# NVlabs/FoundationPose

Measured on AMD Instinct MI355X. Metric: pose-hypotheses/sec (raster+refine+score), 252 hyp x 160x160 @ 640x480 RGB-D, higher is better.
Workload: dtype f16

## Files before the change

foundationpose_amd/_lib.py:

```python
import ctypes as C
import os

import torch

_HERE = os.path.dirname(os.path.abspath(__file__))
LIB_PATH = os.environ.get("FP_AMD_LIB") or os.path.join(_HERE, "csrc", "libfp_amd.so")
ABI_VERSION = 230
_lib = None

vp, ci, cf, cd, sz = C.c_void_p, C.c_int, C.c_float, C.c_double, C.c_size_t

SIGNATURES = {
    "fp_last_error": (C.c_char_p, []),
    "fp_version": (ci, []),
    "fp_mesh_create": (ci, [vp, vp, vp, vp, vp, vp, vp, ci, ci, ci, ci, C.POINTER(vp)]),
    "fp_mesh_destroy": (None, [vp]),
    "fp_mesh_set_create": (ci, [vp, ci, C.POINTER(vp)]),
    "fp_mesh_set_destroy": (None, [vp]),
    "fp_mesh_set_workspace_bytes": (sz, [vp, ci, ci, ci]),
    "fp_depth_erode": (ci, [vp, vp, ci, ci, ci, cf, cf, cf, vp]),
    "fp_depth_bilateral": (ci, [vp, vp, ci, ci, ci, cf, cf, cf, vp]),
    "fp_depth_to_xyz": (ci, [vp, vp, cf, ci, vp, ci, ci, vp]),
    "fp_crop_windows": (ci, [vp, vp, vp, vp, ci, cd, vp, vp, ci, cd, ci, ci, ci, vp, vp, vp]),
    "fp_depth_erode_frames": (ci, [vp, vp, ci, ci, ci, ci, cf, cf, cf, vp]),
    "fp_depth_bilateral_frames": (ci, [vp, vp, ci, ci, ci, ci, cf, cf, cf, vp]),
    "fp_depth_to_xyz_frames": (ci, [vp, vp, cf, ci, vp, ci, ci, ci, vp]),
    "fp_mask_depth_stats": (ci, [vp, vp, vp, ci, ci, ci, ci, cf, vp, vp]),
    "fp_depth_agreement": (ci, [vp, vp, vp, vp, ci, ci, ci, ci, ci, ci, cf, vp, vp]),
    "fp_icp_workspace_bytes": (sz, [ci, ci, ci]),
    "fp_icp_point_plane": (ci, [vp, vp, vp, vp, vp, ci, ci, ci, vp, ci, ci, ci, cf, cd, ci, vp, vp, vp, sz, vp]),
    "fp_pose_errors_workspace_bytes": (sz, [ci, ci, ci]),
    "fp_pose_errors": (ci, [vp, ci, vp, ci, vp, vp, vp, ci, ci, ci, vp, vp, sz, vp]),
    "fp_vsd_counts": (ci, [vp, vp, vp, ci, ci, ci, ci, vp, vp, ci, ci, ci, ci, cf, vp, ci, vp, vp]),
    "fp_mspd": (ci, [vp, ci, vp, ci, vp, vp, vp, ci, ci, vp, vp, vp]),
    "fp_tsdf_integrate": (ci, [vp, vp, vp, vp, vp, ci, ci, ci, ci, ci, ci, vp, cf, cf, cf, vp, vp, vp, vp, vp]),
    "fp_tsdf_count_triangles": (ci, [vp, vp, ci, ci, ci, cf, vp, vp]),
    "fp_tsdf_emit_triangles": (ci, [vp, vp, vp, vp, ci, ci, ci, vp, cf, cf, vp, C.c_longlong, vp, vp, vp, vp, vp]),
    "fp_tsdf_label_components": (ci, [vp, ci, ci, ci, vp, vp, vp]),
    "fp_tsdf_raycast": (ci, [vp, vp, vp, vp, ci, ci, ci, vp, cf, cf, vp, vp, vp, vp, ci, vp, ci, ci, ci, ci, ci, cf, cf, cf, vp, vp, vp, vp, vp]),
    "fp_texture_bake": (ci, [vp, ci, vp, ci, vp, vp, vp, vp, vp, vp, ci, ci, ci, ci, ci, cf, cf, cf, vp, vp, vp]),
    "fp_workspace_bytes": (sz, [ci, ci, ci, ci, ci]),
    "fp_raster_lds_bytes": (sz, [ci]),
    "fp_render_crops": (ci, [vp, vp, vp, vp, cf, vp, vp, vp, vp, vp, ci, ci, ci, ci, ci, ci, cf, cf, cf, ci, vp, vp, vp, vp, vp, vp, vp, vp, sz, vp]),
    "fp_warp_crops": (ci, [vp, vp, vp, vp, vp, vp, vp, ci, vp, cf, vp, vp, ci, ci, ci, ci, ci, ci, ci, ci, vp, vp]),
    "fp_pose_update": (ci, [vp, vp, vp, ci, ci, vp, cf, cf, vp, vp, ci, ci, vp, vp, vp, ci, vp, vp, vp, ci, vp, cf, vp]),
    "fp_conv7x7s2_bn_relu_fwd": (ci, [vp, vp, vp, vp, vp, vp, ci, ci, ci, ci, vp]),
    "fp_igemm_f16_fwd": (ci, [vp, vp, vp, vp, vp, ci, ci, ci, ci, vp, vp]),
    "fp_pack_conv3x3_tiles_f16": (ci, [vp, vp, ci, ci, vp]),
    "fp_pack_conv3x3_tiles_direct_f16": (ci, [vp, vp, ci, ci, vp]),
    "fp_conv3x3_sw_lds_bytes": (ci, []),
    "fp_igemm_splitk_workspace_bytes": (sz, [ci, ci, ci]),
    "fp_igemm_f16_splitk_fwd": (ci, [vp, vp, vp, vp, vp, ci, ci, ci, ci, vp, ci, vp, sz, vp]),
    "fp_add_pe_f16_fwd": (ci, [vp, vp, vp, ci, ci, ci, vp]),
    "fp_replicate_rows_f16": (ci, [vp, vp, ci, ci, ci, ci, ci, C.c_longlong, vp]),
    "fp_replicate_segments_f16": (ci, [vp, vp, ci, ci, ci, ci, ci, C.c_longlong, vp]),
    "fp_layernorm_res_fwd": (ci, [vp, vp, vp, ci, vp, vp, vp, cf, vp, vp, ci, ci, vp]),
    "fp_pack_linear512_f16": (ci, [vp, vp, vp]),
    "fp_linear512_f16_fwd": (ci, [vp, vp, vp, vp, ci, ci, ci, vp]),
    "fp_linear_layernorm_fwd": (ci, [vp, vp, vp, vp, vp, vp, ci, vp, vp, cf, vp, vp, ci, ci, ci, ci, vp]),
    "fp_ffn_layernorm_mean_fwd": (ci, [vp, vp, vp, vp, vp, vp, vp, vp, cf, vp, vp, C.c_size_t, ci, ci, vp]),
    "fp_encoder_tail_workspace_bytes": (sz, [ci, ci]),
    "fp_encoder_tail_mean_fwd": (ci, [vp, ci, vp, vp, vp, vp, vp, vp, vp, vp, vp, vp, vp, vp, cf, vp, vp, sz, ci, ci, vp]),
    "fp_colmean_f16_fwd": (ci, [vp, vp, vp, vp, cf, vp, ci, ci, ci, vp]),
    "fp_rows_linear_fwd": (ci, [vp, vp, vp, vp, ci, ci, ci, ci, vp]),
    "fp_attention_f16_fwd": (ci, [vp, vp, ci, ci, ci, ci, ci, vp]),
    "fp_attention_segments_f16_fwd": (ci, [vp, vp, vp, ci, ci, ci, ci, ci, vp]),
    "fp_cluster_poses": (ci, [cf, cf, vp, ci, vp, ci, vp]),
}


class FpAmdError(RuntimeError):
    pass


def lib():
    global _lib
    if _lib is None:
        if not os.path.exists(LIB_PATH):
            raise FpAmdError(
                f"{LIB_PATH} is missing: the HIP extension is not built (run __graft_entry__.build() or "
                f"`make -C foundationpose_amd/csrc`). There is no CPU fallback.")
        handle = C.CDLL(LIB_PATH)
        for name, (res, args) in SIGNATURES.items():
            fn = getattr(handle, name)
            fn.restype = res
            fn.argtypes = args
        got = int(handle.fp_version())
        if got != ABI_VERSION:
            raise FpAmdError(f"{LIB_PATH} reports ABI version {got}, this binding was written for {ABI_VERSION}: rebuild the library "
                             f"(`make -C foundationpose_amd/csrc`) -- entry points changed meaning between versions (include/fp_amd.h)")
        _lib = handle
    return _lib


def check(status, what):
    if status != 0:
        msg = lib().fp_last_error()
        raise FpAmdError(f"{what} failed ({status}): {msg.decode() if msg else '?'}")
```

foundationpose_amd/csrc/conv_sw.hip:

```cpp
#include <hip/hip_fp16.h>
#include <stdlib.h>
#include <string.h>
#include <type_traits>
#include "igemm_common.h"
#include "igemm_epilogue.h"

#ifdef FP_PROFILE_BUILD
__device__ unsigned long long sw_dbg[10];
extern "C" int fp_dbg_conv_sw(unsigned long long* out, int reset) {
  if (reset) { unsigned long long z[10] = {0, 0, 0, 0, 0, 0, ~0ull, 0, 0, 0}; return (int)hipMemcpyToSymbol(HIP_SYMBOL(sw_dbg), z, sizeof(z)); }
  return (int)hipMemcpyFromSymbol(out, HIP_SYMBOL(sw_dbg), 8 * sizeof(unsigned long long));
}
extern "C" int fp_dbg_conv_sw_direct(unsigned long long* out) {
  return (int)hipMemcpyFromSymbol(out, HIP_SYMBOL(sw_dbg), 2 * sizeof(unsigned long long), 8 * sizeof(unsigned long long));
}
extern "C" int fp_dbg_conv_sw_epilogue(unsigned long long* out, int reset) {
  if (reset) { unsigned long long z[8] = {0, 0, 0, 0, 0, 0, 0, 0}; return (int)hipMemcpyToSymbol(HIP_SYMBOL(ig_epi_dbg), z, sizeof(z)); }
  return (int)hipMemcpyFromSymbol(out, HIP_SYMBOL(ig_epi_dbg), 8 * sizeof(unsigned long long));
}
#define SW_CLK(t) const unsigned long long t = wall_clock64()
#else
#define SW_CLK(t)
#endif

#ifndef SW_DEFAULT_VARIANT
#define SW_DEFAULT_VARIANT 0
#endif

namespace {

constexpr int SW_BK = 32, SW_NSTW = 4;
constexpr int sw_prows(int BM) { return BM == 256 ? 512 : 768; }

template <int N>
__device__ __forceinline__ void sw_wait_vm() {
  static_assert(N >= 0 && N < 64, "vmcnt is a 6-bit field");
  asm volatile("s_waitcnt vmcnt(%0)" ::"n"(N) : "memory");
}

typedef float sw_float4 __attribute__((ext_vector_type(4)));
__device__ __forceinline__ void sw_mfma16(sw_float4& acc, const half8& a, const half8& b) {
  asm volatile("v_mfma_f32_16x16x32_f16 %0, %1, %2, %0" : "+v"(acc) : "v"(a), "v"(b));
}

template <bool DIRECT>
__device__ __forceinline__ void sw_mfma16x(sw_float4& acc, const half8& w, const half8& a) {
  if constexpr (DIRECT) sw_mfma16(acc, a, w);
  else sw_mfma16(acc, w, a);
}

__host__ __device__ constexpr int sw_direct_row(int r) {
  return (r & 64) + 4 * (4 * ((0x2130 >> (4 * ((r >> 2) & 3))) & 3) + (r & 3)) + ((r >> 4) & 3);
}

__device__ __forceinline__ int sw_div(int n, unsigned mul, unsigned shr) { return (int)(__umulhi((unsigned)n, mul) >> shr); }

struct SwGeom {
  int HoWo, Wo, Hp, Wp;
  unsigned mulP, shrP, mulW, shrW;
};

template <typename G>
__device__ __forceinline__ int sw_q(const G& g, int m) {
  const int b = sw_div(m, g.mulP, g.shrP);
  const int r = m - b * g.HoWo;
  const int oy = sw_div(r, g.mulW, g.shrW);
  const int ox = r - oy * g.Wo;
  return (b * g.Hp + oy) * g.Wp + ox;
}

template <int BM, int BN, int TM, bool S16>
__global__ __launch_bounds__(512, 1) void k_conv_sw(IgemmParams p) {
  constexpr bool DIRECT = false;
#include "conv_sw_tile.inc"
}

template <int BM, int BN, int TM, bool S16>
__global__ __launch_bounds__(512, 1) void k_conv_sw_direct(IgemmParams p) {
  constexpr bool DIRECT = true;
#include "conv_sw_tile.inc"
}

constexpr int LS_PROWS = 448, LS_NSTW = 3;

template <int BM, int BN, int TM>
__global__ __launch_bounds__(256, 2) void k_conv_sw_ls(IgemmParams p) {
  constexpr int BK = SW_BK, NW = 4, THREADS = 256;
  constexpr int NWN = BN / 64;
  static_assert((BM / (32 * TM)) * NWN == NW, "4 waves");
  constexpr int ROWB = BK * 2;
  constexpr int W_BYTES = BN * ROWB;
  constexpr int PATCH_BYTES = LS_PROWS * ROWB;
  constexpr int WI = BN / 16 / NW;
  constexpr int PI = LS_PROWS / 16 / NW;
  static_assert(WI >= 1 && PI >= 1 && PI <= 8 && LS_PROWS == PI * 16 * NW, "tile shape");
  constexpr int STAGES_BYTES = 2 * PATCH_BYTES + LS_NSTW * W_BYTES;
  static_assert(STAGES_BYTES >= BM * BN * 2 + BM * 16 + IG_BIAS_LDS, "the epilogue tile, its tables and the vectors reuse the staging area");
  auto swz = [](int row) { return (row >> 2) & 3; };
  extern __shared__ __attribute__((aligned(16))) unsigned char smem[];
  unsigned char* const patch = smem;
  unsigned char* const wring = smem + 2 * PATCH_BYTES;
  const int tid = threadIdx.x, lane = tid & 63;
  const int wid = __builtin_amdgcn_readfirstlane(tid >> 6);
  const int wm = wid / NWN, wn = wid - wm * NWN;

  const int tiles_n = p.N / BN;
  const int nwg = gridDim.x;
  const int xcd = blockIdx.x & 7, loc = blockIdx.x >> 3;
  const int qd8 = nwg >> 3, r8 = nwg & 7;
  const int tile = (xcd < r8 ? xcd * (qd8 + 1) : r8 * (qd8 + 1) + (xcd - r8) * qd8) + loc;
  const int bm = tile / tiles_n, bn = tile - bm * tiles_n;
  const int m0 = bm * BM, n0 = bn * BN;
  const int Cin = p.Cin, Ktot = 9 * Cin, Wp = p.in.Wp;
  const int ncc = Cin / BK;

  const int q0 = sw_q(p.in, m0);
  const int qmax = (p.M / p.in.HoWo) * p.in.Hp * Wp - 1;
  unsigned poff32[PI], woff32[WI];
#pragma unroll
  for (int j = 0; j < PI; ++j) {
    const int row = (wid * PI + j) * 16 + (lane >> 2);
    const int c = (lane & 3) ^ swz(row);
    int q = q0 + row;
    q = q < qmax ? q : qmax;
    poff32[j] = (unsigned)(((long long)q * p.in.cstride + p.in.coff + c * 8) * 2);
  }
#pragma unroll
  for (int j = 0; j < WI; ++j) {
    const int row = (wid * WI + j) * 16 + (lane >> 2);
    const int c = (lane & 3) ^ swz(row);
    woff32[j] = (unsigned)((((size_t)(n0 + row) * Ktot) + c * 8) * 2);
  }
  const __amdgpu_buffer_rsrc_t rsA = __builtin_amdgcn_make_buffer_rsrc(const_cast<_Float16*>(p.A), 0, 0x7FFFFFFF, 0x00020000);
  const __amdgpu_buffer_rsrc_t rsW = __builtin_amdgcn_make_buffer_rsrc(const_cast<_Float16*>(p.Wt), 0, 0x7FFFFFFF, 0x00020000);

  auto stage_patch = [&](int cc, int j) {
    unsigned char* dst = patch + (cc & 1) * PATCH_BYTES + (wid * PI + j) * 1024;
    __builtin_amdgcn_raw_ptr_buffer_load_lds(rsA, (__attribute__((address_space(3))) void*)dst, 16, (int)poff32[j],
                                             cc * (BK * 2), 0, 0);
  };
  auto stage_w = [&](int cc, int tap, int slot) {
    const int wsoff = (tap * Cin + cc * BK) * 2;
    unsigned char* dst = wring + slot * W_BYTES + wid * (WI * 1024);
#pragma unroll
    for (int j = 0; j < WI; ++j)
      __builtin_amdgcn_raw_ptr_buffer_load_lds(rsW, (__attribute__((address_space(3))) void*)(dst + j * 1024), 16,
                                               (int)woff32[j], wsoff, 0, 0);
  };

  float16_ acc[2][TM];
#pragma unroll
  for (int i = 0; i < 2; ++i)
#pragma unroll
    for (int j = 0; j < TM; ++j)
#pragma unroll
      for (int e = 0; e < 16; ++e) acc[i][j][e] = 0.f;

  const int frow = lane & 31, fhalf = lane >> 5;
  int arow[TM], w_off[2][2];
#pragma unroll
  for (int t = 0; t < TM; ++t) {
    int m = m0 + wm * (32 * TM) + t * 32 + frow;
    m = m < p.M ? m : p.M - 1;
    arow[t] = sw_q(p.in, m) - q0;
  }
#pragma unroll
  for (int t = 0; t < 2; ++t) {
    const int rw = wn * 64 + t * 32 + frow;
#pragma unroll
    for (int kk = 0; kk < 2; ++kk) w_off[t][kk] = rw * ROWB + (((2 * kk + fhalf) ^ swz(rw)) << 4);
  }

#pragma unroll
  for (int j = 0; j < PI; ++j) stage_patch(0, j);
  stage_w(0, 0, 0);
  stage_w(0, 1, 1);

  auto kstep = [&](int cc, auto tap_c, auto last_c, auto first_c) {
    constexpr int T = decltype(tap_c)::value;
    constexpr bool LAST = decltype(last_c)::value;
    constexpr bool FIRST = decltype(first_c)::value;
    constexpr int ky = T / 3, kx = T - 3 * ky;
    {
      constexpr bool prev_w = FIRST || T == 0 || !LAST || (T - 1) + 2 < 9;
      constexpr bool prev_p = !FIRST && T >= 1 && !LAST && (T - 1) < PI;
      sw_wait_vm<(prev_w ? WI : 0) + (prev_p ? 1 : 0)>();
    }
    __builtin_amdgcn_sched_barrier(0);
    __builtin_amdgcn_s_barrier();
    __builtin_amdgcn_sched_barrier(0);
    if constexpr (!LAST) {
      if constexpr (T < PI) stage_patch(cc + 1, T);
      if constexpr (T + 2 < 9) stage_w(cc, T + 2, (T + 2) % LS_NSTW);
      else stage_w(cc + 1, T - 7, (T + 2) % LS_NSTW);
    } else {
      if constexpr (T + 2 < 9) stage_w(cc, T + 2, (T + 2) % LS_NSTW);
    }
    const unsigned char* pb = patch + (cc & 1) * PATCH_BYTES;
    const unsigned char* wb = wring + (T % LS_NSTW) * W_BYTES;
    const int shift = ky * Wp + kx;
    half8 fa[2][TM], fw[2][2];
    int a0[TM];
#pragma unroll
    for (int t = 0; t < TM; ++t) {
      int ar = arow[t];
      asm volatile("" : "+v"(ar));
      const int pr = ar + shift;
      a0[t] = (pr << 6) + ((fhalf ^ swz(pr)) << 4);
    }
#pragma unroll
    for (int t = 0; t < TM; ++t) fa[0][t] = *reinterpret_cast<const half8*>(pb + a0[t]);
#pragma unroll
    for (int t = 0; t < 2; ++t) fw[0][t] = *reinterpret_cast<const half8*>(wb + w_off[t][0]);
#pragma unroll
    for (int t = 0; t < TM; ++t) fa[1][t] = *reinterpret_cast<const half8*>(pb + (a0[t] ^ 32));
#pragma unroll
    for (int t = 0; t < 2; ++t) fw[1][t] = *reinterpret_cast<const half8*>(wb + w_off[t][1]);
    __builtin_amdgcn_sched_barrier(0);
#pragma unroll
    for (int kk = 0; kk < 2; ++kk)
#pragma unroll
      for (int i = 0; i < 2; ++i)
#pragma unroll
        for (int j = 0; j < TM; ++j)
          acc[i][j] = __builtin_amdgcn_mfma_f32_32x32x16_f16(fw[kk][i], fa[kk][j], acc[i][j], 0, 0, 0);
    __builtin_amdgcn_sched_barrier(0);
  };
  auto chunk = [&](int cc, auto last_c, auto first_c) {
    kstep(cc, std::integral_constant<int, 0>{}, last_c, first_c);
    kstep(cc, std::integral_constant<int, 1>{}, last_c, std::false_type{});
    kstep(cc, std::integral_constant<int, 2>{}, last_c, std::false_type{});
    kstep(cc, std::integral_constant<int, 3>{}, last_c, std::false_type{});
    kstep(cc, std::integral_constant<int, 4>{}, last_c, std::false_type{});
    kstep(cc, std::integral_constant<int, 5>{}, last_c, std::false_type{});
    kstep(cc, std::integral_constant<int, 6>{}, last_c, std::false_type{});
    kstep(cc, std::integral_constant<int, 7>{}, last_c, std::false_type{});
    kstep(cc, std::integral_constant<int, 8>{}, last_c, std::false_type{});
  };
  chunk(0, std::false_type{}, std::true_type{});
  for (int cc = 1; cc + 1 < ncc; ++cc) chunk(cc, std::false_type{}, std::false_type{});
  chunk(ncc - 1, std::true_type{}, std::false_type{});
  __syncthreads();
  float* bias_lds = reinterpret_cast<float*>(smem + BM * BN * 2 + BM * 16);
  ig_bias_to_lds(p, n0, bias_lds, wid, lane);
  asm volatile("s_waitcnt vmcnt(0)" ::: "memory");
  ig_epilogue<BM, BN, TM, THREADS, 0>(p, acc, smem, m0, n0, wm, wn, tid, lane, bias_lds);
}

template <int BM, int BN, int TM>
int sw_ls_launch(const IgemmParams& p, hipStream_t stream) {
  constexpr int LDS = 2 * LS_PROWS * SW_BK * 2 + LS_NSTW * BN * SW_BK * 2;
  static_assert(2 * LDS <= 160 * 1024, "two workgroups per CU");
  const long long tiles = (long long)fp_cdiv(p.M, BM) * (p.N / BN);
  FP_REQUIRE(tiles < (1ll << 31), "fp_igemm_f16_fwd: too many tiles");
  FP_SET_MAX_LDS((k_conv_sw_ls<BM, BN, TM>), LDS);
  hipLaunchKernelGGL((k_conv_sw_ls<BM, BN, TM>), dim3((unsigned)tiles), dim3(256), LDS, stream, p);
  FP_CHECK_LAUNCH("fp_igemm_f16_fwd(conv_sw_ls)");
  return FP_OK;
}

constexpr int sw_lds_bytes(int BM, int BN) {
  return (BM == 256 ? ig_lds_main_slim<256, 256>(2 * sw_prows(256) * SW_BK * 2 + SW_NSTW * 256 * SW_BK * 2)
                    : ig_lds_main_slim<512, 128>(2 * sw_prows(512) * SW_BK * 2 + SW_NSTW * 128 * SW_BK * 2)) + IG_BIAS_LDS;
}

template <int BM, int BN, int TM, bool S16>
int sw_launch(const IgemmParams& p, hipStream_t stream) {
  static_assert((BM == 256 && BN == 256) || (BM == 512 && BN == 128), "tile shapes of sw_lds_bytes");
  constexpr int LDS = sw_lds_bytes(BM, BN);
  static_assert(LDS <= 160 * 1024, "does not fit the 160 KiB LDS");
  const long long tiles = (long long)fp_cdiv(p.M, BM) * (p.N / BN);
  FP_REQUIRE(tiles < (1ll << 31), "fp_igemm_f16_fwd: too many tiles");
  FP_SET_MAX_LDS((k_conv_sw<BM, BN, TM, S16>), LDS);
  hipLaunchKernelGGL((k_conv_sw<BM, BN, TM, S16>), dim3((unsigned)tiles), dim3(512), LDS, stream, p);
  FP_CHECK_LAUNCH("fp_igemm_f16_fwd(conv_sw)");
  return FP_OK;
}

}

static int sw_span(const IgemmGeom& g, int BM) {
  const int row_cross = (BM - 1) / g.Wo + 1, img_cross = (BM - 1) / g.HoWo + 1;
  return (BM - 1) + 2 * row_cross + (2 * g.Wp + 2) * img_cross + 2 * g.Wp + 3;
}

static int sw_variant(const IgemmParams& p) {
  int v = SW_DEFAULT_VARIANT;
#ifdef FP_PROFILE_BUILD
  static int forced = -2;
  if (forced == -2) {
    const char* e = getenv("FP_CONV_SW");
    forced = e ? (!strcmp(e, "ls") ? 1 : (!strcmp(e, "pp") ? 0 : -1)) : -1;
  }
  if (forced >= 0) v = forced;
#endif
  if (v == 2) v = p.Cin <= 128 ? 1 : 0;
  if (v == 3) v = p.Cin <= 256 ? 1 : 0;
  if (v == 1 && sw_span(p.in, 256) > LS_PROWS) v = 0;
  return v;
}

#ifndef SW_FORCE_512
#define SW_FORCE_512 1
#endif
static bool sw_use_256(const IgemmParams& p) { return (p.N % 256) == 0 && (!SW_FORCE_512 || p.M < 2 * 512); }
static int sw_tile_rows(const IgemmParams& p) { return sw_variant(p) == 1 ? 256 : (sw_use_256(p) ? 256 : 512); }

bool fp_conv3x3_sw_applicable(const IgemmParams& p) {
  const IgemmGeom& g = p.in;
  if (p.taps != 9 || g.stride != 1 || g.off != 0 || g.bsplit != 0) return false;
  if (g.HoWo % g.Wo != 0 || g.Wp != g.Wo + 2 || g.Hp != g.HoWo / g.Wo + 2) return false;
  if (g.Wo < 2) return false;
  const int BM = sw_tile_rows(p);
  if (p.M % g.HoWo != 0 || p.M < 2 * BM) return false;
  if (p.Cin % 64 != 0 || p.N % 128 != 0) return false;
  const long long bytes = (long long)(p.M / g.HoWo) * g.Hp * g.Wp * g.cstride * 2;
  if (bytes >= (1ll << 31)) return false;
  if (g.cstride >= (1 << 19)) return false;
  const IgemmGeom& o = p.out;
  const long long imgs = o.bsplit > 0 ? o.bsplit : p.M / g.HoWo, groups = o.bsplit > 0 ? (p.M / g.HoWo) / o.bsplit + 1 : 0;
  if (imgs * o.Hp * o.Wp * o.cstride + o.coff + groups * (long long)o.cgroup >= (1ll << 31)) return false;
  if (p.R) {
    const IgemmGeom& r = p.res;
    const long long rimgs = r.bsplit > 0 ? r.bsplit : p.M / g.HoWo, rgroups = r.bsplit > 0 ? (p.M / g.HoWo) / r.bsplit + 1 : 0;
    if (rimgs * r.Hp * r.Wp * r.cstride + r.coff + rgroups * (long long)r.cgroup >= (1ll << 31)) return false;
  }
  return sw_span(g, BM) <= (sw_variant(p) == 1 ? LS_PROWS : sw_prows(BM));
}

int fp_conv3x3_sw_tile_rows(const IgemmParams& p) { return sw_tile_rows(p); }

extern "C" int fp_conv3x3_sw_lds_bytes(void) { return sw_lds_bytes(512, 128); }

static bool sw_direct(const IgemmParams& p) {
  if (!p.direct || !p.mfma16 || sw_variant(p) == 1 || sw_use_256(p)) return false;
  return p.epi == IG_EPI_CONV || p.epi == (IG_EPI_CONV | IG_EPI_RES) || p.epi == (IG_EPI_CONV | IG_EPI_BN) || p.epi == (IG_EPI_CONV | IG_EPI_BN | IG_EPI_RES);
}

static int sw_direct_launch(const IgemmParams& p, hipStream_t stream) {
  constexpr int LDS = sw_lds_bytes(512, 128);
  const long long tiles = (long long)fp_cdiv(p.M, 512) * (p.N / 128);
  FP_REQUIRE(tiles < (1ll << 31), "fp_igemm_f16_fwd: too many tiles");
  FP_SET_MAX_LDS((k_conv_sw_direct<512, 128, 4, true>), LDS);
  hipLaunchKernelGGL((k_conv_sw_direct<512, 128, 4, true>), dim3((unsigned)tiles), dim3(512), LDS, stream, p);
  FP_CHECK_LAUNCH("fp_igemm_f16_fwd(conv_sw_direct)");
  return FP_OK;
}

int fp_conv3x3_sw_launch(const IgemmParams& p, hipStream_t stream) {
  const bool direct = sw_direct(p);
  if (p.Wpk && sw_variant(p) != 1 && !sw_use_256(p))
    FP_REQUIRE((p.wpk_direct != 0) == direct, "fp_igemm_f16_fwd: w_tiles is in the layout of %s but this launch runs %s (FP_IGEMM_W_TILES_DIRECT, FP_IGEMM_DIRECT_STORE)",
               p.wpk_direct ? "fp_pack_conv3x3_tiles_direct_f16" : "fp_pack_conv3x3_tiles_f16", direct ? "k_conv_sw_direct" : "k_conv_sw");
  if (direct) return sw_direct_launch(p, stream);
  if (sw_variant(p) == 1) return sw_ls_launch<256, 128, 4>(p, stream);
  if (sw_use_256(p)) return p.mfma16 ? sw_launch<256, 256, 4, true>(p, stream) : sw_launch<256, 256, 4, false>(p, stream);
  return p.mfma16 ? sw_launch<512, 128, 4, true>(p, stream) : sw_launch<512, 128, 4, false>(p, stream);
}

template <bool DIRECT>
__global__ __launch_bounds__(256) void k_pack_conv3x3_tiles(const _Float16* __restrict__ w, _Float16* __restrict__ out, int N, int Cin) {
  const int nk = 9 * (Cin / 32);
  const long long total = (long long)N * nk * 4;
  const long long q = (long long)blockIdx.x * 256 + threadIdx.x;
  if (q >= total) return;
  const int pc = (int)(q & 3);
  const int r = (int)((q >> 2) & 127);
  const long long blk = q >> 9;
  const int s = (int)(blk % nk), bn = (int)(blk / nk);
  const int cc = s / 9, tap = s - 9 * cc;
  const int lc = pc ^ ((r >> 2) & 3);
  const int src = DIRECT ? sw_direct_row(r) : r;
  const half8 v = *reinterpret_cast<const half8*>(w + (size_t)(bn * 128 + src) * (9 * Cin) + tap * Cin + cc * 32 + lc * 8);
  *reinterpret_cast<half8*>(out + q * 8) = v;
}

template <bool DIRECT>
static int sw_pack_tiles(const void* w, void* w_tiles, int N, int Cin, void* stream, const char* who) {
  FP_REQUIRE(w && w_tiles && w != w_tiles, "%s: NULL tensor or in-place repack", who);
  FP_REQUIRE(N > 0 && N % 128 == 0 && Cin > 0 && Cin % 32 == 0, "%s: N=%d must be a multiple of 128, Cin=%d of 32", who, N, Cin);
  FP_REQUIRE((((size_t)w | (size_t)w_tiles) & 15) == 0, "%s: tensors must be 16-byte aligned", who);
  const long long total = (long long)N * 9 * (Cin / 32) * 4;
  hipLaunchKernelGGL(k_pack_conv3x3_tiles<DIRECT>, dim3((unsigned)((total + 255) / 256)), dim3(256), 0, (hipStream_t)stream, (const _Float16*)w,
                     (_Float16*)w_tiles, N, Cin);
  FP_CHECK_LAUNCH(who);
  return FP_OK;
}

extern "C" int fp_pack_conv3x3_tiles_f16(const void* w, void* w_tiles, int N, int Cin, void* stream) {
  return sw_pack_tiles<false>(w, w_tiles, N, Cin, stream, "fp_pack_conv3x3_tiles_f16");
}

extern "C" int fp_pack_conv3x3_tiles_direct_f16(const void* w, void* w_tiles, int N, int Cin, void* stream) {
  return sw_pack_tiles<true>(w, w_tiles, N, Cin, stream, "fp_pack_conv3x3_tiles_direct_f16");
}
```

foundationpose_amd/csrc/conv_sw_tile.inc:

```
  static_assert(!DIRECT || (S16 && BM == 512 && BN == 128 && TM == 4), "the direct epilogue is the 512 x 128 tile's, on 16x16x32 MFMAs");
  constexpr int BK = SW_BK, NW = 8, THREADS = 512;
  constexpr int NWN = BN / 64;
  static_assert((BM / (32 * TM)) * NWN == NW, "8 waves");
  constexpr int ROWB = BK * 2;
  constexpr int W_BYTES = BN * ROWB;
  constexpr int SW_PROWS = sw_prows(BM);
  constexpr int SW_PATCH_BYTES = SW_PROWS * ROWB;
  constexpr int WI = BN / 16 / NW;
  constexpr int PI = SW_PROWS / 16 / NW;
  static_assert(WI >= 1 && PI >= 1 && PI <= 7 && SW_PROWS == PI * 16 * NW, "tile shape");
  constexpr int STAGES_BYTES = 2 * SW_PATCH_BYTES + SW_NSTW * W_BYTES;
  constexpr int LDS_MAIN = ig_lds_main_slim<BM, BN>(STAGES_BYTES);
  auto swz = [](int row) { return (row >> 2) & 3; };
  auto swzp = [](int row) { return S16 ? (row >> 1) & 2 : (row >> 2) & 3; };
  extern __shared__ __attribute__((aligned(16))) unsigned char smem[];
  SW_CLK(t_start);
  unsigned char* const patch = smem;
  unsigned char* const wring = smem + 2 * SW_PATCH_BYTES;
  const int tid = threadIdx.x, lane = tid & 63;
  const int wid = __builtin_amdgcn_readfirstlane(tid >> 6);
  const int grp = wid >> 2;
  const int wm = wid / NWN, wn = wid - wm * NWN;
  float* bias_lds = reinterpret_cast<float*>(smem + LDS_MAIN);

  const _Float16* A_ = p.A;
  const _Float16* W_ = p.Wt;
  const _Float16* Wpk_ = p.Wpk;
  const float* bias_ = p.bias;
  const float* bnsc_ = p.bn_scale;
  const float* bnsh_ = p.bn_shift;
  const int M = p.M, N = p.N, Cin = p.Cin, cstride = p.in.cstride, coff = p.in.coff;
  const SwGeom gi = {p.in.HoWo, p.in.Wo, p.in.Hp, p.in.Wp, p.in.mulP, p.in.shrP, p.in.mulW, p.in.shrW};
  asm volatile("" ::"s"(A_), "s"(W_), "s"(Wpk_), "s"(bias_), "s"(bnsc_), "s"(bnsh_), "s"(M), "s"(N), "s"(Cin), "s"(cstride), "s"(coff),
               "s"(gi.HoWo), "s"(gi.Wo), "s"(gi.Hp), "s"(gi.Wp), "s"(gi.mulP), "s"(gi.shrP), "s"(gi.mulW), "s"(gi.shrW));
  __builtin_amdgcn_sched_barrier(0);

  const int tiles_n = N / BN;
  const int nwg = (int)(((unsigned)M + BM - 1) / BM) * tiles_n;
  const int xcd = blockIdx.x & 7, loc = blockIdx.x >> 3;
  const int qd8 = nwg >> 3, r8 = nwg & 7;
  const int tile = (xcd < r8 ? xcd * (qd8 + 1) : r8 * (qd8 + 1) + (xcd - r8) * qd8) + loc;
  const int bm = __builtin_popcount(tiles_n) == 1 ? tile >> __builtin_ctz(tiles_n) : tile / tiles_n, bn = tile - bm * tiles_n;
  const int m0 = bm * BM, n0 = bn * BN;
  const int Ktot = 9 * Cin, Wp = gi.Wp;
  const int ncc = Cin / BK;
  ig_bias_to_lds(bias_, bnsc_, bnsh_, N, n0, bias_lds, wid, lane);

  const int q0 = sw_q(gi, m0);
  const int qmax = sw_div(M, gi.mulP, gi.shrP) * gi.Hp * Wp - 1;
  unsigned poff32[PI], woff32[WI];
  {
    const int row0 = wid * PI * 16 + (lane >> 2);
    const int c = (lane & 3) ^ swzp(row0);
    static_assert(((16 >> 1) & 2) == 0 && ((16 >> 2) & 3) == 0, "swzp(row0 + 16 j) == swzp(row0)");
    const unsigned ps2 = (unsigned)cstride * 2, omax = (unsigned)qmax * ps2, lane_off = (unsigned)(coff + c * 8) * 2;
    const unsigned o0 = (unsigned)(q0 + row0) * ps2;
#pragma unroll
    for (int j = 0; j < PI; ++j) {
      const unsigned o = o0 + j * 16 * ps2;
      poff32[j] = (o < omax ? o : omax) + lane_off;
    }
  }
#pragma unroll
  for (int j = 0; j < WI; ++j) {
    const int row = (wid * WI + j) * 16 + (lane >> 2);
    const int c = (lane & 3) ^ swz(row);
    const int src = DIRECT ? sw_direct_row(row) : row;
    woff32[j] = (unsigned)((((size_t)(n0 + src) * Ktot) + c * 8) * 2);
  }
  const bool wpk = (BN == 128) && Wpk_ != nullptr;
  if (wpk) {
#pragma unroll
    for (int j = 0; j < WI; ++j) woff32[j] = (unsigned)(((wid * WI + j) * 64 + lane) * 16);
  }
  const int wpk_base = wpk ? bn * (ncc * 9) * W_BYTES : 0;
  const __amdgpu_buffer_rsrc_t rsA = __builtin_amdgcn_make_buffer_rsrc(const_cast<_Float16*>(A_), 0, 0x7FFFFFFF, 0x00020000);
  const __amdgpu_buffer_rsrc_t rsW = __builtin_amdgcn_make_buffer_rsrc(const_cast<_Float16*>(wpk ? Wpk_ : W_), 0, 0x7FFFFFFF, 0x00020000);

  auto stage_patch = [&](int cc, int j) {
    unsigned char* dst = patch + (cc & 1) * SW_PATCH_BYTES + (wid * PI + j) * 1024;
    __builtin_amdgcn_raw_ptr_buffer_load_lds(rsA, (__attribute__((address_space(3))) void*)dst, 16, (int)poff32[j],
                                             cc * (BK * 2), 0, 0);
  };
  auto stage_w = [&](int cc, int tap, int slot) {
    const int wsoff = wpk ? wpk_base + (cc * 9 + tap) * W_BYTES : (tap * Cin + cc * BK) * 2;
    unsigned char* dst = wring + slot * W_BYTES + wid * (WI * 1024);
#pragma unroll
    for (int j = 0; j < WI; ++j)
      __builtin_amdgcn_raw_ptr_buffer_load_lds(rsW, (__attribute__((address_space(3))) void*)(dst + j * 1024), 16,
                                               (int)woff32[j], wsoff, 0, 0);
  };

#pragma unroll
  for (int j = 0; j < PI; ++j) stage_patch(0, j);
  stage_w(0, 0, 0);
  stage_w(0, 1, 1);
  stage_w(0, 2, 2);
  __builtin_amdgcn_sched_barrier(0);
  SW_CLK(t_issue);

  constexpr int NFA = S16 ? 2 * TM : TM, NFW = S16 ? 4 : 2;
  constexpr int FR = S16 ? 16 : 32;
  typedef float float4_ __attribute__((ext_vector_type(4)));
  typedef typename std::conditional<S16, float4_, float16_>::type acc_t;
  acc_t acc[NFW][NFA];
#pragma unroll
  for (int i = 0; i < NFW; ++i)
#pragma unroll
    for (int j = 0; j < NFA; ++j)
#pragma unroll
      for (int e = 0; e < (S16 ? 4 : 16); ++e) acc[i][j][e] = 0.f;

  const int frow = lane & (FR - 1), fhalf = lane >> (S16 ? 4 : 5);
  int arow[NFA], w_off[2][2];
#pragma unroll
  for (int t = 0; t < NFA; ++t) {
    int m = m0 + wm * (32 * TM) + t * FR + frow;
    m = m < M ? m : M - 1;
    arow[t] = sw_q(gi, m) - q0;
    if constexpr (S16) arow[t] = (arow[t] << 6) + (fhalf << 4);
  }
  if constexpr (S16) {
    const int quad = (0x1320 >> (4 * (frow >> 2))) & 3;
#pragma unroll
    for (int t = 0; t < 4; ++t) {
      const int rw = wn * 64 + t * 16 + 4 * quad + (frow & 3);
      w_off[t >> 1][t & 1] = rw * ROWB + ((fhalf ^ swz(rw)) << 4);
    }
  } else {
#pragma unroll
    for (int t = 0; t < 2; ++t) {
      const int rw = wn * 64 + t * 32 + frow;
#pragma unroll
      for (int kk = 0; kk < 2; ++kk) w_off[t][kk] = rw * ROWB + (((2 * kk + fhalf) ^ swz(rw)) << 4);
    }
  }
  static_assert(TM == 4, "the fragment addresses of the next tap are computed behind the MFMA groups of a k-step, one per group of four");
  int anext[NFA], aflip[NFA];
#pragma unroll
  for (int t = 0; t < NFA; ++t) {
    anext[t] = S16 ? arow[t] : (arow[t] << 6) + ((fhalf ^ swz(arow[t])) << 4);
    aflip[t] = S16 ? (arow[t] >> 3) & 32 : 0;
  }

#pragma unroll
  for (int t = 0; t < NFA; ++t) {
    asm volatile("" : "+v"(arow[t]), "+v"(anext[t]));
    if constexpr (S16) asm volatile("" : "+v"(aflip[t]));
  }
  asm volatile("" : "+v"(w_off[0][0]), "+v"(w_off[0][1]), "+v"(w_off[1][0]), "+v"(w_off[1][1]));
#pragma unroll
  for (int i = 0; i < NFW; ++i)
#pragma unroll
    for (int j = 0; j < NFA; ++j) asm volatile("" : "+v"(acc[i][j]));
  if constexpr (DIRECT) {
    static_assert(THREADS == BM && STAGES_BYTES + BM * 4 <= LDS_MAIN, "one thread per row; the table lies behind the stages");
    const int m = m0 + tid;
    reinterpret_cast<int*>(smem + STAGES_BYTES)[tid] = m < M ? (int)(ig_row_off(p.out, m) + n0) : IG_ROW_NONE;
  }
  __builtin_amdgcn_sched_barrier(0);

  sw_wait_vm<2 * WI>();
  __builtin_amdgcn_s_barrier();
  SW_CLK(t_cold);
  if (grp) __builtin_amdgcn_s_barrier();

  half8 fa[2][TM], fw[2][2];
  auto kstep = [&](int cc, auto tap_c, auto last_c) {
    constexpr int T = decltype(tap_c)::value;
    constexpr bool LAST = decltype(last_c)::value;
    constexpr int ky = T / 3, kx = T - 3 * ky;
    const int s = cc * 9 + T;
    const unsigned char* pb = patch + (cc & 1) * SW_PATCH_BYTES;
    const unsigned char* wb = wring + (s & (SW_NSTW - 1)) * W_BYTES;
    const int shift = ky * Wp + kx;
    if constexpr (S16) {
#pragma unroll
      for (int t = 0; t < NFA; ++t) fa[t >> 2][t & 3] = *reinterpret_cast<const half8*>(pb + (anext[t] ^ aflip[t]));
#pragma unroll
      for (int t = 0; t < 4; ++t) fw[t >> 1][t & 1] = *reinterpret_cast<const half8*>(wb + w_off[t >> 1][t & 1]);
    } else {
#pragma unroll
      for (int t = 0; t < TM; ++t) {
        const int a0 = anext[t];
        fa[0][t] = *reinterpret_cast<const half8*>(pb + a0);
        fa[1][t] = *reinterpret_cast<const half8*>(pb + (a0 ^ 32));
      }
#pragma unroll
      for (int kk = 0; kk < 2; ++kk)
#pragma unroll
        for (int t = 0; t < 2; ++t) fw[kk][t] = *reinterpret_cast<const half8*>(wb + w_off[t][kk]);
    }
    (void)shift;
    if constexpr (!LAST) {
      if constexpr (T < PI) stage_patch(cc + 1, T);
      if constexpr (T + 3 < 9) stage_w(cc, T + 3, (s + 3) & (SW_NSTW - 1));
      else stage_w(cc + 1, T - 6, (s + 3) & (SW_NSTW - 1));
      constexpr int NP = (T < PI ? 1 : 0) + ((T >= 1 && T - 1 < PI) ? 1 : 0);
      sw_wait_vm<2 * WI + NP>();
    } else {
      if constexpr (T + 3 < 9) stage_w(cc, T + 3, (s + 3) & (SW_NSTW - 1));
      constexpr int NYOUNGER = T <= 5 ? 2 : (T == 6 ? 1 : 0);
      sw_wait_vm<NYOUNGER * WI>();
    }
    asm volatile("s_waitcnt lgkmcnt(0)" ::: "memory");
    __builtin_amdgcn_sched_barrier(0);
    __builtin_amdgcn_s_barrier();
    __builtin_amdgcn_sched_barrier(0);
    __builtin_amdgcn_s_setprio(1);
    {
      constexpr int TN = (T + 1) % 9, kyn = TN / 3, kxn = TN - 3 * kyn;
      const int shift_n = kyn * Wp + kxn;
      if constexpr (S16) {
        int sh = shift_n << 6;
        asm volatile("" : "+s"(sh));
#pragma unroll
        for (int i = 0; i < 4; ++i)
#pragma unroll
          for (int jh = 0; jh < 2; ++jh) {
            const int t = i * 2 + jh;
            int x, y;
            sw_mfma16x<DIRECT>(acc[i][jh * 4 + 0], fw[i >> 1][i & 1], fa[jh][0]);
            asm volatile("v_add_u32 %0, %1, %2" : "=v"(x) : "s"(sh), "v"(arow[t]));
            sw_mfma16x<DIRECT>(acc[i][jh * 4 + 1], fw[i >> 1][i & 1], fa[jh][1]);
            asm volatile("v_lshrrev_b32 %0, 3, %1" : "=v"(y) : "v"(x));
            sw_mfma16x<DIRECT>(acc[i][jh * 4 + 2], fw[i >> 1][i & 1], fa[jh][2]);
            asm volatile("v_and_b32 %0, 32, %0" : "+v"(y));
            sw_mfma16x<DIRECT>(acc[i][jh * 4 + 3], fw[i >> 1][i & 1], fa[jh][3]);
            anext[t] = x; aflip[t] = y;
          }
      } else {
#pragma unroll
      for (int kk = 0; kk < 2; ++kk)
#pragma unroll
        for (int i = 0; i < 2; ++i) {
#pragma unroll
          for (int j = 0; j < TM; ++j)
            acc[i][j] = __builtin_amdgcn_mfma_f32_32x32x16_f16(fw[kk][i], fa[kk][j], acc[i][j], 0, 0, 0);
          const int t = kk * 2 + i;
          {
            int ar = arow[t];
            asm volatile("" : "+v"(ar));
            const int pr = ar + shift_n;
            anext[t] = (pr << 6) + ((fhalf ^ swz(pr)) << 4);
          }
        }
      }
    }
    __builtin_amdgcn_s_setprio(0);
    __builtin_amdgcn_sched_barrier(0);
    __builtin_amdgcn_s_barrier();
    __builtin_amdgcn_sched_barrier(0);
  };
  auto chunk = [&](int cc, auto last_c) {
    kstep(cc, std::integral_constant<int, 0>{}, last_c);
    kstep(cc, std::integral_constant<int, 1>{}, last_c);
    kstep(cc, std::integral_constant<int, 2>{}, last_c);
    kstep(cc, std::integral_constant<int, 3>{}, last_c);
    kstep(cc, std::integral_constant<int, 4>{}, last_c);
    kstep(cc, std::integral_constant<int, 5>{}, last_c);
    kstep(cc, std::integral_constant<int, 6>{}, last_c);
    kstep(cc, std::integral_constant<int, 7>{}, last_c);
    kstep(cc, std::integral_constant<int, 8>{}, last_c);
  };
  for (int cc = 0; cc + 1 < ncc; ++cc) chunk(cc, std::false_type{});
  chunk(ncc - 1, std::true_type{});
  if (!grp) __builtin_amdgcn_s_barrier();
  __syncthreads();
  SW_CLK(t_loop);
  if constexpr (DIRECT) {
    const IgEpiArgs q = {p.out, p.res, p.R, p.Y, p.pe, p.Ype, p.pe_period, p.pe_mul, p.pe_shr, p.N};
    const int* rowY32 = reinterpret_cast<const int*>(smem + STAGES_BYTES);
#define SW_DIRECT_CASE(E)                                                                                     \
    case E:                                                                                                   \
      if (m0 + BM <= M) ig_epilogue_direct<E, true>(q, acc, smem, rowY32, m0, n0, M, wm, wn, tid, lane, bias_lds);  \
      else ig_epilogue_direct<E, false>(q, acc, smem, rowY32, m0, n0, M, wm, wn, tid, lane, bias_lds);         \
      break
    switch (p.epi) {
      SW_DIRECT_CASE(IG_EPI_CONV);
      SW_DIRECT_CASE(IG_EPI_CONV | IG_EPI_RES);
      SW_DIRECT_CASE(IG_EPI_CONV | IG_EPI_BN);
      SW_DIRECT_CASE(IG_EPI_CONV | IG_EPI_BN | IG_EPI_RES);
      default: break;
    }
#undef SW_DIRECT_CASE
  } else {
    ig_epilogue<BM, BN, TM, THREADS, 0, true>(p, acc, smem, m0, n0, wm, wn, tid, lane, bias_lds);
  }
#ifdef FP_PROFILE_BUILD
  asm volatile("s_waitcnt vmcnt(0)" ::: "memory");
  SW_CLK(t_end);
  if (tid == 0) {
    atomicAdd(&sw_dbg[0], t_cold - t_start); atomicAdd(&sw_dbg[1], t_loop - t_cold); atomicAdd(&sw_dbg[2], t_end - t_loop);
    atomicAdd(&sw_dbg[3], 1ull); atomicAdd(&sw_dbg[4], t_issue - t_start); atomicMin(&sw_dbg[6], t_start); atomicMax(&sw_dbg[7], t_end);
    if constexpr (DIRECT) { atomicAdd(&sw_dbg[8], t_end - t_loop); atomicAdd(&sw_dbg[9], 1ull); }
  }
#endif
```

foundationpose_amd/csrc/igemm.hip:

```cpp
#include <hip/hip_fp16.h>
#include <stdlib.h>
#include <string.h>
#include "igemm_common.h"
#include "igemm_epilogue.h"

int fp_igemm_pp_launch(const IgemmParams& p, int variant, hipStream_t stream);
int fp_conv3x3_sw_launch(const IgemmParams& p, hipStream_t stream);
bool fp_conv3x3_sw_applicable(const IgemmParams& p);
int fp_conv3x3_sw_tile_rows(const IgemmParams& p);

template <int BM, int BN, int TM, int NST, int BK, bool SPLITK = false>
__global__ __launch_bounds__((BM / (32 * TM)) * (BN / 64) * 64, ((BM / (32 * TM)) * (BN / 64) == 4 && TM == 4) ? 2 : 1) void k_igemm_f16(IgemmParams p) {
  constexpr int NWN = BN / 64;
  constexpr int NW = (BM / (32 * TM)) * NWN;
  constexpr int THREADS = NW * 64;
  constexpr int ROWB = BK * 2;
  constexpr int CPK = BK / 8;
  constexpr int RPI = 1024 / ROWB;
  constexpr int KK = BK / 16;
  constexpr int A_BYTES = BM * ROWB;
  constexpr int STAGE_BYTES = A_BYTES + BN * ROWB;
  constexpr int AI = BM / RPI / NW;
  constexpr int WI = BN / RPI / NW;
  static_assert(AI >= 1 && WI >= 1, "tile too small for this wave count");
// ... 14 lines not shown
  const int bm = tile / tiles_n, bn = tile - bm * tiles_n;
  const int m0 = bm * BM, n0 = bn * BN;
  const int Ktot = p.taps * p.Cin;
  if constexpr (!SPLITK) ig_bias_to_lds(p, n0, bias_lds, wid, lane);

  unsigned aoff32[AI], woff32[WI];
#pragma unroll
  for (int j = 0; j < AI; ++j) {
    const int row = wid * (AI * RPI) + j * RPI + lane / CPK;
    const int c = (lane % CPK) ^ swz(row);
    int m = m0 + row;
    m = m < p.M ? m : p.M - 1;
    aoff32[j] = (unsigned)((ig_row_off(p.in, m) + c * 8) * 2);
  }
#pragma unroll
  for (int j = 0; j < WI; ++j) {
    const int row = wid * (WI * RPI) + j * RPI + lane / CPK;
    const int c = (lane % CPK) ^ swz(row);
    woff32[j] = (unsigned)((((size_t)(n0 + row) * Ktot) + c * 8) * 2);
  }
  int nk = p.taps * (p.Cin / BK);
  int st_ci0 = 0, st_kx = 0, st_ky = 0, st_k = 0;
  const int inWp = p.in.Wp, inCs = p.in.cstride, Cin = p.Cin;
  if constexpr (SPLITK) {
    const int split = blockIdx.y, cpt = Cin / BK;
    const int ks0 = (int)(((long long)split * nk) / p.nsplit), ks1 = (int)(((long long)(split + 1) * nk) / p.nsplit);
    const int tap = ks0 / cpt;
    st_k = ks0; st_ci0 = (ks0 - tap * cpt) * BK; st_ky = tap / 3; st_kx = tap - 3 * st_ky;
    nk = ks1 - ks0;
  }
  const __amdgpu_buffer_rsrc_t rsA = __builtin_amdgcn_make_buffer_rsrc(const_cast<_Float16*>(p.A), 0, 0x7FFFFFFF, 0x00020000);
  const __amdgpu_buffer_rsrc_t rsW = __builtin_amdgcn_make_buffer_rsrc(const_cast<_Float16*>(p.Wt), 0, 0x7FFFFFFF, 0x00020000);

  auto stage = [&](int buf) {
    const int asoff = (((st_ky * inWp + st_kx) * inCs) + st_ci0) * 2;
    const int wsoff = st_k * (BK * 2);
    unsigned char* sa = smem + buf * STAGE_BYTES + wid * (AI * 1024);
    unsigned char* sw = smem + buf * STAGE_BYTES + A_BYTES + wid * (WI * 1024);
#pragma unroll
    for (int j = 0; j < AI; ++j)
      __builtin_amdgcn_raw_ptr_buffer_load_lds(rsA, (__attribute__((address_space(3))) void*)(sa + j * 1024), 16,
                                               (int)aoff32[j], asoff, 0, 0);
#pragma unroll
    for (int j = 0; j < WI; ++j)
      __builtin_amdgcn_raw_ptr_buffer_load_lds(rsW, (__attribute__((address_space(3))) void*)(sw + j * 1024), 16,
                                               (int)woff32[j], wsoff, 0, 0);
    ++st_k;
    st_ci0 += BK;
    if (st_ci0 == Cin) { st_ci0 = 0; if (++st_kx == 3) { st_kx = 0; ++st_ky; } }
  };

  float16_ acc[2][TM];
#pragma unroll
  for (int i = 0; i < 2; ++i)
#pragma unroll
    for (int j = 0; j < TM; ++j)
#pragma unroll
      for (int e = 0; e < 16; ++e) acc[i][j][e] = 0.f;

  const int frow = lane & 31, fhalf = lane >> 5;
  int a_off[TM][KK], w_off[2][KK];
#pragma unroll
  for (int t = 0; t < TM; ++t) {
    const int ra = wm * (32 * TM) + t * 32 + frow;
#pragma unroll
    for (int kk = 0; kk < KK; ++kk) a_off[t][kk] = ra * ROWB + (((2 * kk + fhalf) ^ swz(ra)) << 4);
  }
#pragma unroll
  for (int t = 0; t < 2; ++t) {
    const int rw = wn * 64 + t * 32 + frow;
#pragma unroll
    for (int kk = 0; kk < KK; ++kk) w_off[t][kk] = A_BYTES + rw * ROWB + (((2 * kk + fhalf) ^ swz(rw)) << 4);
  }

#pragma unroll
  for (int s = 0; s < NST - 1; ++s)
    if (s < nk) stage(s);
  int buf = 0, nbuf = NST - 1;
  for (int ks = 0; ks < nk; ++ks) {
    if (NST > 2 && ks + NST - 2 < nk) {
      constexpr int INFLIGHT = LPS * (NST - 2);
      static_assert(NST <= 2 || INFLIGHT == 4 || INFLIGHT == 6 || INFLIGHT == 8 || INFLIGHT == 12, "add the counted wait");
      if (INFLIGHT == 4) asm volatile("s_waitcnt vmcnt(4)" ::: "memory");
      else if (INFLIGHT == 6) asm volatile("s_waitcnt vmcnt(6)" ::: "memory");
      else if (INFLIGHT == 8) asm volatile("s_waitcnt vmcnt(8)" ::: "memory");
      else asm volatile("s_waitcnt vmcnt(12)" ::: "memory");
    } else {
      asm volatile("s_waitcnt vmcnt(0)" ::: "memory");
    }
    __builtin_amdgcn_s_barrier();
    if (ks + NST - 1 < nk) stage(nbuf);
    const unsigned char* sb = smem + buf * STAGE_BYTES;
    half8 fa[2][TM], fw[2][2];
    auto load_frags = [&](int kk, int slot) {
#pragma unroll
      for (int t = 0; t < TM; ++t) fa[slot][t] = *reinterpret_cast<const half8*>(sb + a_off[t][kk]);
#pragma unroll
      for (int t = 0; t < 2; ++t) fw[slot][t] = *reinterpret_cast<const half8*>(sb + w_off[t][kk]);
    };
    load_frags(0, 0);
#pragma unroll
    for (int kk = 0; kk < KK; ++kk) {
      if (kk < KK - 1) load_frags(kk + 1, (kk + 1) & 1);
      __builtin_amdgcn_sched_barrier(0);
#pragma unroll
      for (int i = 0; i < 2; ++i)
#pragma unroll
        for (int j = 0; j < TM; ++j)
          acc[i][j] = __builtin_amdgcn_mfma_f32_32x32x16_f16(fw[kk & 1][i], fa[kk & 1][j], acc[i][j], 0, 0, 0);
    }
    buf = (buf + 1 == NST) ? 0 : buf + 1;
    nbuf = (nbuf + 1 == NST) ? 0 : nbuf + 1;
  }
  if constexpr (SPLITK) {
    typedef float float4_ __attribute__((ext_vector_type(4)));
    float4_* dst = reinterpret_cast<float4_*>(p.slab) + ((((size_t)blockIdx.y * nwg + tile) * NW + wid) * (8 * TM)) * 64 + lane;
#pragma unroll
    for (int i = 0; i < 2; ++i)
#pragma unroll
      for (int g = 0; g < 4; ++g)
#pragma unroll
        for (int j = 0; j < TM; ++j) {
          const float4_ v = {acc[i][j][g * 4 + 0], acc[i][j][g * 4 + 1], acc[i][j][g * 4 + 2], acc[i][j][g * 4 + 3]};
          dst[((i * 4 + g) * TM + j) * 64] = v;
        }
    return;
  }
  __syncthreads();

  ig_epilogue<BM, BN, TM, THREADS, 0>(p, acc, smem, m0, n0, wm, wn, tid, lane, bias_lds);
}

template <int BM, int BN, int TM, int NST, int BK>
static int ig_launch(const IgemmParams& p, hipStream_t stream) {
  constexpr int LDS = ig_lds_main<BM, BN>(NST * (BM + BN) * BK * 2) + IG_BIAS_LDS;
  constexpr int THREADS = (BM / (32 * TM)) * (BN / 64) * 64;
  static_assert(LDS <= 160 * 1024, "tile does not fit the 160 KiB LDS");
  const long long tiles = (long long)fp_cdiv(p.M, BM) * (p.N / BN);
  FP_REQUIRE(tiles < (1ll << 31), "fp_igemm_f16_fwd: too many tiles");
  FP_SET_MAX_LDS((k_igemm_f16<BM, BN, TM, NST, BK>), LDS);
  hipLaunchKernelGGL((k_igemm_f16<BM, BN, TM, NST, BK>), dim3((unsigned)tiles), dim3(THREADS), LDS, stream, p);
  FP_CHECK_LAUNCH("fp_igemm_f16_fwd");
  return FP_OK;
}

template <int BM, int BN, int TM>
__global__ __launch_bounds__(256) void k_splitk_epilogue(IgemmParams p, int ntiles) {
  constexpr int NWN = BN / 64, NW = (BM / (32 * TM)) * NWN;
  typedef float float4_ __attribute__((ext_vector_type(4)));
  typedef _Float16 half2_ __attribute__((ext_vector_type(2)));
  const size_t t = (size_t)blockIdx.x * 256 + threadIdx.x;
  const int lane = (int)(t & 63);
  size_t q = t >> 6;
  const int j = (int)(q % TM); q /= TM;
  const int g = (int)(q & 3); q >>= 2;
  const int i = (int)(q & 1); q >>= 1;
  const int wid = (int)(q % NW);
  const int tile = (int)(q / NW);
  if (tile >= ntiles) return;
  const int tiles_n = p.N / BN;
  const int bm = tile / tiles_n, bn = tile - bm * tiles_n;
  const int wm = wid / NWN, wn = wid - wm * NWN;
  const int m = bm * BM + wm * (32 * TM) + j * 32 + (lane & 31);
  const int n = bn * BN + wn * 64 + i * 32 + 8 * g + 4 * (lane >> 5);
  if (m >= p.M) return;
  const float4_* src = reinterpret_cast<const float4_*>(p.slab) + t;
  const size_t per_split = (size_t)ntiles * NW * (8 * TM) * 64;
  float4_ a = src[0];
  for (int s = 1; s < p.nsplit; ++s) {
    const float4_ b = src[(size_t)s * per_split];
    a[0] += b[0]; a[1] += b[1]; a[2] += b[2]; a[3] += b[3];
  }
  float4_ bv = {0.f, 0.f, 0.f, 0.f};
  if (p.bias) bv = *reinterpret_cast<const float4_*>(p.bias + n);
  half4 v;
  if (p.round_acc) {
    const half2_ b01 = {(_Float16)bv[0], (_Float16)bv[1]}, b23 = {(_Float16)bv[2], (_Float16)bv[3]};
    half2_ t01 = {(_Float16)a[0], (_Float16)a[1]};
    half2_ t23 = {(_Float16)a[2], (_Float16)a[3]};
    t01 = t01 + b01;
    t23 = t23 + b23;
    if (p.bn_scale) {
      const float4_ sc = *reinterpret_cast<const float4_*>(p.bn_scale + n), sh = *reinterpret_cast<const float4_*>(p.bn_shift + n);
      v[0] = (_Float16)fmaf((float)t01[0], sc[0], sh[0]);
      v[1] = (_Float16)fmaf((float)t01[1], sc[1], sh[1]);
      v[2] = (_Float16)fmaf((float)t23[0], sc[2], sh[2]);
      v[3] = (_Float16)fmaf((float)t23[1], sc[3], sh[3]);
    } else {
      v[0] = t01[0]; v[1] = t01[1]; v[2] = t23[0]; v[3] = t23[1];
    }
  } else {
#pragma unroll
    for (int e = 0; e < 4; ++e) v[e] = (_Float16)(a[e] + bv[e]);
  }
  if (p.R) v = v + *reinterpret_cast<const half4*>(p.R + ig_row_off(p.res, m) + n);
  if (p.relu) {
    const half4 zero = {0, 0, 0, 0};
    v = __builtin_elementwise_max(v, zero);
  }
  *reinterpret_cast<half4*>(p.Y + ig_row_off(p.out, m) + n) = v;
  if (p.Ype) {
    const float4_ e0 = *reinterpret_cast<const float4_*>(p.pe + (size_t)(m % p.pe_period) * p.N + n);
    half4 w;
#pragma unroll
    for (int e = 0; e < 4; ++e) w[e] = (_Float16)((float)v[e] + e0[e]);
    *reinterpret_cast<half4*>(p.Ype + (size_t)m * p.N + n) = w;
  }
}

constexpr int SK_BM = 128, SK_BN = 128, SK_TM = 2, SK_NST = 2, SK_BK = 64;
static size_t ig_splitk_bytes(int M, int N, int splits) {
  return (size_t)splits * fp_cdiv(M, SK_BM) * (N / SK_BN) * (size_t)(SK_BM * SK_BN * 4);
}
static int ig_launch_splitk(const IgemmParams& p, hipStream_t stream) {
  constexpr int LDS = ig_lds_main<SK_BM, SK_BN>(SK_NST * (SK_BM + SK_BN) * SK_BK * 2) + IG_BIAS_LDS;
  const long long tiles = (long long)fp_cdiv(p.M, SK_BM) * (p.N / SK_BN);
  FP_REQUIRE(tiles * p.nsplit < (1ll << 31) && p.nsplit <= 65535, "fp_igemm_f16_splitk_fwd: too many tiles");
  FP_SET_MAX_LDS((k_igemm_f16<SK_BM, SK_BN, SK_TM, SK_NST, SK_BK, true>), LDS);
  hipLaunchKernelGGL((k_igemm_f16<SK_BM, SK_BN, SK_TM, SK_NST, SK_BK, true>), dim3((unsigned)tiles, (unsigned)p.nsplit), dim3(256), LDS, stream, p);
  FP_CHECK_LAUNCH("fp_igemm_f16_splitk_fwd(partial products)");
  const long long threads = tiles * 4 * (8 * SK_TM) * 64;
  hipLaunchKernelGGL((k_splitk_epilogue<SK_BM, SK_BN, SK_TM>), dim3((unsigned)((threads + 255) / 256)), dim3(256), 0, stream, p, (int)tiles);
  FP_CHECK_LAUNCH("fp_igemm_f16_splitk_fwd(reduce + epilogue)");
  return FP_OK;
}

static int ig_check_geom(const fp_igemm_geom* g, const char* what, const char* who) {
  FP_REQUIRE(g->pixels_per_image > 0 && g->width > 0 && g->padded_h > 0 && g->padded_w > 0 && g->cstride > 0 &&
                 g->stride > 0 && g->offset >= 0 && g->coff >= 0 && g->bsplit >= 0,
             "%s: bad %s geometry", who, what);
  FP_REQUIRE((g->cstride % 8) == 0 && (g->coff % 8) == 0 && (g->cgroup % 8) == 0,
             "%s: %s channel stride/offset must be multiples of 8 (16-byte rows)", who, what);
  return FP_OK;
}

static IgemmGeom ig_geom(const fp_igemm_geom* g) {
  IgemmGeom o;
  o.HoWo = g->pixels_per_image; o.Wo = g->width; o.Hp = g->padded_h; o.Wp = g->padded_w; o.stride = g->stride;
  o.off = g->offset; o.cstride = g->cstride; o.coff = g->coff; o.bsplit = g->bsplit; o.cgroup = g->cgroup;
  ig_fastdiv_init(o.HoWo, &o.mulP, &o.shrP);
  ig_fastdiv_init(o.Wo, &o.mulW, &o.shrW);
  ig_fastdiv_init(o.bsplit, &o.mulB, &o.shrB);
  return o;
}

static int ig_dispatch(IgemmParams& p, hipStream_t stream) {
  int sel = 0;
#ifdef FP_PROFILE_BUILD
  static int forced = -1;
  if (forced < 0) {
    const char* e = getenv("FP_IGEMM_TILE");
    forced = 0;
    if (e) {
      if (!strcmp(e, "128x128")) forced = 1;
      else if (!strcmp(e, "256x128")) forced = 2;
      else if (!strcmp(e, "256x256")) forced = 3;
      else if (!strcmp(e, "ls256x128")) forced = 4;
      else if (!strcmp(e, "pp256x256")) forced = 7;
      else if (!strcmp(e, "pp256x128")) forced = 9;
      else if (!strcmp(e, "generic")) forced = 100;
    }
  }
  sel = forced;
#endif
  const bool sw = sel == 0 && fp_conv3x3_sw_applicable(p);
  if (sel >= 100) sel = 0;
  if (!sw && sel == 0) {
    const bool wide = (p.N % 256) == 0;
    const bool pp = wide && (p.M >= 150000 || p.N >= 1024 || (p.taps == 9 && p.Cin >= 256) || (p.taps == 1 && p.M < 75000 && p.M >= 4096));
    sel = pp ? 7 : 1;
    if ((p.taps == 9 && p.in.stride == 2 && p.Cin <= 64) || (p.taps == 1 && p.N >= 1024)) sel = 4;
  }
  if (sel == 3 && (p.N % 256) != 0) sel = 2;
  if (sel == 7 && (p.N % 256) != 0) sel = 9;
  if (sw) return fp_conv3x3_sw_launch(p, stream);
  if (sel >= 7) return fp_igemm_pp_launch(p, sel - 7, stream);
#ifdef FP_PROFILE_BUILD
  if (sel == 2) return ig_launch<256, 128, 2, 3, 64>(p, stream);
  if (sel == 3) return ig_launch<256, 256, 4, 2, 64>(p, stream);
#endif
  if (sel == 4) return ig_launch<256, 128, 4, 3, 32>(p, stream);
  return ig_launch<128, 128, 2, 2, 64>(p, stream);
}


static int ig_epilogue_mode(const IgemmParams& p, int flags) {
  if (flags & FP_IGEMM_EPILOGUE_GENERIC) return 0;
  if (!p.round_acc || !p.bias || !p.relu || (p.Ype && !p.R)) return 0;
  return IG_EPI_CONV | (p.bn_scale ? IG_EPI_BN : 0) | (p.R ? IG_EPI_RES : 0) | (p.Ype ? IG_EPI_PE : 0);
}

static int ig_build_params(const void* x, const fp_igemm_geom* x_geom, const void* w, void* y, const fp_igemm_geom* y_geom,
                           int M, int N, int Cin, int taps, const fp_igemm_epilogue* ep, IgemmParams& p, const char* who) {
  FP_REQUIRE(x && w && y && x_geom && y_geom, "%s: NULL tensor / geometry", who);
  FP_REQUIRE(taps == 1 || taps == 9, "%s: taps must be 1 (GEMM) or 9 (3x3 conv), got %d", who, taps);
  FP_REQUIRE(N > 0 && N % 128 == 0, "%s: N=%d must be a multiple of 128", who, N);
  FP_REQUIRE(Cin > 0 && Cin % 64 == 0, "%s: Cin=%d must be a multiple of 64", who, Cin);
  static const fp_igemm_epilogue no_epilogue = {nullptr, nullptr, nullptr, nullptr, nullptr, 0, nullptr, 0, nullptr, nullptr};
  const fp_igemm_epilogue& e = ep ? *ep : no_epilogue;
  FP_REQUIRE(!e.residual || e.r_geom, "%s: residual without geometry", who);
  FP_REQUIRE((e.bn_scale == nullptr) == (e.bn_shift == nullptr), "%s: bn_scale and bn_shift go together", who);
  FP_REQUIRE(!e.bn_scale || (e.flags & FP_IGEMM_ROUND_ACC), "%s: BatchNorm needs FP_IGEMM_ROUND_ACC (conv semantics)", who);
  FP_REQUIRE((e.flags & ~(FP_IGEMM_RELU | FP_IGEMM_ROUND_ACC | FP_IGEMM_HAS_W_TILES | FP_IGEMM_MFMA_16X16X32 | FP_IGEMM_MFMA_32X32X16 | FP_IGEMM_EPILOGUE_GENERIC |
                           FP_IGEMM_DIRECT_STORE | FP_IGEMM_W_TILES_DIRECT)) == 0,
             "%s: unknown flags 0x%x", who, e.flags);
  FP_REQUIRE((e.flags & (FP_IGEMM_MFMA_16X16X32 | FP_IGEMM_MFMA_32X32X16)) != (FP_IGEMM_MFMA_16X16X32 | FP_IGEMM_MFMA_32X32X16),
             "%s: FP_IGEMM_MFMA_16X16X32 and FP_IGEMM_MFMA_32X32X16 exclude each other", who);
  FP_REQUIRE((e.pe == nullptr) == (e.y_pe == nullptr) && (!e.pe || e.pe_period > 0), "%s: pe, pe_period and y_pe go together", who);
  FP_REQUIRE((((size_t)x | (size_t)w | (size_t)y | (size_t)e.residual | (size_t)e.bias | (size_t)e.bn_scale | (size_t)e.bn_shift |
               (size_t)e.pe | (size_t)e.y_pe) & 15) == 0, "%s: tensors must be 16-byte aligned", who);
  if (int err = ig_check_geom(x_geom, "input", who)) return err;
  if (int err = ig_check_geom(y_geom, "output", who)) return err;
  if (e.residual) if (int err = ig_check_geom(e.r_geom, "residual", who)) return err;
  const void* w_tiles = (e.flags & FP_IGEMM_HAS_W_TILES) ? e.w_tiles : nullptr;
  FP_REQUIRE(!(e.flags & FP_IGEMM_W_TILES_DIRECT) || w_tiles, "%s: FP_IGEMM_W_TILES_DIRECT without w_tiles (and FP_IGEMM_HAS_W_TILES)", who);
  FP_REQUIRE(!w_tiles || (taps == 9 && (((size_t)w_tiles) & 15) == 0 && w_tiles != w), "%s: w_tiles is for 3x3 convolutions, 16-byte aligned, not w itself", who);
  p.A = (const _Float16*)x; p.Wt = (const _Float16*)w; p.Wpk = (const _Float16*)w_tiles; p.bias = e.bias; p.bn_scale = e.bn_scale; p.bn_shift = e.bn_shift;
  p.R = (const _Float16*)e.residual; p.Y = (_Float16*)y;
  p.pe = e.pe; p.Ype = (_Float16*)e.y_pe; p.pe_period = e.pe_period;
  p.M = M; p.N = N; p.Cin = Cin; p.taps = taps; p.relu = (e.flags & FP_IGEMM_RELU) ? 1 : 0;
  p.round_acc = (e.flags & FP_IGEMM_ROUND_ACC) ? 1 : 0;
  p.mfma16 = (e.flags & FP_IGEMM_MFMA_32X32X16) ? 0 : ((e.flags & FP_IGEMM_MFMA_16X16X32) ? 1 : SW_DEFAULT_MFMA16);
  p.in = ig_geom(x_geom); p.out = ig_geom(y_geom); p.res = e.residual ? ig_geom(e.r_geom) : ig_geom(y_geom);
  p.slab = nullptr; p.nsplit = 0;
  p.epi = ig_epilogue_mode(p, e.flags);
  p.direct = (e.flags & FP_IGEMM_DIRECT_STORE) ? 1 : 0; p.wpk_direct = (e.flags & FP_IGEMM_W_TILES_DIRECT) ? 1 : 0;
  ig_fastdiv_init(p.pe_period, &p.pe_mul, &p.pe_shr);
  return FP_OK;
}

extern "C" int fp_igemm_f16_fwd(const void* x, const fp_igemm_geom* x_geom, const void* w, void* y, const fp_igemm_geom* y_geom,
                                int M, int N, int Cin, int taps, const fp_igemm_epilogue* ep, void* stream) {
  FP_REQUIRE(M >= 0, "fp_igemm_f16_fwd: M < 0");
  if (M == 0) return FP_OK;
  IgemmParams p;
  if (int err = ig_build_params(x, x_geom, w, y, y_geom, M, N, Cin, taps, ep, p, "fp_igemm_f16_fwd")) return err;
  return ig_dispatch(p, (hipStream_t)stream);
}

extern "C" size_t fp_igemm_splitk_workspace_bytes(int M, int N, int splits) {
  if (M <= 0 || N <= 0 || N % SK_BN != 0 || splits <= 0) return 0;
  return ig_splitk_bytes(M, N, splits);
}

extern "C" int fp_igemm_f16_splitk_fwd(const void* x, const fp_igemm_geom* x_geom, const void* w, void* y, const fp_igemm_geom* y_geom,
                                       int M, int N, int Cin, int taps, const fp_igemm_epilogue* ep, int splits, void* workspace,
                                       size_t workspace_bytes, void* stream) {
  FP_REQUIRE(M >= 0, "fp_igemm_f16_splitk_fwd: M < 0");
  if (M == 0) return FP_OK;
  IgemmParams p;
  if (int err = ig_build_params(x, x_geom, w, y, y_geom, M, N, Cin, taps, ep, p, "fp_igemm_f16_splitk_fwd")) return err;
  FP_REQUIRE(!p.Wpk, "fp_igemm_f16_splitk_fwd: w_tiles is the operand layout of the shifted-window kernel; the split-K kernels do not take it");
  const int nk = taps * (Cin / SK_BK);
  FP_REQUIRE(splits >= 1 && splits <= nk, "fp_igemm_f16_splitk_fwd: splits=%d must be in [1, %d] (k-steps of 64)", splits, nk);
  const size_t need = ig_splitk_bytes(M, N, splits);
  if (!workspace || workspace_bytes < need || ((size_t)workspace & 15)) {
    fp_set_error("fp_igemm_f16_splitk_fwd: workspace too small or unaligned (%zu < %zu bytes, see fp_igemm_splitk_workspace_bytes)", workspace_bytes, need);
    return FP_ERR_WORKSPACE;
  }
  p.slab = (float*)workspace; p.nsplit = splits;
  return ig_launch_splitk(p, (hipStream_t)stream);
}
```

foundationpose_amd/csrc/igemm_common.h:

```cpp
#pragma once
#include <hip/hip_fp16.h>
#include <stddef.h>
#include "fp_common.h"

typedef _Float16 half8 __attribute__((ext_vector_type(8)));
typedef _Float16 half4 __attribute__((ext_vector_type(4)));
typedef float float16_ __attribute__((ext_vector_type(16)));

#define IG_BK 64
#ifndef SW_DEFAULT_MFMA16
#define SW_DEFAULT_MFMA16 1
#endif

struct IgemmGeom {
  int HoWo, Wo;
  int Hp, Wp;
  int stride;
  int off;
  int cstride;
  int coff;
  int bsplit;
  int cgroup;
  unsigned mulP, shrP;
  unsigned mulW, shrW;
  unsigned mulB, shrB;
};

static inline void ig_fastdiv_init(int d, unsigned* mul, unsigned* shr) {
  if (d <= 1) { *mul = 0; *shr = 0; return; }
  int lg = 0;
  while ((1u << lg) < (unsigned)d) ++lg;
  const int p = 31 + lg;
  *mul = (unsigned)(((1ull << p) + (unsigned)d - 1) / (unsigned)d);
  *shr = (unsigned)(p - 32);
}
__device__ __forceinline__ int ig_fastdiv(int n, unsigned mul, unsigned shr) {
  return mul ? (int)(__umulhi((unsigned)n, mul) >> shr) : n;
}

struct IgemmParams {
  const _Float16* A;
  const _Float16* Wt;
  const _Float16* Wpk;
  const float* bias;
  const float* bn_scale;
  const float* bn_shift;
  int M, N, Cin, taps;
  IgemmGeom in;
  IgemmGeom out, res;
  const _Float16* R;
  _Float16* Y;
  const float* pe;
  _Float16* Ype;
  int pe_period;
  int relu;
  int round_acc;
  int mfma16;
  int epi;
  unsigned pe_mul, pe_shr;
  int direct;
  float* slab;
  int nsplit;
  int wpk_direct;
};
static_assert(sizeof(IgemmParams) == 336, "IgemmParams grew: the hidden kernel arguments move");
static_assert(sizeof(IgemmGeom) == 64 && offsetof(IgemmParams, in) == 64 && offsetof(IgemmParams, out) == 128, "the head of IgemmParams is its first 128 bytes");

#define IG_EPI_SPEC 1
#define IG_EPI_ROUND_ACC 2
#define IG_EPI_BIAS 4
#define IG_EPI_BN 8
#define IG_EPI_RES 16
#define IG_EPI_RELU 32
#define IG_EPI_PE 64
#define IG_EPI_CONV (IG_EPI_SPEC | IG_EPI_ROUND_ACC | IG_EPI_BIAS | IG_EPI_RELU)

__device__ __forceinline__ long long ig_row_off(const IgemmGeom& g, int m) {
  const int b = ig_fastdiv(m, g.mulP, g.shrP);
  const int r = m - b * g.HoWo;
  const int oy = ig_fastdiv(r, g.mulW, g.shrW);
  const int ox = r - oy * g.Wo;
  int bb = b, cg = 0;
  if (g.bsplit > 0) { cg = ig_fastdiv(b, g.mulB, g.shrB); bb = b - cg * g.bsplit; }
  return (((long long)bb * g.Hp + (oy * g.stride + g.off)) * g.Wp + (ox * g.stride + g.off)) * g.cstride + g.coff +
         (long long)cg * g.cgroup;
}
```

foundationpose_amd/csrc/igemm_epilogue.h:

```cpp
#pragma once
#include <type_traits>
#include "igemm_common.h"

#ifdef FP_PROFILE_BUILD
static __device__ unsigned long long ig_epi_dbg[8];
#define IG_CLK(t) const unsigned long long t = wall_clock64()
#else
#define IG_CLK(t)
#endif

#define IG_VEC_FLOATS 256
#define IG_BIAS_LDS (3 * IG_VEC_FLOATS * 4)

template <int BM, int BN>
constexpr int ig_lds_main(int stage_bytes) {
  return stage_bytes > BM * BN * 2 + BM * 16 ? stage_bytes : BM * BN * 2 + BM * 16;
}

template <int BM, int BN>
constexpr int ig_lds_main_slim(int stage_bytes) {
  return stage_bytes > BM * BN * 2 + BM * 4 ? stage_bytes : BM * BN * 2 + BM * 4;
}
#define IG_ROW_NONE ((int)0x80000000)

typedef float ig_float4 __attribute__((ext_vector_type(4)));
struct IgEpiArgs {
  IgemmGeom out, res;
  const _Float16* R;
  _Float16* Y;
  const float* pe;
  _Float16* Ype;
  int pe_period;
  unsigned pe_mul, pe_shr;
  int N;
};

template <typename T>
__device__ __forceinline__ T* ig_uniform_ptr(const T* ptr) {
  const unsigned long long a = reinterpret_cast<unsigned long long>(ptr);
  const unsigned lo = __builtin_amdgcn_readfirstlane((unsigned)a), hi = __builtin_amdgcn_readfirstlane((unsigned)(a >> 32));
  return reinterpret_cast<T*>(((unsigned long long)hi << 32) | lo);
}

__device__ __forceinline__ half8 ig_relu8(const half8& v) {
  typedef _Float16 half2_ __attribute__((ext_vector_type(2)));
  half8 r;
#pragma unroll
  for (int e = 0; e < 4; ++e) {
    const half2_ x = {v[2 * e], v[2 * e + 1]};
    half2_ y;
    asm("v_pk_max_f16 %0, %1, 0" : "=v"(y) : "v"(x));
    r[2 * e] = y[0]; r[2 * e + 1] = y[1];
  }
  return r;
}

__device__ __forceinline__ half4 ig_relu4(const half4& v) {
  typedef _Float16 half2_ __attribute__((ext_vector_type(2)));
  half4 r;
#pragma unroll
  for (int e = 0; e < 2; ++e) {
    const half2_ x = {v[2 * e], v[2 * e + 1]};
    half2_ y;
    asm("v_pk_max_f16 %0, %1, 0" : "=v"(y) : "v"(x));
    r[2 * e] = y[0]; r[2 * e + 1] = y[1];
  }
  return r;
}

template <int BM, int BN, int TM, int THREADS, bool SLIM, int EPI, typename Acc>
__device__ __forceinline__ void ig_epilogue_spec(const IgEpiArgs& p, Acc& acc, unsigned char* smem, int m0, int n0,
                                                 int wm, int wn, int tid, int lane, const float* bias_lds) {
  constexpr bool S16 = std::is_same<Acc, ig_float4[4][2 * TM]>::value;
  static_assert(S16 || std::is_same<Acc, float16_[2][TM]>::value, "accumulator layout");
  static_assert((EPI & IG_EPI_SPEC) && (EPI & IG_EPI_BIAS), "a layer kind with a bias");
  constexpr bool ROUND_ACC = (EPI & IG_EPI_ROUND_ACC) != 0, HAS_BN = (EPI & IG_EPI_BN) != 0, RES = (EPI & IG_EPI_RES) != 0;
  constexpr bool RELU = (EPI & IG_EPI_RELU) != 0, PE = (EPI & IG_EPI_PE) != 0;
  static_assert(ROUND_ACC || !HAS_BN, "BatchNorm follows the conv rounding");
  constexpr int CPR = BN / 8;
  constexpr int NIT = (BM * CPR) / THREADS;
  constexpr int RPI = THREADS / CPR;
  static_assert(THREADS % CPR == 0 && RPI % 16 == 0 && NIT * RPI == BM, "the store loop's swizzle term must not depend on the iteration");
  constexpr int ROWB = 2 * BN;
  typedef float float4_ __attribute__((ext_vector_type(4)));
  typedef _Float16 half2_ __attribute__((ext_vector_type(2)));
  typedef unsigned uint4_ __attribute__((ext_vector_type(4)));
  unsigned char* E = smem;
  long long* rowY = reinterpret_cast<long long*>(smem + BM * ROWB);
  long long* rowR = SLIM ? reinterpret_cast<long long*>(smem) : rowY + BM;
  int* rowY32 = reinterpret_cast<int*>(smem + BM * ROWB);
  const long long baseY = SLIM ? ig_row_off(p.out, m0) + n0 : 0;
  IG_CLK(te0);
  for (int r = tid; r < BM; r += THREADS) {
    const int m = m0 + r;
    if constexpr (SLIM) rowY32[r] = (int)(ig_row_off(p.out, m) + n0 - baseY);
    else rowY[r] = ig_row_off(p.out, m) + n0;
    if constexpr (RES) rowR[r] = ig_row_off(p.res, m) + n0;
  }
  __syncthreads();
  IG_CLK(te1);
  const int ml0 = tid / CPR, ch = tid % CPR;
  half8 rv[RES ? NIT : 1];
  constexpr int NRG = S16 ? 4 : 8;
  static_assert(NIT % NRG == 0, "residual loads per channel group");
  unsigned roff[RES && SLIM ? NIT : 1];
  const __amdgpu_buffer_rsrc_t rsR = __builtin_amdgcn_make_buffer_rsrc(ig_uniform_ptr(p.R), 0, -1, 0x00020000);
  auto res_group = [&](int g) {
    if constexpr (RES && SLIM) {
#pragma unroll
      for (int it = g * (NIT / NRG); it < (g + 1) * (NIT / NRG); ++it)
        rv[it] = __builtin_bit_cast(half8, __builtin_amdgcn_raw_buffer_load_b128(rsR, (int)roff[it], 0, 0));
      __builtin_amdgcn_sched_barrier(0);
    }
  };
  if constexpr (RES) {
    if constexpr (SLIM) {
      const int* rR = reinterpret_cast<const int*>(rowR + ml0);
#pragma unroll
      for (int it = 0; it < NIT; ++it) roff[it] = ((unsigned)rR[it * RPI * 2] + ch * 8) << 1;
      __builtin_amdgcn_sched_barrier(0);
      asm volatile("s_waitcnt lgkmcnt(0)" ::: "memory");
      __builtin_amdgcn_s_barrier();
      __builtin_amdgcn_sched_barrier(0);
    } else {
      const long long* rR = rowR + ml0;
#pragma unroll
      for (int it = 0; it < NIT; ++it) rv[it] = *reinterpret_cast<const half8*>(p.R + rR[it * RPI] + ch * 8);
    }
  }
  IG_CLK(te2);
  struct Vecs { float4_ bv, sc, sh; half2_ b01, b23; };
  auto vecs = [&](int nl) {
    Vecs c;
    c.bv = *reinterpret_cast<const float4_*>(bias_lds + nl);
    c.b01 = half2_{(_Float16)c.bv[0], (_Float16)c.bv[1]};
    c.b23 = half2_{(_Float16)c.bv[2], (_Float16)c.bv[3]};
    if constexpr (HAS_BN) {
      c.sc = *reinterpret_cast<const float4_*>(bias_lds + IG_VEC_FLOATS + nl);
      c.sh = *reinterpret_cast<const float4_*>(bias_lds + 2 * IG_VEC_FLOATS + nl);
    }
    return c;
  };
  auto put4 = [&](unsigned char* dst, float a0, float a1, float a2, float a3, const Vecs& c) {
    half4 v;
    if constexpr (ROUND_ACC) {
      half2_ t01 = {(_Float16)a0, (_Float16)a1};
      half2_ t23 = {(_Float16)a2, (_Float16)a3};
      t01 = t01 + c.b01;
      t23 = t23 + c.b23;
      if constexpr (HAS_BN) {
        v[0] = (_Float16)fmaf((float)t01[0], c.sc[0], c.sh[0]);
        v[1] = (_Float16)fmaf((float)t01[1], c.sc[1], c.sh[1]);
        v[2] = (_Float16)fmaf((float)t23[0], c.sc[2], c.sh[2]);
        v[3] = (_Float16)fmaf((float)t23[1], c.sc[3], c.sh[3]);
      } else {
        v[0] = t01[0]; v[1] = t01[1]; v[2] = t23[0]; v[3] = t23[1];
      }
    } else {
      v[0] = (_Float16)(a0 + c.bv[0]); v[1] = (_Float16)(a1 + c.bv[1]); v[2] = (_Float16)(a2 + c.bv[2]); v[3] = (_Float16)(a3 + c.bv[3]);
    }
    *reinterpret_cast<half4*>(dst) = v;
  };
  const int r15 = lane & 15;
  if constexpr (S16) {
    const int quad = (0x1320 >> (4 * (lane >> 4))) & 3;
    unsigned char* Erow = E + (wm * (32 * TM) + r15) * ROWB + ((quad & 1) << 3);
    const int cx = (wn * 8 + (quad >> 1)) ^ r15;
#pragma unroll
    for (int i = 0; i < 4; ++i) {
      res_group(i);
      const Vecs c = vecs(wn * 64 + i * 16 + 4 * quad);
      unsigned char* Ei = Erow + ((cx ^ (2 * i)) << 4);
#pragma unroll
      for (int j = 0; j < 2 * TM; ++j) put4(Ei + j * (16 * ROWB), acc[i][j][0], acc[i][j][1], acc[i][j][2], acc[i][j][3], c);
    }
  } else {
    unsigned char* Erow = E + (wm * (32 * TM) + (lane & 31)) * ROWB + ((lane >> 5) << 3);
    const int cx = (wn * 8) ^ r15;
#pragma unroll
    for (int i = 0; i < 2; ++i) {
#pragma unroll
      for (int g = 0; g < 4; ++g) {
        res_group(i * 4 + g);
        const Vecs c = vecs(wn * 64 + i * 32 + 8 * g + 4 * (lane >> 5));
        unsigned char* Ei = Erow + ((cx ^ (4 * i + g)) << 4);
#pragma unroll
        for (int j = 0; j < TM; ++j)
          put4(Ei + j * (32 * ROWB), acc[i][j][g * 4 + 0], acc[i][j][g * 4 + 1], acc[i][j][g * 4 + 2], acc[i][j][g * 4 + 3], c);
      }
    }
  }
  __syncthreads();
  IG_CLK(te3);
  const unsigned char* Erd = E + ml0 * ROWB + ((ch ^ (ml0 & 15)) << 4);
  const __amdgpu_buffer_rsrc_t rsY = __builtin_amdgcn_make_buffer_rsrc(ig_uniform_ptr(p.Y), 0, -1, 0x00020000);
  const unsigned cbY = ((unsigned)baseY + ch * 8) << 1;
#pragma unroll
  for (int it = 0; it < NIT; ++it) {
    half8 v = *reinterpret_cast<const half8*>(Erd + it * (RPI * ROWB));
    if constexpr (RES) v = v + rv[it];
    if constexpr (RELU) v = ig_relu8(v);
    if constexpr (SLIM) __builtin_amdgcn_raw_buffer_store_b128(__builtin_bit_cast(uint4_, v), rsY, (int)(cbY + ((unsigned)rowY32[ml0 + it * RPI] << 1)), 0, 0);
    else *reinterpret_cast<half8*>(p.Y + rowY[ml0 + it * RPI] + ch * 8) = v;
    if constexpr (PE) {
      const int m = m0 + ml0 + it * RPI;
      const int mp = m - ig_fastdiv(m, p.pe_mul, p.pe_shr) * p.pe_period;
      const float* per = p.pe + (size_t)mp * p.N + n0 + ch * 8;
      const float4_ e0 = *reinterpret_cast<const float4_*>(per), e1 = *reinterpret_cast<const float4_*>(per + 4);
      half8 w;
#pragma unroll
      for (int e = 0; e < 4; ++e) { w[e] = (_Float16)((float)v[e] + e0[e]); w[4 + e] = (_Float16)((float)v[4 + e] + e1[e]); }
      *reinterpret_cast<half8*>(p.Ype + (size_t)m * p.N + n0 + ch * 8) = w;
      __builtin_amdgcn_sched_barrier(0);
    }
  }
#ifdef FP_PROFILE_BUILD
  IG_CLK(te4);
  if (tid == 0) {
    atomicAdd(&ig_epi_dbg[0], te1 - te0); atomicAdd(&ig_epi_dbg[1], te2 - te1); atomicAdd(&ig_epi_dbg[2], te3 - te2);
    atomicAdd(&ig_epi_dbg[3], te4 - te3); atomicAdd(&ig_epi_dbg[4], 1ull);
  }
#endif
}
template <int EPI, bool FULL, typename Acc>
__device__ __forceinline__ void ig_epilogue_direct(const IgEpiArgs& p, Acc& acc, unsigned char* smem, const int* rowY32, int m0, int n0, int M,
                                                   int wm, int wn, int tid, int lane, const float* bias_lds) {
  constexpr int TM = 4;
  static_assert(std::is_same<Acc, ig_float4[4][2 * TM]>::value, "accumulators of the 16x16x32 loop");
  static_assert((EPI & IG_EPI_CONV) == IG_EPI_CONV && !(EPI & IG_EPI_PE), "conv rounding + bias + ReLU, without the positional output");
  constexpr bool HAS_BN = (EPI & IG_EPI_BN) != 0, RES = (EPI & IG_EPI_RES) != 0;
  typedef float float4_ __attribute__((ext_vector_type(4)));
  typedef int int4_ __attribute__((ext_vector_type(4)));
  typedef unsigned uint2_ __attribute__((ext_vector_type(2)));
  typedef _Float16 half2_ __attribute__((ext_vector_type(2)));
  constexpr int JG = 2, NG = 2 * TM / JG;
  const int nl = wn * 64 + 4 * (lane & 15);
  const int prow = wm * (32 * TM) + 4 * (lane >> 4);
  int* rowR32 = reinterpret_cast<int*>(smem);
  IG_CLK(te0);
  if constexpr (RES) {
    const int m = FULL || m0 + tid < M ? m0 + tid : M - 1;
    rowR32[tid] = (int)(ig_row_off(p.res, m) + n0);
    __syncthreads();
  }
  IG_CLK(te1);
  const float4_ bv = *reinterpret_cast<const float4_*>(bias_lds + nl);
  const half2_ b01 = {(_Float16)bv[0], (_Float16)bv[1]}, b23 = {(_Float16)bv[2], (_Float16)bv[3]};
  float4_ sc, sh;
  if constexpr (HAS_BN) {
    sc = *reinterpret_cast<const float4_*>(bias_lds + IG_VEC_FLOATS + nl);
    sh = *reinterpret_cast<const float4_*>(bias_lds + 2 * IG_VEC_FLOATS + nl);
  }
  const __amdgpu_buffer_rsrc_t rsY = __builtin_amdgcn_make_buffer_rsrc(ig_uniform_ptr(p.Y), 0, -1, 0x00020000);
  const __amdgpu_buffer_rsrc_t rsR = __builtin_amdgcn_make_buffer_rsrc(ig_uniform_ptr(p.R), 0, -1, 0x00020000);
  half4 rv[RES ? 2 : 1][JG * 4];
  auto res_group = [&](int g) {
    if constexpr (RES) {
#pragma unroll
      for (int jj = 0; jj < JG; ++jj) {
        const int4_ ro = *reinterpret_cast<const int4_*>(rowR32 + prow + 16 * (g * JG + jj));
#pragma unroll
        for (int e = 0; e < 4; ++e)
          rv[g & 1][jj * 4 + e] = __builtin_bit_cast(half4, __builtin_amdgcn_raw_buffer_load_b64(rsR, (int)((unsigned)(ro[e] + nl) << 1), 0, 0));
      }
      __builtin_amdgcn_sched_barrier(0);
    }
  };
  res_group(0);
#pragma unroll
  for (int g = 0; g < NG; ++g) {
    if (g + 1 < NG) res_group(g + 1);
#pragma unroll
    for (int jj = 0; jj < JG; ++jj) {
      const int j = g * JG + jj;
      const int4_ yo = *reinterpret_cast<const int4_*>(rowY32 + prow + 16 * j);
#pragma unroll
      for (int e = 0; e < 4; ++e) {
        half4 v;
        half2_ t01 = {(_Float16)acc[0][j][e], (_Float16)acc[1][j][e]};
        half2_ t23 = {(_Float16)acc[2][j][e], (_Float16)acc[3][j][e]};
        t01 = t01 + b01;
        t23 = t23 + b23;
        if constexpr (HAS_BN) {
          v[0] = (_Float16)fmaf((float)t01[0], sc[0], sh[0]);
          v[1] = (_Float16)fmaf((float)t01[1], sc[1], sh[1]);
          v[2] = (_Float16)fmaf((float)t23[0], sc[2], sh[2]);
          v[3] = (_Float16)fmaf((float)t23[1], sc[3], sh[3]);
        } else {
          v[0] = t01[0]; v[1] = t01[1]; v[2] = t23[0]; v[3] = t23[1];
        }
        if constexpr (RES) v = v + rv[g & 1][jj * 4 + e];
        v = ig_relu4(v);
        if (FULL || yo[e] != IG_ROW_NONE)
          __builtin_amdgcn_raw_buffer_store_b64(__builtin_bit_cast(uint2_, v), rsY, (int)((unsigned)(yo[e] + nl) << 1), 0, 0);
      }
    }
    __builtin_amdgcn_sched_barrier(0);
  }
#ifdef FP_PROFILE_BUILD
  IG_CLK(te2);
  if (tid == 0) { atomicAdd(&ig_epi_dbg[5], te1 - te0); atomicAdd(&ig_epi_dbg[6], te2 - te1); atomicAdd(&ig_epi_dbg[7], 1ull); }
#endif
}

template <int BM, int BN, int TM, int THREADS, int DBG, bool FULL, bool SLIM, int EPI = 0, typename Acc, typename P>
__device__ __forceinline__ void ig_epilogue_body(const P& p, Acc& acc, unsigned char* smem, int m0, int n0,
                                                 int wm, int wn, int tid, int lane, const float* bias_lds) {
  if constexpr (EPI != 0) {
    static_assert(FULL && std::is_same<P, IgEpiArgs>::value, "the layer-kind bodies take whole tiles and their own argument block");
    ig_epilogue_spec<BM, BN, TM, THREADS, SLIM, EPI>(p, acc, smem, m0, n0, wm, wn, tid, lane, bias_lds);
  } else {
  static_assert(std::is_same<P, IgemmParams>::value, "the generic body reads IgemmParams");
  constexpr bool S16 = std::is_same<Acc, ig_float4[4][2 * TM]>::value;
  static_assert(S16 || std::is_same<Acc, float16_[2][TM]>::value, "accumulator layout");
  constexpr int CPR = BN / 8;
  constexpr int NIT = (BM * CPR) / THREADS;
  unsigned char* E = smem;
  typedef float float4_ __attribute__((ext_vector_type(4)));
  const bool round_acc = p.round_acc != 0, has_bn = p.bn_scale != nullptr;
  long long* rowY = reinterpret_cast<long long*>(smem + BM * 2 * BN);
  long long* rowR = SLIM ? reinterpret_cast<long long*>(smem) : rowY + BM;
  int* rowY32 = reinterpret_cast<int*>(smem + BM * 2 * BN);
  const long long baseY = SLIM ? ig_row_off(p.out, m0) + n0 : 0;
  auto row_exists = [&](int ml) { return SLIM ? rowY32[ml] != IG_ROW_NONE : rowY[ml] >= 0; };
  IG_CLK(te0);
  for (int r = tid; r < BM; r += THREADS) {
    const int m = m0 + r;
    const bool in = m < p.M;
    if constexpr (SLIM) rowY32[r] = in ? (int)(ig_row_off(p.out, m) + n0 - baseY) : IG_ROW_NONE;
    else rowY[r] = in ? ig_row_off(p.out, m) + n0 : -1;
    if (p.R) rowR[r] = in ? ig_row_off(p.res, m) + n0 : 0;
  }
  __syncthreads();
  IG_CLK(te1);
  half8 rv[NIT];
  if (p.R) {
#pragma unroll
    for (int it = 0; it < NIT; ++it) {
      const int qd = tid + it * THREADS;
      const int ml = qd / CPR, ch = qd % CPR;
      if (FULL || row_exists(ml)) rv[it] = *reinterpret_cast<const half8*>(p.R + rowR[ml] + ch * 8);
    }
    if constexpr (SLIM) {
      __builtin_amdgcn_sched_barrier(0);
      asm volatile("s_waitcnt lgkmcnt(0)" ::: "memory");
      __builtin_amdgcn_s_barrier();
      __builtin_amdgcn_sched_barrier(0);
    }
  }
  IG_CLK(te2);
  auto put4 = [&](int nl, int ml, float a0, float a1, float a2, float a3, const float4_& bv, const float4_& sc, const float4_& sh) {
    half4 v;
    if (round_acc) {
      typedef _Float16 half2_ __attribute__((ext_vector_type(2)));
      const half2_ b01 = {(_Float16)bv[0], (_Float16)bv[1]}, b23 = {(_Float16)bv[2], (_Float16)bv[3]};
      half2_ t01 = {(_Float16)a0, (_Float16)a1};
      half2_ t23 = {(_Float16)a2, (_Float16)a3};
      t01 = t01 + b01;
      t23 = t23 + b23;
      if (has_bn) {
        v[0] = (_Float16)fmaf((float)t01[0], sc[0], sh[0]);
        v[1] = (_Float16)fmaf((float)t01[1], sc[1], sh[1]);
        v[2] = (_Float16)fmaf((float)t23[0], sc[2], sh[2]);
        v[3] = (_Float16)fmaf((float)t23[1], sc[3], sh[3]);
      } else {
        v[0] = t01[0]; v[1] = t01[1]; v[2] = t23[0]; v[3] = t23[1];
      }
    } else {
      v[0] = (_Float16)(a0 + bv[0]); v[1] = (_Float16)(a1 + bv[1]); v[2] = (_Float16)(a2 + bv[2]); v[3] = (_Float16)(a3 + bv[3]);
    }
    const int chunk = (nl >> 3) ^ (ml & 15);
    *reinterpret_cast<half4*>(E + ml * (2 * BN) + (chunk << 4) + ((nl & 4) << 1)) = v;
  };
  auto vecs = [&](int nl, float4_& bv, float4_& sc, float4_& sh) {
    bv = *reinterpret_cast<const float4_*>(bias_lds + nl);
    sc = float4_{1.f, 1.f, 1.f, 1.f}; sh = float4_{0.f, 0.f, 0.f, 0.f};
    if (has_bn) {
      sc = *reinterpret_cast<const float4_*>(bias_lds + IG_VEC_FLOATS + nl);
      sh = *reinterpret_cast<const float4_*>(bias_lds + 2 * IG_VEC_FLOATS + nl);
    }
  };
  if constexpr (S16) {
    const int quad = (0x1320 >> (4 * (lane >> 4))) & 3;
#pragma unroll
    for (int i = 0; i < 4; ++i) {
      const int nl = wn * 64 + i * 16 + 4 * quad;
      float4_ bv, sc, sh;
      vecs(nl, bv, sc, sh);
#pragma unroll
      for (int j = 0; j < 2 * TM; ++j) {
        const int ml = wm * (32 * TM) + j * 16 + (lane & 15);
        put4(nl, ml, acc[i][j][0], acc[i][j][1], acc[i][j][2], acc[i][j][3], bv, sc, sh);
      }
    }
  } else {
#pragma unroll
    for (int i = 0; i < 2; ++i) {
#pragma unroll
      for (int g = 0; g < 4; ++g) {
        const int nl = wn * 64 + i * 32 + 8 * g + 4 * (lane >> 5);
        float4_ bv, sc, sh;
        vecs(nl, bv, sc, sh);
#pragma unroll
        for (int j = 0; j < TM; ++j) {
          const int ml = wm * (32 * TM) + j * 32 + (lane & 31);
          put4(nl, ml, acc[i][j][g * 4 + 0], acc[i][j][g * 4 + 1], acc[i][j][g * 4 + 2], acc[i][j][g * 4 + 3], bv, sc, sh);
        }
      }
    }
  }
  __syncthreads();
  IG_CLK(te3);
  const half8 zero = {0, 0, 0, 0, 0, 0, 0, 0};
#pragma unroll
  for (int it = 0; it < NIT; ++it) {
    const int qd = tid + it * THREADS;
    const int ml = qd / CPR, ch = qd % CPR;
    if (!FULL && !row_exists(ml)) continue;
    const long long yo = SLIM ? baseY + rowY32[ml] : rowY[ml];
    half8 v = *reinterpret_cast<const half8*>(E + ml * (2 * BN) + ((ch ^ (ml & 15)) << 4));
    if (p.R) v = v + rv[it];
    if (p.relu) v = __builtin_elementwise_max(v, zero);
    *reinterpret_cast<half8*>(p.Y + yo + ch * 8) = v;
    if (p.Ype) {
      const int m = m0 + ml;
      const float* per = p.pe + (size_t)(m % p.pe_period) * p.N + n0 + ch * 8;
      const float4_ e0 = *reinterpret_cast<const float4_*>(per), e1 = *reinterpret_cast<const float4_*>(per + 4);
      half8 w;
#pragma unroll
      for (int e = 0; e < 4; ++e) { w[e] = (_Float16)((float)v[e] + e0[e]); w[4 + e] = (_Float16)((float)v[4 + e] + e1[e]); }
      *reinterpret_cast<half8*>(p.Ype + (size_t)m * p.N + n0 + ch * 8) = w;
    }
  }
#ifdef FP_PROFILE_BUILD
  IG_CLK(te4);
  if (tid == 0) {
    atomicAdd(&ig_epi_dbg[0], te1 - te0); atomicAdd(&ig_epi_dbg[1], te2 - te1); atomicAdd(&ig_epi_dbg[2], te3 - te2);
    atomicAdd(&ig_epi_dbg[3], te4 - te3); atomicAdd(&ig_epi_dbg[4], 1ull);
  }
#endif
  }
}

template <int BM, int BN, int TM, int THREADS, int DBG = 0, bool SLIM = false, typename Acc>
__device__ __forceinline__ void ig_epilogue(const IgemmParams& p, Acc& acc, unsigned char* smem, int m0, int n0,
                                            int wm, int wn, int tid, int lane, const float* bias_lds) {
  if (m0 + BM <= p.M) {
    if constexpr (DBG == 0) {
#define IG_EPI_CASE(E) case E: ig_epilogue_body<BM, BN, TM, THREADS, DBG, true, SLIM, E>(q, acc, smem, m0, n0, wm, wn, tid, lane, bias_lds); return
      const IgEpiArgs q = {p.out, p.res, p.R, p.Y, p.pe, p.Ype, p.pe_period, p.pe_mul, p.pe_shr, p.N};
      switch (p.epi) {
        IG_EPI_CASE(IG_EPI_CONV);
        IG_EPI_CASE(IG_EPI_CONV | IG_EPI_RES);
        IG_EPI_CASE(IG_EPI_CONV | IG_EPI_RES | IG_EPI_PE);
        IG_EPI_CASE(IG_EPI_CONV | IG_EPI_BN);
        IG_EPI_CASE(IG_EPI_CONV | IG_EPI_BN | IG_EPI_RES);
        IG_EPI_CASE(IG_EPI_CONV | IG_EPI_BN | IG_EPI_RES | IG_EPI_PE);
        default: break;
      }
#undef IG_EPI_CASE
    }
    ig_epilogue_body<BM, BN, TM, THREADS, DBG, true, SLIM>(p, acc, smem, m0, n0, wm, wn, tid, lane, bias_lds);
  }
  else ig_epilogue_body<BM, BN, TM, THREADS, DBG, false, SLIM>(p, acc, smem, m0, n0, wm, wn, tid, lane, bias_lds);
}
__device__ __forceinline__ void ig_bias_to_lds(const float* bias, const float* bn_scale, const float* bn_shift, int N, int n0, float* bias_lds,
                                               int wid, int lane) {
  if (wid > 2) return;
  const float* src = wid == 0 ? bias : (wid == 1 ? bn_scale : bn_shift);
  float* dst = bias_lds + wid * IG_VEC_FLOATS;
  if (src) {
    const __amdgpu_buffer_rsrc_t rs = __builtin_amdgcn_make_buffer_rsrc(const_cast<float*>(src), 0, N * 4, 0x00020000);
    __builtin_amdgcn_raw_ptr_buffer_load_lds(rs, (__attribute__((address_space(3))) void*)dst, 16, lane * 16, n0 * 4, 0, 0);
  } else if (wid == 0) {
    typedef float f4 __attribute__((ext_vector_type(4)));
    *reinterpret_cast<f4*>(dst + lane * 4) = f4{0.f, 0.f, 0.f, 0.f};
  }
}
__device__ __forceinline__ void ig_bias_to_lds(const IgemmParams& p, int n0, float* bias_lds, int wid, int lane) {
  ig_bias_to_lds(p.bias, p.bn_scale, p.bn_shift, p.N, n0, bias_lds, wid, lane);
}
```

foundationpose_amd/engine.py:

```python
import contextlib

import torch
import torch.nn.functional as F

from . import ops

USE_MIOPEN = False


FUSED_OUT_PROJ_LN = True


FUSED_FFN = True


ROWS_QKV = True
ROWS_QKV_MIN_ROWS = 4096
PACKED_CONV_TILES = True
MERGED_HEAD_QKV = True
FUSED_TAIL = True
CONV_MFMA_16X16X32 = True
SPECIALIZED_EPILOGUE = True
CONV_DIRECT_STORE = True


def _conv_backend():
    if USE_MIOPEN or not torch.backends.cudnn.is_available():
        return contextlib.nullcontext()
    return torch.backends.cudnn.flags(enabled=False)


def _bn_affine(sd, bn_p):
    if bn_p is None or (bn_p + ".weight") not in sd:
        return None, None
    scale = sd[bn_p + ".weight"].float() / torch.sqrt(sd[bn_p + ".running_var"].float() + 1e-5)
    shift = sd[bn_p + ".bias"].float() - sd[bn_p + ".running_mean"].float() * scale
    return scale.contiguous(), shift.contiguous()


def _r16(t):
    return t.to(torch.float16).to(torch.float32).contiguous()


class _Conv:

    def __init__(self, sd, conv_p, bn_p, stride, dtype, channels_last):
        w = sd[conv_p + ".weight"].float()
        b = sd.get(conv_p + ".bias")
        b = torch.zeros(w.shape[0], device=w.device) if b is None else b.float()
        scale, shift = _bn_affine(sd, bn_p)
        if scale is not None:
            w, b = w * scale[:, None, None, None], b * scale + shift
        wf = w.to(dtype)
        self.w = wf.contiguous(memory_format=torch.channels_last) if channels_last else wf.contiguous()
        self.b = b.to(dtype)
        self.stride = stride
        self.pad = (w.shape[-1] - 1) // 2

    def __call__(self, x, relu=True):
        y = F.conv2d(x, self.w, self.b, stride=self.stride, padding=self.pad)
        return F.relu_(y) if relu else y


class _Block:
    def __init__(self, sd, p, dtype, cl):
        self.c1 = _Conv(sd, p + ".conv1", p + ".bn1", 1, dtype, cl)
        self.c2 = _Conv(sd, p + ".conv2", p + ".bn2", 1, dtype, cl)

    def __call__(self, x):
        y = self.c2(self.c1(x), relu=False)
        y += x
        return F.relu_(y)


class _Encoder:

    def __init__(self, sd, stem, joint, dtype, channels_last):
        cl = channels_last
        self.dtype, self.cl = dtype, cl
        self.c1 = _Conv(sd, stem + ".0.net.0", stem + ".0.net.1", 2, dtype, cl)
        self.c2 = _Conv(sd, stem + ".1.net.0", stem + ".1.net.1", 2, dtype, cl)
        self.s2, self.s3 = _Block(sd, stem + ".2", dtype, cl), _Block(sd, stem + ".3", dtype, cl)
        self.j0, self.j1 = _Block(sd, joint + ".0", dtype, cl), _Block(sd, joint + ".1", dtype, cl)
        self.j2 = _Conv(sd, joint + ".2.net.0", joint + ".2.net.1", 2, dtype, cl)
        self.j3, self.j4 = _Block(sd, joint + ".3", dtype, cl), _Block(sd, joint + ".4", dtype, cl)
        self.pe = sd["pos_embed.pe"].to(dtype)

    def __call__(self, AB):
        n = AB.shape[0] // 2
        if self.cl:
            AB = AB.contiguous(memory_format=torch.channels_last)
        x = self.s3(self.s2(self.c2(self.c1(AB))))
        ab = torch.cat((x[:n], x[n:]), dim=1)
        ab = self.j4(self.j3(self.j2(self.j1(self.j0(ab)))))
        tok = ab.permute(0, 2, 3, 1).reshape(n, -1, ab.shape[1])
        return tok + self.pe[:, : tok.shape[1]]


class _TorchMHA:

    def __init__(self, sd, p, dtype, nhead=4):
        self.wi, self.bi = sd[p + ".in_proj_weight"].to(dtype), sd[p + ".in_proj_bias"].to(dtype)
        self.wo, self.bo = sd[p + ".out_proj.weight"].to(dtype), sd[p + ".out_proj.bias"].to(dtype)
        self.nhead = nhead

    def __call__(self, x):
        Bn, L, D = x.shape
        hd = D // self.nhead
        qkv = F.linear(x, self.wi, self.bi).reshape(Bn, L, 3, self.nhead, hd)
        q, k, v = (qkv[:, :, i].permute(0, 2, 1, 3) for i in range(3))
        ctx = F.scaled_dot_product_attention(q, k, v).permute(0, 2, 1, 3).reshape(Bn, L, D)
        return F.linear(ctx, self.wo, self.bo)


class _TorchEncoderLayer:

    def __init__(self, sd, p, dtype):
        self.att = _TorchMHA(sd, p + ".self_attn", dtype)
        self.l1 = (sd[p + ".linear1.weight"].to(dtype), sd[p + ".linear1.bias"].to(dtype))
        self.l2 = (sd[p + ".linear2.weight"].to(dtype), sd[p + ".linear2.bias"].to(dtype))
        self.n1 = (sd[p + ".norm1.weight"].to(dtype), sd[p + ".norm1.bias"].to(dtype))
        self.n2 = (sd[p + ".norm2.weight"].to(dtype), sd[p + ".norm2.bias"].to(dtype))

    def __call__(self, x):
        x = F.layer_norm(x + self.att(x), (x.shape[-1],), self.n1[0], self.n1[1], 1e-5)
        ff = F.linear(F.relu(F.linear(x, *self.l1)), *self.l2)
        return F.layer_norm(x + ff, (x.shape[-1],), self.n2[0], self.n2[1], 1e-5)


def _conv_params(sd, conv_p, bn_p, second_output=False):
    w = sd[conv_p + ".weight"].float()
    b = sd.get(conv_p + ".bias")
    scale, shift = _bn_affine(sd, bn_p)
    wk = w.permute(0, 2, 3, 1).reshape(w.shape[0], -1).to(torch.float16).contiguous()
    tiles, direct = None, bool(CONV_DIRECT_STORE and CONV_MFMA_16X16X32 and SPECIALIZED_EPILOGUE and b is not None and not second_output)
    if wk.is_cuda and w.shape[2] == 3 and w.shape[3] == 3 and w.shape[0] % 128 == 0 and w.shape[1] % 32 == 0 and PACKED_CONV_TILES:
        tiles = (ops.pack_conv3x3_tiles_direct if direct else ops.pack_conv3x3_tiles)(wk, w.shape[0], w.shape[1])
    return dict(w=wk, w_tiles=tiles, tiles_direct=direct and tiles is not None, bias=None if b is None else _r16(b.float()), scale=scale, shift=shift)


SPLITK_MAX_HYPS = 12
HEADS_TWO_STREAMS_MAX_HYPS = 12
SPLITK_TARGET_WGS = 384
SMALL_CALL_CEILING = 31

_SWITCHES = ("FUSED_OUT_PROJ_LN", "FUSED_FFN", "ROWS_QKV", "PACKED_CONV_TILES", "MERGED_HEAD_QKV", "FUSED_TAIL", "CONV_MFMA_16X16X32", "SPECIALIZED_EPILOGUE", "CONV_DIRECT_STORE", "SPLITK_MAX_HYPS", "HEADS_TWO_STREAMS_MAX_HYPS")


@contextlib.contextmanager
def overrides(**kw):
    g = globals()
    for k, v in kw.items():
        if k not in _SWITCHES:
            raise KeyError(f"engine.overrides: unknown switch {k!r} (known: {', '.join(_SWITCHES)})")
        if k.endswith("_MAX_HYPS") and not (0 <= int(v) <= SMALL_CALL_CEILING):
            raise ValueError(f"engine.overrides: {k} = {v} is outside 0..{SMALL_CALL_CEILING}")
    saved = {k: g[k] for k in kw}
    g.update(kw)
    try:
        yield
    finally:
        g.update(saved)


def small_call(n, limit):
    return n <= min(int(limit), SMALL_CALL_CEILING)


def splitk_pieces(rows, cout, cin):
    tiles = -(-rows // 128) * (cout // 128)
    nk = 9 * cin // 64
    return max(1, min(nk // 2, round(SPLITK_TARGET_WGS / tiles)))


class _HipEncoder:

    def __init__(self, sd, stem, joint, device):
        c1 = sd[stem + ".0.net.0.weight"].float()
        self.c1_w = c1.to(torch.float16).reshape(64, -1).contiguous()
        b1 = sd.get(stem + ".0.net.0.bias")
        self.c1_b = None if b1 is None else _r16(b1.float())
        self.c1_scale, self.c1_shift = _bn_affine(sd, stem + ".0.net.1")
        names = [("c2", stem + ".1.net.0", stem + ".1.net.1")]
        for blk, pre in (("s2", stem + ".2"), ("s3", stem + ".3"), ("j0", joint + ".0"), ("j1", joint + ".1"),
                         ("j3", joint + ".3"), ("j4", joint + ".4")):
            names += [(blk + "a", pre + ".conv1", pre + ".bn1"), (blk + "b", pre + ".conv2", pre + ".bn2")]
        names.append(("j2", joint + ".2.net.0", joint + ".2.net.1"))
        self.w = {k: _conv_params(sd, c, b, second_output=(k == "j4b")) for k, c, b in names}
        self.pe = sd["pos_embed.pe"].float().reshape(-1, sd["pos_embed.pe"].shape[-1]).contiguous()
        self.device = device
        self._bufs = {}

    def _buffers(self, n, H, W, slot, small=True):
        small = bool(small) and small_call(n, SPLITK_MAX_HYPS)
        key = (n, H, W, slot, small)
        b = self._bufs.get(key)
        if b is None:
            z = lambda *shape: torch.zeros(shape, dtype=torch.float16, device=self.device)
            h1, w1, h2, w2, h3, w3 = H // 2, W // 2, H // 4, W // 4, H // 8, W // 8
            sk = None
            if small:
                need = max(ops.igemm_splitk_workspace_bytes(r, co, splitk_pieces(r, co, ci))
                           for r, co, ci in ((2 * n * h2 * w2, 128, 64), (2 * n * h2 * w2, 128, 128), (n * h2 * w2, 256, 256),
                                             (n * h3 * w3, 512, 256), (n * h3 * w3, 512, 512)))
                sk = torch.empty(need, dtype=torch.uint8, device=self.device)
            b = dict(SK=sk, P1=z(2 * n, h1 + 2, w1 + 2, 64), P2=z(2 * n, h2 + 2, w2 + 2, 128), P3=z(2 * n, h2 + 2, w2 + 2, 128),
                     T=z(2 * n, h2 + 2, w2 + 2, 128), CAT=z(n, h2 + 2, w2 + 2, 256), J0=z(n, h2 + 2, w2 + 2, 256),
                     T2=z(n, h2 + 2, w2 + 2, 256), Q0=z(n, h3 + 2, w3 + 2, 512), Q1=z(n, h3 + 2, w3 + 2, 512),
                     T3=z(n, h3 + 2, w3 + 2, 512), dims=(h1, w1, h2, w2, h3, w3))
            self._bufs[key] = b
        return b

    def _conv(self, name, x, Bn, Ho, Wo, Cin, Cout, y, stride=1, res=None, relu=True, gout=None, gres=None, pe=None, y_pe=None, sk=None,
              sk_rows=None):
        c = self.w[name]
        G = ops.IgemmGeom.image
        gin = G(Ho, Wo, 1, Cin, stride=stride, offset=0)
        gout = gout if gout is not None else G(Ho, Wo, 1, Cout)
        if res is not None and gres is None:
            gres = G(Ho, Wo, 1, Cout)
        if sk is not None:
            return ops.igemm_f16_splitk(x, gin, c["w"], c["bias"], y, gout, Bn * Ho * Wo, Cout, Cin, 9,
                                        splitk_pieces(sk_rows if sk_rows is not None else Bn * Ho * Wo, Cout, Cin), sk,
                                        relu=relu, residual=res, r_geom=gres, bn_scale=c["scale"], bn_shift=c["shift"],
                                        conv_rounding=True, pe=pe, y_pe=y_pe)
        return ops.igemm_f16(x, gin, c["w"], c["bias"], y, gout, Bn * Ho * Wo, Cout, Cin, 9, relu=relu, residual=res, r_geom=gres,
                             bn_scale=c["scale"], bn_shift=c["shift"], conv_rounding=True, pe=pe, y_pe=y_pe,
                             w_tiles=c["w_tiles"] if stride == 1 else None, w_tiles_direct=c["tiles_direct"] and stride == 1)

    def __call__(self, AB, slot=0, shared_b=False, small_calls=True):
        n2, _, H, W = AB.shape
        segs = shared_b if isinstance(shared_b, ops.Segments) else None
        if segs is not None:
            n = n2 - len(segs)
            if segs.total != n:
                raise ValueError(f"shared_b: {n2} images and {len(segs)} segments, but the segments cover {segs.total} pairs")
        else:
            n = n2 - 1 if shared_b else n2 // 2
        b = self._buffers(n, H, W, slot, small_calls)
        h1, w1, h2, w2, h3, w3 = b["dims"]
        G = ops.IgemmGeom.image
        ops.conv7x7s2_bn_relu(AB, self.c1_w, self.c1_b, self.c1_scale, self.c1_shift, b["P1"][:n2], 1)
        self._conv("c2", b["P1"], n2, h2, w2, 64, 128, b["P2"], stride=2, sk=b["SK"], sk_rows=2 * n * h2 * w2)
        self._conv("s2a", b["P2"], n2, h2, w2, 128, 128, b["T"], sk=b["SK"], sk_rows=2 * n * h2 * w2)
        self._conv("s2b", b["T"], n2, h2, w2, 128, 128, b["P3"], res=b["P2"], sk=b["SK"], sk_rows=2 * n * h2 * w2)
        self._conv("s3a", b["P3"], n2, h2, w2, 128, 128, b["T"], sk=b["SK"], sk_rows=2 * n * h2 * w2)
        self._conv("s3b", b["T"], n2, h2, w2, 128, 128, b["CAT"], res=b["P3"],
                   gout=G(h2, w2, 1, 256, bsplit=n, cgroup=128), gres=G(h2, w2, 1, 128), sk=b["SK"], sk_rows=2 * n * h2 * w2)
        if segs is not None:
            ops.replicate_segments(b["CAT"], segs, 128, 256)
        elif shared_b and n > 1:
            ops.replicate_channels(b["CAT"], n, 128, 256)
        self._conv("j0a", b["CAT"], n, h2, w2, 256, 256, b["T2"], sk=b["SK"])
        self._conv("j0b", b["T2"], n, h2, w2, 256, 256, b["J0"], res=b["CAT"], sk=b["SK"])
        self._conv("j1a", b["J0"], n, h2, w2, 256, 256, b["T2"], sk=b["SK"])
        self._conv("j1b", b["T2"], n, h2, w2, 256, 256, b["CAT"], res=b["J0"], sk=b["SK"])
        self._conv("j2", b["CAT"], n, h3, w3, 256, 512, b["Q0"], stride=2, sk=b["SK"])
        self._conv("j3a", b["Q0"], n, h3, w3, 512, 512, b["T3"], sk=b["SK"])
        self._conv("j3b", b["T3"], n, h3, w3, 512, 512, b["Q1"], res=b["Q0"], sk=b["SK"])
        self._conv("j4a", b["Q1"], n, h3, w3, 512, 512, b["T3"], sk=b["SK"])
        tok = torch.empty((n, h3 * w3, 512), dtype=torch.float16, device=AB.device)
        x16 = torch.empty_like(tok)
        self._conv("j4b", b["T3"], n, h3, w3, 512, 512, tok, res=b["Q1"], gout=G(h3, w3, 0, 512), gres=G(h3, w3, 1, 512),
                   pe=self.pe[: h3 * w3], y_pe=x16, sk=b["SK"])
        return tok, x16


class _HipLinear:

    def __init__(self, w, b):
        assert w.shape[0] % 128 == 0 and w.shape[1] % 64 == 0
        self.w = w.to(torch.float16).contiguous()
        self.b = _r16(b.float())

    def __call__(self, x, relu=False):
        x2 = x.reshape(-1, x.shape[-1])
        M, K = x2.shape
        No = self.w.shape[0]
        y = torch.empty((M, No), dtype=torch.float16, device=x.device)
        Gm = ops.IgemmGeom.matrix
        ops.igemm_f16(x2, Gm(K), self.w, self.b, y, Gm(No), M, No, K, 1, relu=relu)
        return y.reshape(*x.shape[:-1], No)


class _HipRowsLinear:

    def __init__(self, w, b):
        self.w = w.to(torch.float16).contiguous()
        self.b = _r16(b.float())

    def __call__(self, x, round_f16=True, out_f16=False, out=None):
        return ops.rows_linear(x, self.w, self.b, round_f16=round_f16, out_f16=out_f16, out=out)


class _HipMHA:
    def __init__(self, sd, p, fp16_scores, nhead=4, small_calls=True):
        self.qkv = _HipLinear(sd[p + ".in_proj_weight"], sd[p + ".in_proj_bias"])
        self.out = _HipLinear(sd[p + ".out_proj.weight"], sd[p + ".out_proj.bias"])
        self.out_rows = _HipRowsLinear(sd[p + ".out_proj.weight"], sd[p + ".out_proj.bias"])
        self.nhead, self.fp16_scores = nhead, fp16_scores
        self.qkv_p = ops.PackedLinear512(self.qkv.w) if tuple(self.qkv.w.shape) == (1536, 512) else None
        self.small_calls = small_calls
        self._sk = {}

    def context(self, x16, slot=0, small_calls=True):
        Bn, L, D = x16.shape
        qkv = self.in_proj(x16, slot, small_calls)
        return ops.attention_f16(qkv.reshape(Bn, L, 3 * D), self.nhead, fp16_scores=self.fp16_scores)

    def in_proj(self, x16, slot=0, small_calls=True):
        Bn, L, D = x16.shape
        if ROWS_QKV and self.qkv_p is not None and Bn * L >= ROWS_QKV_MIN_ROWS:
            qkv = ops.linear512(x16, self.qkv_p, self.qkv.b)
        elif self.small_calls and small_calls and small_call(Bn, SPLITK_MAX_HYPS) and D % 64 == 0 and D // 64 >= 4:
            M, No = Bn * L, self.qkv.w.shape[0]
            pieces = max(1, min(D // 64 // 2, round(SPLITK_TARGET_WGS / (-(-M // 128) * (No // 128)))))
            key = (M, No, pieces, x16.device, slot)
            ws = self._sk.get(key)
            if ws is None:
                ws = self._sk[key] = torch.empty(ops.igemm_splitk_workspace_bytes(M, No, pieces), dtype=torch.uint8, device=x16.device)
            qkv = torch.empty((M, No), dtype=torch.float16, device=x16.device)
            Gm = ops.IgemmGeom.matrix
            ops.igemm_f16_splitk(x16.reshape(M, D), Gm(D), self.qkv.w, self.qkv.b, qkv, Gm(No), M, No, D, 1, pieces, ws)
        else:
            qkv = self.qkv(x16)
        return qkv

    def __call__(self, x16, slot=0, small_calls=True):
        return self.out(self.context(x16, slot, small_calls))


class _HipEncoderLayer:

    def __init__(self, sd, p):
        self.att = _HipMHA(sd, p + ".self_attn", fp16_scores=False)
        self.l1 = _HipLinear(sd[p + ".linear1.weight"], sd[p + ".linear1.bias"])
        self.l2 = _HipLinear(sd[p + ".linear2.weight"], sd[p + ".linear2.bias"])
        self.n1 = (sd[p + ".norm1.weight"].float().contiguous(), sd[p + ".norm1.bias"].float().contiguous())
        self.n2 = (sd[p + ".norm2.weight"].float().contiguous(), sd[p + ".norm2.bias"].float().contiguous())
        self.out_p, self.l1_p, self.l2_p = (ops.PackedLinear512(m.w) for m in (self.att.out, self.l1, self.l2))

    def pooled(self, tok16, x16, pe, slot=0, small_calls=True):
        return self.pooled_from_context(self.att.context(x16, slot, small_calls), tok16, pe)

    def pooled_from_context(self, ctx16, tok16, pe):
        if FUSED_TAIL and FUSED_OUT_PROJ_LN and FUSED_FFN and ctx16.shape[1] % 16 == 0 and tuple(pe.shape) == (ctx16.shape[1], 512):
            return ops.encoder_tail_mean(ctx16, self.out_p, self.att.out.b, tok16, pe, self.n1[0], self.n1[1], self.l1_p, self.l1.b,
                                         self.l2_p, self.l2.b, self.n2[0], self.n2[1], 1e-5)
        if FUSED_OUT_PROJ_LN:
            y32, y16 = ops.linear_layernorm_res(ctx16, self.out_p, self.att.out.b, self.n1[0], self.n1[1], 1e-5, tok16=tok16, pe=pe)
        else:
            sa = self.att.out(ctx16.contiguous())
            y32, y16 = ops.layernorm_res(sa, self.n1[0], self.n1[1], 1e-5, tok16=tok16, pe=pe)
        if FUSED_FFN and y16.shape[1] % 16 == 0:
            return ops.ffn_layernorm_mean(y16, self.l1_p, self.l1.b, self.l2_p, self.l2.b, y32, self.n2[0], self.n2[1], 1e-5)
        ff = self.l2(self.l1(y16, relu=True))
        return ops.colmean_f16(ff, self.n2[0], self.n2[1], 1e-5, resid32=y32)


def _check_precision(precision):
    if precision not in ("fp16", "fp32", "torch_amp"):
        raise ValueError(f"precision must be 'fp16', 'fp32' or 'torch_amp', got {precision!r}")


def _dev_sd(module_or_sd, device):
    sd = module_or_sd.state_dict() if hasattr(module_or_sd, "state_dict") else module_or_sd
    return {k: v.detach().to(device) for k, v in sd.items()}


class RefinePlan:
    small_calls = True

    def __init__(self, model, device, precision="fp16", channels_last=True):
        _check_precision(precision)
        self.dtype = torch.float16 if precision == "fp16" else torch.float32
        self.hip = self.dtype == torch.float16
        self.module = model if precision == "torch_amp" else None
        if self.module is not None:
            return
        sd = _dev_sd(model, device)
        self.heads = {}
        if self.hip:
            self.enc = _HipEncoder(sd, "encodeA", "encodeAB", device)
            for name in ("trans", "rot"):
                self.heads[name] = (_HipEncoderLayer(sd, f"{name}_head.0"),
                                    _HipRowsLinear(sd[f"{name}_head.1.weight"], sd[f"{name}_head.1.bias"]))
            wt, wr = (self.heads[n][0].att.qkv for n in ("trans", "rot"))
            if tuple(wt.w.shape) == (1536, 512) and tuple(wr.w.shape) == (1536, 512):
                cut = lambda t: (t[0:512], t[512:1024], t[1024:1536])
                self.qkv2_p = ops.PackedLinear512(torch.cat([p for pair in zip(cut(wt.w), cut(wr.w)) for p in pair], 0).contiguous())
                self.qkv2_b = torch.cat([p for pair in zip(cut(wt.b), cut(wr.b)) for p in pair], 0).contiguous()
            else:
                self.qkv2_p = None
        else:
            self.enc = _Encoder(sd, "encodeA", "encodeAB", self.dtype, channels_last)
            for name in ("trans", "rot"):
                self.heads[name] = (_TorchEncoderLayer(sd, f"{name}_head.0", self.dtype),
                                    sd[f"{name}_head.1.weight"].to(self.dtype), sd[f"{name}_head.1.bias"].to(self.dtype))

    def _head_side_stream(self, tok16):
        if not getattr(self, "two_stream_heads", True) or not self.small_calls or not small_call(tok16.shape[0], HEADS_TWO_STREAMS_MAX_HYPS) \
                or tok16.device.type != "cuda" or ops.KernelTimers.active is not None:
            return None
        from . import overlap
        if torch.cuda.is_current_stream_capturing() and not overlap.reserved(tok16.device, 1):
            return None
        if not overlap.side_streams_overlap(tok16.device, 1):
            return None
        return overlap.reserve_streams(tok16.device, 1)[0]

    @torch.inference_mode()
    def __call__(self, AB, slot=0, shared_b=False):
        out = {}
        if shared_b is not False and shared_b is not None and not self.hip:
            raise ValueError("shared_b is a property of the fp16 plan; expand the observed crop for the torch plans")
        if self.module is not None:
            n = AB.shape[0] // 2
            with _conv_backend(), torch.autocast("cuda", dtype=torch.float16):
                o = self.module(AB[:n], AB[n:])
            return {k: v.float() for k, v in o.items()}
        if self.hip:
            sc = self.small_calls
            tok16, x16 = self.enc(AB, slot, shared_b=shared_b, small_calls=sc)
            run = lambda name, hslot: self.heads[name][1](self.heads[name][0].pooled(tok16, x16, self.enc.pe, hslot, sc), round_f16=True)
            side = self._head_side_stream(tok16)
            if side is None:
                n_seq, L = int(tok16.shape[0]), int(tok16.shape[1])
                if MERGED_HEAD_QKV and self.qkv2_p is not None and ROWS_QKV and n_seq * L >= ROWS_QKV_MIN_ROWS and \
                        not (sc and small_call(n_seq, SPLITK_MAX_HYPS)):
                    ctx = ops.attention_f16(ops.linear512(x16, self.qkv2_p, self.qkv2_b), 8)
                    for i, name in enumerate(("trans", "rot")):
                        layer, lin = self.heads[name]
                        out[name] = lin(layer.pooled_from_context(ctx[..., 512 * i:512 * (i + 1)], tok16, self.enc.pe), round_f16=True)
                    return out
                for name in self.heads:
                    out[name] = run(name, slot)
                return out
            cur = torch.cuda.current_stream(tok16.device)
            side.wait_stream(cur)
            with torch.cuda.stream(side):
                out["rot"] = run("rot", (slot, "side"))
            out["trans"] = run("trans", slot)
            cur.wait_stream(side)
            for t in (tok16, x16):
                t.record_stream(side)
            out["rot"].record_stream(cur)
            return out
        with _conv_backend():
            tok = self.enc(AB)
# ... 87 lines not shown
```

foundationpose_amd/ops.py:

```python
import ctypes as C
from typing import NamedTuple

import numpy as np
import torch

from . import _lib

FLAG_NORMALIZE_XYZ = 1
FLAG_OUT_F16 = 2
MODE_REFINE = 0
MODE_SCORE = 1
ROT_AXIS_ANGLE = 0
ROT_6D = 1
TRANS_TRACKNET, TRANS_DEEPIM, TRANS_RAW = 0, 1, 2


def _stream(t=None):
    if t is None:
        return C.c_void_p(torch.cuda.current_stream().cuda_stream)
    dev = t.device
    if dev.index is not None and dev.index != torch.cuda.current_device():
        raise _lib.FpAmdError(f"tensor on {dev} but the current device is cuda:{torch.cuda.current_device()}: wrap the call in "
                              f"`with torch.cuda.device({dev.index}):` (kernels launch on the current device)")
    return C.c_void_p(torch.cuda.current_stream(dev).cuda_stream)
# ... 894 lines not shown
    host = tri.cpu().numpy().astype(np.int64)
    if host.size == 0:
        return [], roots
    if keep == "largest":
        kept = roots[int(np.argmax(host)):][:1]
    else:
        if int(host.max()) < keep:
            raise ValueError(f"{what}: keep={keep} triangles, the largest of the {host.size} components has {int(host.max())}")
        kept = roots[tri >= keep]
    return sorted((int(x) for x in host), reverse=True), kept


def tsdf_extract(tsdf, weight, color, color_weight, origin, voxel, min_weight=1.0, keep=None):
    what = "tsdf_extract"
    dims, o, s = _tsdf_grid(what, tsdf, weight, color, color_weight, origin, voxel)
    mw = float(min_weight)
    if not np.isfinite(mw):
        raise ValueError(f"{what}: min_weight must be finite, got {min_weight!r}")
    keep = _check_keep(what, keep)
    f, w, c, cw = [_dev(t, torch.float32, name) for name, t in (("tsdf", tsdf), ("weight", weight), ("color", color), ("color_weight", color_weight))]
    dev, L, st = f.device, _lib.lib(), _stream(f)
    nz, ny, nx = dims
    ncubes = (nz - 1) * (ny - 1) * (nx - 1)
    total = 0
    if ncubes > 0:
        counts = torch.empty((ncubes,), dtype=torch.int32, device=dev)
        _lib.check(L.fp_tsdf_count_triangles(_ptr(f), _ptr(w), nz, ny, nx, mw, _ptr(counts), st), "fp_tsdf_count_triangles")
        ends = torch.cumsum(counts, 0, dtype=torch.int64)
        total = int(ends[-1].item())
    report = {} if keep is None else dict(components=[], dropped_triangles=0)
    if total == 0:
        e = torch.empty((0, 3), dtype=torch.float32, device=dev)
        return dict(report, pos=e, vnormals=e.clone(), vertex_color=e.clone(), faces=torch.empty((0, 3), dtype=torch.int32, device=dev))
    if total > 1 << 29:
        raise _lib.FpAmdError(f"{what}: {total} triangles, more than 2^29: use a coarser volume")
    keep_cube = None
    if keep is not None:
        labels, sizes = tsdf_components(counts, dims)
        report["components"], kept = _component_report(what, labels, sizes, keep)
        is_kept = torch.zeros((ncubes,), dtype=torch.bool, device=dev)
        is_kept[kept] = True
        labels = labels.reshape(-1)
        keep_cube = (labels >= 0) & is_kept[labels.clamp(min=0).long()]
    offsets = (ends - counts).contiguous()
    keys = torch.empty((3 * total,), dtype=torch.int64, device=dev)
    pos, col, nrm = (torch.empty((3 * total, 3), dtype=torch.float32, device=dev) for _ in range(3))
    _lib.check(L.fp_tsdf_emit_triangles(_ptr(f), _ptr(w), _ptr(c), _ptr(cw), nz, ny, nx, o.ctypes.data_as(C.c_void_p), s, mw, _ptr(offsets),
                                        total, _ptr(keys), _ptr(pos), _ptr(col), _ptr(nrm), st), "fp_tsdf_emit_triangles")
    if keep_cube is not None:
        rows = torch.repeat_interleave(keep_cube, counts.long(), output_size=total).repeat_interleave(3)
        keys, pos, col, nrm = keys[rows], pos[rows], col[rows], nrm[rows]
        report["dropped_triangles"] = total - int(keys.numel()) // 3
        total = int(keys.numel()) // 3
    uk, inv = torch.unique(keys, return_inverse=True)
    first = torch.full((int(uk.numel()),), 3 * total, dtype=torch.int64, device=dev)
    first.scatter_reduce_(0, inv, torch.arange(3 * total, dtype=torch.int64, device=dev), "amin")
    return dict(report, pos=pos[first], vnormals=nrm[first], vertex_color=col[first], faces=inv.reshape(total, 3).to(torch.int32))


RAYCAST_OUTPUTS = ("depth", "xyz", "normal", "color")
TSDF_RAYCAST_MAX_SAMPLES = 65536
RAYCAST_NO_Z_FAR = float(np.finfo(np.float32).max)


def tsdf_raycast(tsdf, weight, color, color_weight, origin, voxel, poses, K, H, W, out_hw=None, bbox2d=None, step=None, min_weight=1.0,
                 z_near=0.001, z_far=None, want=RAYCAST_OUTPUTS, out=None, views=None):
    what = "tsdf_raycast"
    dims, o, s = _tsdf_grid(what, tsdf, weight, color, color_weight, origin, voxel)
    if not torch.is_tensor(poses):
        raise _lib.FpAmdError(f"{what}: poses must be a tensor, got {type(poses).__name__}")
    if poses.dim() != 3 or tuple(poses.shape[1:]) != (4, 4):
        raise _lib.FpAmdError(f"{what}: poses must be (N,4,4), got {tuple(poses.shape)}")
    N, H, W = int(poses.shape[0]), int(H), int(W)
    if N > 65535:
        raise _lib.FpAmdError(f"{what}: {N} poses in one call, at most 65535 (chunk the batch)")
    if H < 1 or W < 1:
        raise _lib.FpAmdError(f"{what}: a frame of {H} x {W} pixels")
    if bbox2d is None:
        oh, ow = (H, W) if out_hw is None else (int(out_hw[0]), int(out_hw[1]))
        if (oh, ow) != (H, W):
            raise _lib.FpAmdError(f"{what}: without bbox2d the crop is the frame: out_hw must be ({H}, {W}), got ({oh}, {ow})")
    else:
        if out_hw is None:
            raise _lib.FpAmdError(f"{what}: out_hw is required with bbox2d")
        oh, ow = int(out_hw[0]), int(out_hw[1])
        if not torch.is_tensor(bbox2d) or tuple(bbox2d.shape) != (N, 4):
            raise _lib.FpAmdError(f"{what}: bbox2d must be a ({N},4) tensor, got "
                                  f"{tuple(bbox2d.shape) if torch.is_tensor(bbox2d) else type(bbox2d).__name__}")
    if oh < 1 or ow < 1 or oh * ow > 1 << 20:
        raise _lib.FpAmdError(f"{what}: crops of {oh} x {ow} pixels (1 .. 2^20 pixels are supported)")
    want = tuple(want)
    if not want or any(w not in RAYCAST_OUTPUTS for w in want):
        raise ValueError(f"{what}: want must name at least one of {RAYCAST_OUTPUTS}, got {want!r}")
    st = s if step is None else float(step)
    if not (np.isfinite(st) and st > 0 and np.isfinite(np.float32(st)) and np.float32(st) > 0):
        raise ValueError(f"{what}: step must be finite and > 0 (metres), got {step!r}")
    diag = float(np.sqrt(sum((n - 1.0) ** 2 for n in dims))) * s
    if diag / st > TSDF_RAYCAST_MAX_SAMPLES - 2:
        raise ValueError(f"{what}: step={st!r} gives {diag / st:.0f} samples along the volume's diagonal, more than "
                         f"{TSDF_RAYCAST_MAX_SAMPLES - 2}: use a longer step")
    zn, zf, mw = float(z_near), RAYCAST_NO_Z_FAR if z_far is None else float(z_far), float(min_weight)
    if not (np.isfinite(zn) and zn >= 0):
        raise ValueError(f"{what}: z_near must be finite and >= 0 (metres), got {z_near!r}")
    if not (np.isfinite(zf) and zf >= zn):
        raise ValueError(f"{what}: z_far must be finite and >= z_near (metres; None for no limit), got {z_far!r}")
    if not np.isfinite(mw):
        raise ValueError(f"{what}: min_weight must be finite, got {min_weight!r}")
    K9 = vt = None
    if views is not None:
        vt = _views(views, what, N)
    else:
        K9 = np.ascontiguousarray(_hostK33(K, what, "the rays are defined without one").reshape(9).astype(np.float32))
    shapes = dict(depth=(N, oh, ow), xyz=(N, oh, ow, 3), normal=(N, oh, ow, 3), color=(N, oh, ow, 3))
    out = dict(out or {})
    for name in out:
        if name not in want:
            raise ValueError(f"{what}: out has a buffer for '{name}', which is not in want={want!r}")
        if not torch.is_tensor(out[name]) or tuple(out[name].shape) != shapes[name]:
            raise _lib.FpAmdError(f"{what}: out['{name}'] must be a {shapes[name]} tensor")
    P = _dev(poses, torch.float32, "poses")
    bb = _dev(bbox2d, torch.float32, "bbox2d")
    f, w, c, cw = [_dev(t, torch.float32, name) for name, t in (("tsdf", tsdf), ("weight", weight), ("color", color), ("color_weight", color_weight))]
    res = {}
    for name in RAYCAST_OUTPUTS:
        if name in want:
            res[name] = _dev(out[name], torch.float32, f"out['{name}']") if name in out else torch.empty(shapes[name], dtype=torch.float32,
                                                                                                         device=P.device)
    if N == 0:
        return res
    nul = C.c_void_p(0)
    _lib.check(_lib.lib().fp_tsdf_raycast(_ptr(f), _ptr(w), _ptr(c), _ptr(cw), dims[0], dims[1], dims[2], o.ctypes.data_as(C.c_void_p), s, mw,
                                          _ptr(P), nul if K9 is None else K9.ctypes.data_as(C.c_void_p), nul if vt is None else _ptr(vt.K32),
                                          nul if vt is None else _ptr(vt.dev), 0 if vt is None else vt.V, _ptr(bb), H, W, N, oh, ow, st, zn,
                                          zf, _ptr(res.get("depth")), _ptr(res.get("xyz")), _ptr(res.get("normal")), _ptr(res.get("color")),
                                          _stream(P)), "fp_tsdf_raycast")
    return res


TEXTURE_BAKE_MAX_TEXELS, TEXTURE_BAKE_MAX_SIDE = 16, 16384


def texture_atlas_layout(F, texels, Bx=None):
    what = "texture_bake"
    F, T = int(F), int(texels)
    if not 2 <= T <= TEXTURE_BAKE_MAX_TEXELS:
        raise ValueError(f"{what}: texels must be 2..{TEXTURE_BAKE_MAX_TEXELS} (the side of a face's block), got {texels!r}")
    if F > 1 << 24:
        raise ValueError(f"{what}: {F} faces, at most 2^24")
    if Bx is None:
        Bx = max(int(np.ceil(np.sqrt(F))), 1)
        while Bx * Bx < F:
            Bx += 1
        while Bx > 1 and (Bx - 1) * (Bx - 1) >= F:
            Bx -= 1
    Bx = int(Bx)
    if Bx < 1:
        raise ValueError(f"{what}: Bx must be >= 1 block columns, got {Bx}")
    Ht, Wt = -(-F // Bx) * T, Bx * T
    if max(Ht, Wt) > TEXTURE_BAKE_MAX_SIDE:
        raise ValueError(f"{what}: an atlas of {Ht} x {Wt} texels for {F} faces; at most {TEXTURE_BAKE_MAX_SIDE} a side (fewer texels a "
                         "face, or another Bx)")
    return Bx, Ht, Wt


def texture_atlas_uv(F, texels, Bx, device=None):
    Bx, Ht, Wt = texture_atlas_layout(F, texels, Bx)
    T = int(texels)
    f = torch.arange(int(F), dtype=torch.float64, device=device)
    bx, by = torch.remainder(f, Bx), torch.div(f, Bx, rounding_mode="floor")
    dx = torch.tensor([0.0, T - 1.0, 0.0], dtype=torch.float64, device=device)
    dy = torch.tensor([0.0, 0.0, T - 1.0], dtype=torch.float64, device=device)
    uv = torch.stack([(bx[:, None] * T + 0.5 + dx[None]) / Wt, (by[:, None] * T + 0.5 + dy[None]) / Ht], -1)
    return uv.reshape(3 * int(F), 2).float().contiguous(), torch.arange(3 * int(F), dtype=torch.int32, device=device).view(int(F), 3)


def texture_bake(pos, faces, vertex_color, depth, rgb, masks, ob_in_cams, Ks, tol, min_cos, texels=4, Bx=None, min_depth=0.001):
    what = "texture_bake"
    for name, t, nd in (("pos", pos, 2), ("faces", faces, 2), ("depth", depth, 3), ("rgb", rgb, 4), ("ob_in_cams", ob_in_cams, 3)):
        if not torch.is_tensor(t):
            raise _lib.FpAmdError(f"{what}: {name} must be a tensor, got {type(t).__name__}")
        if t.dim() != nd:
            raise _lib.FpAmdError(f"{what}: {name} must have {nd} dimensions, got {tuple(t.shape)}")
    if pos.shape[1] != 3 or faces.shape[1] != 3:
        raise _lib.FpAmdError(f"{what}: pos must be (Nv,3) and faces (F,3), got {tuple(pos.shape)} and {tuple(faces.shape)}")
    Nv, F = int(pos.shape[0]), int(faces.shape[0])
    if vertex_color is not None and (not torch.is_tensor(vertex_color) or tuple(vertex_color.shape) != (Nv, 3)):
        raise _lib.FpAmdError(f"{what}: vertex_color must be a ({Nv},3) tensor like pos or None")
    V, H, W = (int(x) for x in depth.shape)
    if V > 4096:
        raise _lib.FpAmdError(f"{what}: {V} views in one call, at most 4096")
    if H < 1 or W < 1 or H * W > 1 << 28:
        raise _lib.FpAmdError(f"{what}: frames of {H} x {W} pixels (1 .. 2^28 pixels are supported)")
    if tuple(rgb.shape) != (V, H, W, 3):
        raise _lib.FpAmdError(f"{what}: rgb must be ({V},{H},{W},3) like depth, got {tuple(rgb.shape)}")
    if masks is not None and (not torch.is_tensor(masks) or tuple(masks.shape) != (V, H, W)):
        raise _lib.FpAmdError(f"{what}: masks must be a ({V},{H},{W}) tensor like depth or None")
    if tuple(ob_in_cams.shape) != (V, 4, 4):
        raise _lib.FpAmdError(f"{what}: ob_in_cams must be ({V},4,4), got {tuple(ob_in_cams.shape)}")
    Bx, Ht, Wt = texture_atlas_layout(F, texels, Bx)
    tl, mc, md = float(tol), float(min_cos), float(min_depth)
    if not (np.isfinite(tl) and tl >= 0 and np.isfinite(np.float32(tl))):
        raise ValueError(f"{what}: tol must be finite and >= 0 (metres), got {tol!r}")
    if not (0 < np.float32(mc) <= 1):
        raise ValueError(f"{what}: min_cos must be in (0, 1], got {min_cos!r}")
    if not (np.isfinite(md) and md >= 0):
        raise ValueError(f"{what}: min_depth must be finite and >= 0 (metres), got {min_depth!r}")
    K_dev = None
    if torch.is_tensor(Ks) and Ks.is_cuda:
        if tuple(Ks.shape) != (V, 3, 3):
            raise _lib.FpAmdError(f"{what}: device Ks must be ({V},3,3), got {tuple(Ks.shape)}")
        K_dev = Ks
    else:
        Kh = [_hostK33(K, what, "the projection of a texel is defined without one") for K in Ks]
        if len(Kh) != V:
            raise _lib.FpAmdError(f"{what}: {len(Kh)} intrinsic matrices for {V} views")
    p = _dev(pos, torch.float32, "pos")
    fc = _dev(faces, torch.int32, "faces")
    vc = _dev(vertex_color, torch.float32, "vertex_color")
    d = _dev(depth, torch.float32, "depth")
    c = _dev(rgb, torch.float32, "rgb")
    m = _dev(masks, torch.uint8, "masks")
    P = _dev(ob_in_cams, torch.float32, "ob_in_cams")
    K_dev = _dev(K_dev, torch.float64, "Ks")
    tex = torch.empty((Ht, Wt, 3), dtype=torch.float32, device=p.device)
    coverage = torch.empty((Ht, Wt), dtype=torch.uint8, device=p.device)
    uv, uv_idx = texture_atlas_uv(F, texels, Bx, p.device)
    if F == 0:
        return tex, coverage, uv, uv_idx
    if K_dev is None and V > 0:
        K_dev = torch.as_tensor(np.stack(Kh), device=p.device)
    _lib.check(_lib.lib().fp_texture_bake(_ptr(p), Nv, _ptr(fc), F, _ptr(vc), _ptr(d), _ptr(c), _ptr(m), _ptr(P), _ptr(K_dev), V, H, W,
                                          int(texels), Bx, tl, mc, md, _ptr(tex), _ptr(coverage), _stream(p)), "fp_texture_bake")
    return tex, coverage, uv, uv_idx


def pose_update(trans, rot, poses, rot_rep="axis_angle", normalize_xyz=True, trans_normalizer=(1.0, 1.0, 1.0),
                rot_normalizer=1.0, mesh_diameter=1.0, out=None, trans_delta_out=None, rot_delta_out=None, trans_rep="tracknet",
                K=None, tf_to_crops=None, input_w=0, obj=None, views=None):
    if _overlap(out, poses):
        raise _lib.FpAmdError("pose_update: out must not overlap poses (poses_in / poses_out are __restrict__; there is no in-place update)")
    tr = _dev(trans, torch.float32, "trans")
    ro = _dev(rot, torch.float32, "rot")
    P = _dev(poses, torch.float32, "poses")
    N = int(P.shape[0])
    if rot_rep == "axis_angle":
        rr = ROT_AXIS_ANGLE
    elif rot_rep == "6d":
        rr = ROT_6D
    else:
        raise RuntimeError(f"unknown rot_rep {rot_rep}")
    tn = np.ascontiguousarray(np.broadcast_to(np.asarray(trans_normalizer, dtype=np.float32).reshape(-1), (3,)))
    O = out if out is not None else torch.empty_like(P)
    deepim = trans_rep == "deepim"
    tf = _dev(tf_to_crops, torch.float32, "tf_to_crops") if deepim else None
    tro = TRANS_DEEPIM if deepim else (TRANS_TRACKNET if trans_rep == "tracknet" else TRANS_RAW)
    (Kp, Ks, view, V), (dia, d, o, M) = _scene("pose_update", N, K, mesh_diameter, obj, views, need_K=deepim)
    st = _lib.lib().fp_pose_update(_ptr(tr), _ptr(ro), _ptr(P), rr, int(bool(normalize_xyz)), tn.ctypes.data_as(C.c_void_p),
                                   float(rot_normalizer), dia, d, o, M, N, _ptr(O),
                                   _ptr(_dev(trans_delta_out, torch.float32, "trans_delta_out")),
                                   _ptr(_dev(rot_delta_out, torch.float32, "rot_delta_out")), tro, Kp, Ks, view, V, _ptr(tf),
                                   float(input_w), _stream(P))
    _lib.check(st, "fp_pose_update")
    return O


def conv7x7s2_bn_relu(x, w_flat, bias, scale, shift, out, pad):
    x = _dev(x, torch.float16, "x")
    w = _dev(w_flat, torch.float16, "w")
    y = _dev(out, torch.float16, "out")
    Bn, Cin, H, W = x.shape
    if Cin != 6:
        raise _lib.FpAmdError("conv7x7s2_bn_relu: C_in must be 6")
    if tuple(y.shape) != (Bn, H // 2 + 2 * pad, W // 2 + 2 * pad, 64):
        raise _lib.FpAmdError(f"conv7x7s2_bn_relu: out has shape {tuple(y.shape)}")
    st = _lib.lib().fp_conv7x7s2_bn_relu_fwd(_ptr(x), _ptr(w), _ptr(_dev(bias, torch.float32, "bias")),
                                             _ptr(_dev(scale, torch.float32, "scale")), _ptr(_dev(shift, torch.float32, "shift")),
                                             _ptr(y), int(Bn), int(H), int(W), int(pad), _stream(x))
    _lib.check(st, "fp_conv7x7s2_bn_relu_fwd")
    return y


class IgemmGeom(C.Structure):
    _fields_ = [(n, C.c_int) for n in ("pixels_per_image", "width", "padded_h", "padded_w", "stride", "offset", "cstride",
                                       "coff", "bsplit", "cgroup")]

    @staticmethod
    def matrix(ld):
        return IgemmGeom(1, 1, 1, 1, 1, 0, int(ld), 0, 0, 0)

    @staticmethod
    def image(Ho, Wo, pad, C_, stride=1, offset=None, coff=0, bsplit=0, cgroup=0):
        return IgemmGeom(Ho * Wo, Wo, Ho * stride + 2 * pad, Wo * stride + 2 * pad, stride, pad if offset is None else offset,
                         C_, coff, bsplit, cgroup)


IGEMM_RELU = 1
IGEMM_ROUND_ACC = 2
IGEMM_HAS_W_TILES = 4
IGEMM_MFMA_16X16X32 = 16
IGEMM_MFMA_32X32X16 = 32
IGEMM_EPILOGUE_GENERIC = 64
IGEMM_DIRECT_STORE = 256
IGEMM_W_TILES_DIRECT = 512


class IgemmEpilogue(C.Structure):
    _fields_ = [("bias", C.c_void_p), ("bn_scale", C.c_void_p), ("bn_shift", C.c_void_p), ("residual", C.c_void_p),
                ("r_geom", C.POINTER(IgemmGeom)), ("flags", C.c_int), ("pe", C.c_void_p), ("pe_period", C.c_int), ("y_pe", C.c_void_p),
                ("w_tiles", C.c_void_p)]


def pack_conv3x3_tiles(w, N, Cin):
    w = _dev(w, torch.float16, "w")
    out = torch.empty_like(w)
    _lib.check(_lib.lib().fp_pack_conv3x3_tiles_f16(_ptr(w), _ptr(out), int(N), int(Cin), _stream(w)), "fp_pack_conv3x3_tiles_f16")
    return out


def pack_conv3x3_tiles_direct(w, N, Cin):
    w = _dev(w, torch.float16, "w")
    out = torch.empty_like(w)
    _lib.check(_lib.lib().fp_pack_conv3x3_tiles_direct_f16(_ptr(w), _ptr(out), int(N), int(Cin), _stream(w)), "fp_pack_conv3x3_tiles_direct_f16")
    return out


def _igemm_epilogue(bias, residual, r_geom, bn_scale, bn_shift, pe, y_pe, flags, w_tiles=None):
    pe = _dev(pe, torch.float32, "pe")
    ep = IgemmEpilogue()
    ep.bias, ep.bn_scale = _ptr(_dev(bias, torch.float32, "bias")), _ptr(_dev(bn_scale, torch.float32, "bn_scale"))
    ep.bn_shift, ep.residual = _ptr(_dev(bn_shift, torch.float32, "bn_shift")), _ptr(_dev(residual, torch.float16, "residual"))
    ep.r_geom = C.pointer(r_geom) if r_geom is not None else None
    ep.flags = flags
    ep.pe, ep.pe_period, ep.y_pe = _ptr(pe), (int(pe.shape[-2]) if pe is not None else 0), _ptr(_dev(y_pe, torch.float16, "y_pe"))
    ep.w_tiles = _ptr(_dev(w_tiles, torch.float16, "w_tiles"))
    return ep


def igemm_f16(x, x_geom, w, bias, y, y_geom, M, N, Cin, taps, relu=False, residual=None, r_geom=None, bn_scale=None,
              bn_shift=None, conv_rounding=False, pe=None, y_pe=None, w_tiles=None, mfma16=None, direct_store=None, w_tiles_direct=False):
    x = _dev(x, torch.float16, "x"); w = _dev(w, torch.float16, "w"); y = _dev(y, torch.float16, "y")
    from . import engine
    if mfma16 is None:
        mfma16 = engine.CONV_MFMA_16X16X32
    if direct_store is None:
        direct_store = engine.CONV_DIRECT_STORE and (w_tiles is None or bool(w_tiles_direct))
    ep = _igemm_epilogue(bias, residual, r_geom, bn_scale, bn_shift, pe, y_pe,
                         (IGEMM_RELU if relu else 0) | (IGEMM_ROUND_ACC if conv_rounding else 0) | IGEMM_HAS_W_TILES |
                         (IGEMM_MFMA_16X16X32 if mfma16 else IGEMM_MFMA_32X32X16) |
                         (0 if engine.SPECIALIZED_EPILOGUE else IGEMM_EPILOGUE_GENERIC) |
                         (IGEMM_DIRECT_STORE if direct_store else 0) | (IGEMM_W_TILES_DIRECT if w_tiles_direct else 0), w_tiles)
    st = _lib.lib().fp_igemm_f16_fwd(_ptr(x), C.byref(x_geom), _ptr(w), _ptr(y), C.byref(y_geom), int(M), int(N), int(Cin),
                                     int(taps), C.byref(ep), _stream(x))
    _lib.check(st, "fp_igemm_f16_fwd")
    return y


def igemm_splitk_workspace_bytes(M, N, splits):
    return int(_lib.lib().fp_igemm_splitk_workspace_bytes(int(M), int(N), int(splits)))


def igemm_f16_splitk(x, x_geom, w, bias, y, y_geom, M, N, Cin, taps, splits, workspace, relu=False, residual=None, r_geom=None,
                     bn_scale=None, bn_shift=None, conv_rounding=False, pe=None, y_pe=None):
    x = _dev(x, torch.float16, "x"); w = _dev(w, torch.float16, "w"); y = _dev(y, torch.float16, "y")
    ws = _dev(workspace, torch.uint8, "workspace")
    ep = _igemm_epilogue(bias, residual, r_geom, bn_scale, bn_shift, pe, y_pe, (IGEMM_RELU if relu else 0) | (IGEMM_ROUND_ACC if conv_rounding else 0))
    st = _lib.lib().fp_igemm_f16_splitk_fwd(_ptr(x), C.byref(x_geom), _ptr(w), _ptr(y), C.byref(y_geom), int(M), int(N), int(Cin),
                                            int(taps), C.byref(ep), int(splits), _ptr(ws), ws.numel(), _stream(x))
    _lib.check(st, "fp_igemm_f16_splitk_fwd")
    return y


def _work_igemm_splitk(x, x_geom, w, bias, y, y_geom, M, N, Cin, taps, splits, workspace, relu=False, residual=None, r_geom=None, **k):
    return _work_igemm(x, x_geom, w, bias, y, y_geom, M, N, Cin, taps, relu=relu, residual=residual, r_geom=r_geom)


def _work_igemm(x, x_geom, w, bias, y, y_geom, M, N, Cin, taps, relu=False, residual=None, r_geom=None, **k):
    by = 2 * (M * Cin * (1 if taps == 1 else 1.0 / (x_geom.stride ** 2)) + N * Cin * taps + M * N * (2 if residual is not None else 1))
    return by, 2.0 * M * N * Cin * taps


def add_pe_f16(tok, pe):
    tok = _dev(tok, torch.float16, "tok")
    pe = _dev(pe, torch.float32, "pe")
    S, D = int(pe.shape[-2]), int(pe.shape[-1])
    M = tok.numel() // D
    out = torch.empty_like(tok)
    _lib.check(_lib.lib().fp_add_pe_f16_fwd(_ptr(tok), _ptr(pe), _ptr(out), M, S, D, _stream(tok)), "fp_add_pe_f16_fwd")
    return out


def replicate_channels(buf, n, c0, c1):
    buf = _dev(buf, torch.float16, "buf")
    if buf.dim() != 4 or not buf.is_contiguous() or buf.shape[0] < n:
        raise _lib.FpAmdError(f"replicate_channels: buf must be a contiguous (>= {n}, Hp, Wp, C) tensor, got {tuple(buf.shape)}")
    if n <= 1:
        return buf
    _, Hp, Wp, Ct = (int(v) for v in buf.shape)
    src = buf.data_ptr() + 2 * int(c0)
    st = _lib.lib().fp_replicate_rows_f16(C.c_void_p(src), C.c_void_p(src + 2 * Hp * Wp * Ct), int(n) - 1, Hp * Wp, int(c1) - int(c0), Ct, Ct,
                                          Hp * Wp * Ct, _stream(buf))
    _lib.check(st, "fp_replicate_rows_f16")
    return buf


def replicate_segments(buf, segments, c0, c1):
    buf = _dev(buf, torch.float16, "buf")
    n = int(segments.total)
    if buf.dim() != 4 or not buf.is_contiguous() or buf.shape[0] < n:
        raise _lib.FpAmdError(f"replicate_segments: buf must be a contiguous (>= {n}, Hp, Wp, C) tensor, got {tuple(buf.shape)}")
    if int(segments.lengths.min()) < 1:
        raise _lib.FpAmdError("replicate_segments: every segment must hold at least one image (its source)")
    if segments.dev.device != buf.device:
        raise _lib.FpAmdError(f"replicate_segments: offsets on {segments.dev.device}, buf on {buf.device}")
    _, Hp, Wp, Ct = (int(v) for v in buf.shape)
    st = _lib.lib().fp_replicate_segments_f16(C.c_void_p(buf.data_ptr() + 2 * int(c0)), _ptr(segments.dev), len(segments), n, Hp * Wp,
                                              int(c1) - int(c0), Ct, Hp * Wp * Ct, _stream(buf))
    _lib.check(st, "fp_replicate_segments_f16")
    return buf


def layernorm_res(branch16, gamma, beta, eps=1e-5, x32=None, tok16=None, pe=None, want32=True, want16=True):
    br = _dev(branch16, torch.float16, "branch16")
    D = int(br.shape[-1])
    M = br.numel() // D
    x32 = _dev(x32, torch.float32, "x32"); tok16 = _dev(tok16, torch.float16, "tok16"); pe = _dev(pe, torch.float32, "pe")
    S = int(pe.shape[-2]) if pe is not None else 0
    y32 = torch.empty(br.shape, dtype=torch.float32, device=br.device) if want32 else None
    y16 = torch.empty_like(br) if want16 else None
    st = _lib.lib().fp_layernorm_res_fwd(_ptr(x32), _ptr(tok16), _ptr(pe), S, _ptr(br), _ptr(_dev(gamma, torch.float32, "gamma")),
                                         _ptr(_dev(beta, torch.float32, "beta")), float(eps), _ptr(y32), _ptr(y16), M, D, _stream(br))
    _lib.check(st, "fp_layernorm_res_fwd")
    return y32, y16


class PackedLinear512:

    def __init__(self, w16):
        w = _dev(w16, torch.float16, "w16")
        if w.dim() != 2 or int(w.shape[1]) != 512 or int(w.shape[0]) % 512 or int(w.shape[0]) == 0:
            raise _lib.FpAmdError(f"PackedLinear512: weight {tuple(w.shape)}, must be (512 n, 512)")
        self.out_features = int(w.shape[0])
        self.data = torch.empty_like(w)
        for blk in range(self.out_features // 512):
            _lib.check(_lib.lib().fp_pack_linear512_f16(_ptr(w[blk * 512:]), _ptr(self.data[blk * 512:]), _stream(w)), "fp_pack_linear512_f16")


def _packed(w, name, out_features=512):
    if not isinstance(w, PackedLinear512):
        raise _lib.FpAmdError(f"{name}: the weight must be a PackedLinear512 (ops.PackedLinear512(w16))")
    if out_features is not None and w.out_features != out_features:
        raise _lib.FpAmdError(f"{name}: packed weight has {w.out_features} output features, expected {out_features}")
    return w.data


def linear512(x16, w_packed, bias, relu=False, out=None):
    x = _dev(x16, torch.float16, "x16")
    w = _packed(w_packed, "linear512", None)
    if int(x.shape[-1]) != 512:
        raise _lib.FpAmdError(f"linear512: x16 (..., {int(x.shape[-1])}), must be (..., 512)")
    N = w_packed.out_features
    M = x.numel() // 512
    y = out if out is not None else torch.empty(tuple(x.shape[:-1]) + (N,), dtype=torch.float16, device=x.device)
    if y.dtype != torch.float16 or y.numel() != M * N or not y.is_contiguous():
        raise _lib.FpAmdError("linear512: out must be a contiguous fp16 tensor of M x N elements")
    _lib.check(_lib.lib().fp_linear512_f16_fwd(_ptr(x), _ptr(w), _ptr(_dev(bias, torch.float32, "bias")), _ptr(y), M, N, 1 if relu else 0,
                                               _stream(x)), "fp_linear512_f16_fwd")
    return y


def linear_layernorm_res(x16, w_packed, bias, gamma, beta, eps=1e-5, x32=None, tok16=None, pe=None, want32=True, want16=True):
    w = _packed(w_packed, "linear_layernorm_res")
    if not (torch.is_tensor(x16) and x16.is_cuda and x16.dtype == torch.float16):
        raise _lib.FpAmdError("linear_layernorm_res: x16 must be a CUDA float16 tensor")
    K = int(x16.shape[-1])
    D = 512
    if K != 512:
        raise _lib.FpAmdError(f"linear_layernorm_res: x16 (..., {K}), must be (..., 512)")
    M = x16.numel() // K
    x, ldx = x16, _column_block(x16, "linear_layernorm_res: x16", sep="")
    x32 = _dev(x32, torch.float32, "x32"); tok16 = _dev(tok16, torch.float16, "tok16"); pe = _dev(pe, torch.float32, "pe")
    S = int(pe.shape[-2]) if pe is not None else 0
    shape = tuple(x.shape[:-1]) + (D,)
    y32 = torch.empty(shape, dtype=torch.float32, device=x.device) if want32 else None
    y16 = torch.empty(shape, dtype=torch.float16, device=x.device) if want16 else None
    st = _lib.lib().fp_linear_layernorm_fwd(_ptr(x), _ptr(w), _ptr(_dev(bias, torch.float32, "bias")), _ptr(x32), _ptr(tok16), _ptr(pe), S,
                                            _ptr(_dev(gamma, torch.float32, "gamma")), _ptr(_dev(beta, torch.float32, "beta")), float(eps),
                                            _ptr(y32), _ptr(y16), M, K, D, ldx, _stream(x))
    _lib.check(st, "fp_linear_layernorm_fwd")
    return y32, y16


def ffn_layernorm_mean(y16, w1_packed, b1, w2_packed, b2, x32, gamma, beta, eps=1e-5):
    y = _dev(y16, torch.float16, "y16")
    G_, R, D = (int(v) for v in y.shape)
    if D != 512:
        raise _lib.FpAmdError("ffn_layernorm_mean: d_model must be 512")
    x32 = _dev(x32, torch.float32, "x32")
    out = torch.empty((G_, D), dtype=torch.float32, device=y.device)
    if R % 16:
        raise _lib.FpAmdError(f"ffn_layernorm_mean: {R} rows per group, must be a multiple of 16")
    ws = torch.empty((max(G_ * R // 16, 1), 512), dtype=torch.float32, device=y.device)
    st = _lib.lib().fp_ffn_layernorm_mean_fwd(_ptr(y), _ptr(_packed(w1_packed, "ffn_layernorm_mean")), _ptr(_dev(b1, torch.float32, "b1")),
                                              _ptr(_packed(w2_packed, "ffn_layernorm_mean")), _ptr(_dev(b2, torch.float32, "b2")), _ptr(x32),
                                              _ptr(_dev(gamma, torch.float32, "gamma")), _ptr(_dev(beta, torch.float32, "beta")), float(eps),
                                              _ptr(out), _ptr(ws), ws.numel() * 4, G_, R, _stream(y))
    _lib.check(st, "fp_ffn_layernorm_mean_fwd")
    return out


def _column_block(x16, name, sep=":"):
    if not (torch.is_tensor(x16) and x16.is_cuda and x16.dtype == torch.float16 and int(x16.shape[-1]) == 512):
        raise _lib.FpAmdError(f"{name}{sep} must be a CUDA float16 tensor (..., 512)")
    if x16.is_contiguous():
        return 512
    ldx = int(x16.stride(-2)) if x16.dim() >= 2 else 512
    ok = x16.stride(-1) == 1 and ldx % 8 == 0 and ldx >= 512 and x16.storage_offset() % 8 == 0
    for d in range(x16.dim() - 2, 0, -1):
        ok = ok and x16.stride(d - 1) == x16.stride(d) * x16.shape[d]
    if not ok:
        raise _lib.FpAmdError(f"{name}{sep} must be contiguous or a column block of a contiguous tensor")
    return ldx


_TAIL_WS = {}


def encoder_tail_mean(ctx16, wo_packed, bo, tok16, pe, gamma1, beta1, w1_packed, b1, w2_packed, b2, gamma2, beta2, eps=1e-5, workspace=None):
    ldx = _column_block(ctx16, "encoder_tail_mean: ctx16")
    G_, R, _ = (int(v) for v in ctx16.shape)
    tok = _dev(tok16, torch.float16, "tok16")
    pe = _dev(pe, torch.float32, "pe")
    if int(pe.shape[-2]) != R or tuple(tok.shape) != (G_, R, 512):
        raise _lib.FpAmdError("encoder_tail_mean: tok16 must be (G, R, 512) and pe (R, 512)")
    if R % 16:
        raise _lib.FpAmdError(f"encoder_tail_mean: {R} rows per group, must be a multiple of 16")
    out = torch.empty((G_, 512), dtype=torch.float32, device=ctx16.device)
    need = int(_lib.lib().fp_encoder_tail_workspace_bytes(G_, R))
    ws = workspace if workspace is not None else torch.empty(need, dtype=torch.uint8, device=ctx16.device)
    f32 = lambda t, n: _ptr(_dev(t, torch.float32, n))
    st = _lib.lib().fp_encoder_tail_mean_fwd(_ptr(ctx16), ldx, _ptr(_packed(wo_packed, "encoder_tail_mean")), f32(bo, "bo"), _ptr(tok), _ptr(pe),
                                             f32(gamma1, "gamma1"), f32(beta1, "beta1"), _ptr(_packed(w1_packed, "encoder_tail_mean")), f32(b1, "b1"),
                                             _ptr(_packed(w2_packed, "encoder_tail_mean")), f32(b2, "b2"), f32(gamma2, "gamma2"), f32(beta2, "beta2"),
                                             float(eps), _ptr(out), _ptr(ws), ws.numel(), G_, R, _stream(ctx16))
    _lib.check(st, "fp_encoder_tail_mean_fwd")
    return out


def colmean_f16(x, gamma=None, beta=None, eps=1e-5, resid32=None):
    x = _dev(x, torch.float16, "x")
    G_, R, D = (int(v) for v in x.shape)
    out = torch.empty((G_, D), dtype=torch.float32, device=x.device)
    st = _lib.lib().fp_colmean_f16_fwd(_ptr(x), _ptr(_dev(resid32, torch.float32, "resid32")), _ptr(_dev(gamma, torch.float32, "gamma")),
                                       _ptr(_dev(beta, torch.float32, "beta")), float(eps), _ptr(out), G_, R, D, _stream(x))
    _lib.check(st, "fp_colmean_f16_fwd")
    return out


ROWS_ROUND_F16, ROWS_X_F16, ROWS_Y_F16 = 1, 2, 4


def rows_linear(x, w, bias=None, round_f16=False, out_f16=False, out=None):
    if not (torch.is_tensor(x) and x.dtype in (torch.float32, torch.float16)):
        raise _lib.FpAmdError("rows_linear: x must be an f32 or f16 tensor")
    x = _dev(x, x.dtype, "x"); w = _dev(w, torch.float16, "w"); b = _dev(bias, torch.float32, "bias")
    M, K = (int(v) for v in x.shape)
    N = int(w.shape[0])
    ydt = torch.float16 if out_f16 else torch.float32
    y = torch.empty((M, N), dtype=ydt, device=x.device) if out is None else _dev(out, ydt, "out")
    if tuple(y.shape) != (M, N):
        raise _lib.FpAmdError(f"rows_linear: out has shape {tuple(y.shape)}, expected {(M, N)}")
    flags = (ROWS_ROUND_F16 if round_f16 else 0) | (ROWS_X_F16 if x.dtype == torch.float16 else 0) | (ROWS_Y_F16 if out_f16 else 0)
    _lib.check(_lib.lib().fp_rows_linear_fwd(_ptr(x), _ptr(w), _ptr(b), _ptr(y), M, K, N, flags, _stream(x)), "fp_rows_linear_fwd")
    return y


ATT_FP16_SCORES = 1


def _att_head_dim(D3, n_heads, name):
    n_heads = int(n_heads)
    if n_heads <= 0 or D3 % (3 * n_heads):
        raise _lib.FpAmdError(f"{name}: a qkv row of {D3} values is not [q | k | v] of {n_heads} equal heads")
    return D3 // (3 * n_heads)


def attention_f16(qkv, n_heads, fp16_scores=False):
    if qkv.dim() != 3:
        raise _lib.FpAmdError(f"attention_f16: qkv must be (B, S, 3*D), got {tuple(qkv.shape)}")
    hd = _att_head_dim(int(qkv.shape[2]), n_heads, "attention_f16")
    qkv = _dev(qkv, torch.float16, "qkv")
    B, S, D3 = (int(v) for v in qkv.shape)
    D = D3 // 3
    out = torch.empty((B, S, D), dtype=torch.float16, device=qkv.device)
    st = _lib.lib().fp_attention_f16_fwd(_ptr(qkv), _ptr(out), B, S, int(n_heads), hd,
                                         ATT_FP16_SCORES if fp16_scores else 0, _stream(qkv))
    _lib.check(st, "fp_attention_f16_fwd")
    return out


class Segments:

    def __init__(self, lengths, device):
        L = np.asarray(lengths).reshape(-1)
        if L.size == 0:
            raise ValueError("Segments: no segments")
        if L.dtype.kind not in "iu":
            raise ValueError(f"Segments: lengths must be integers, got {L.dtype}")
        L = L.astype(np.int64)
        if L.min() < 0:
            raise ValueError(f"Segments: negative length {int(L.min())}")
        self.lengths = L
        self.offsets = np.concatenate([[0], np.cumsum(L)]).astype(np.int64)
        self.total = int(self.offsets[-1])
        if self.total > np.iinfo(np.int32).max:
            raise ValueError(f"Segments: {self.total} rows do not fit the int32 offset table")
        self.max_S = int(L.max())
        self.B = int(L.size)
        self.dev = torch.as_tensor(self.offsets.astype(np.int32), device=device)

    def __len__(self):
        return self.B

    def rows(self, k):
        return int(self.offsets[k]), int(self.offsets[k + 1])

    def row_ids(self):
        if getattr(self, "_row_ids", None) is None:
            self._row_ids = torch.as_tensor(np.repeat(np.arange(self.B), self.lengths).astype(np.int32), device=self.dev.device)
        return self._row_ids


def attention_f16_segments(qkv, segments, n_heads, fp16_scores=False):
    if qkv.dim() != 2 or qkv.shape[1] % 3:
        raise _lib.FpAmdError(f"attention_f16_segments: qkv must be (Ntot, 3*D), got {tuple(qkv.shape)}")
    hd = _att_head_dim(int(qkv.shape[1]), n_heads, "attention_f16_segments")
    qkv = _dev(qkv, torch.float16, "qkv")
    Ntot, D = int(qkv.shape[0]), int(qkv.shape[1]) // 3
    if Ntot != segments.total:
        raise _lib.FpAmdError(f"attention_f16_segments: {Ntot} rows but the segments cover {segments.total}")
    if segments.dev.device != qkv.device:
        raise _lib.FpAmdError(f"attention_f16_segments: offsets on {segments.dev.device}, qkv on {qkv.device}")
    out = torch.empty((Ntot, D), dtype=torch.float16, device=qkv.device)
    st = _lib.lib().fp_attention_segments_f16_fwd(_ptr(qkv), _ptr(out), _ptr(segments.dev), segments.B, segments.max_S, int(n_heads),
                                                  hd, ATT_FP16_SCORES if fp16_scores else 0, _stream(qkv))
    _lib.check(st, "fp_attention_segments_f16_fwd")
    return out


def cluster_poses(angle_diff, dist_diff, poses, symmetry_tfs):
    P = np.ascontiguousarray(np.asarray(poses, dtype=np.float32).reshape(-1, 16))
    S = np.ascontiguousarray(np.asarray(symmetry_tfs, dtype=np.float32).reshape(-1, 16))
    keep = np.empty(P.shape[0], np.int32)
    n = _lib.lib().fp_cluster_poses(float(angle_diff), float(dist_diff), P.ctypes.data_as(C.c_void_p), P.shape[0],
# ... 134 lines not shown
```

include/fp_amd.h:

```cpp
#ifndef FP_AMD_H
#define FP_AMD_H

#include <stddef.h>
#include <stdint.h>

#ifdef __cplusplus
extern "C" {
#endif

typedef enum {
  FP_OK = 0,
  FP_ERR_INVALID_ARG = -1,
  FP_ERR_WORKSPACE = -2,
  FP_ERR_LAUNCH = -3,
  FP_ERR_UNSUPPORTED = -4
} fp_status;

#define FP_FLAG_NORMALIZE_XYZ 1
#define FP_FLAG_OUT_F16 2

#define FP_MODE_REFINE 0
#define FP_MODE_SCORE 1

#define FP_ROT_AXIS_ANGLE 0
#define FP_ROT_6D 1
#define FP_TRANS_TRACKNET 0
#define FP_TRANS_DEEPIM 1
#define FP_TRANS_RAW 2

#define FP_SUBPIXEL_BITS 4
#define FP_ZBUF_STEPS_PER_METRE 1048576
#define FP_ZBUF_EMPTY 0xFFFFFFFFu

typedef struct fp_mesh fp_mesh;
typedef struct fp_mesh_set fp_mesh_set;

const char* fp_last_error(void);
#define FP_AMD_ABI_VERSION 230
int fp_version(void);

int fp_mesh_create(const float* pos , const float* nrm , const int32_t* faces ,
                   const float* uv , const int32_t* uv_idx ,
                   const float* tex , const float* vcol , int V, int T, int Ht,
                   int Wt, fp_mesh** out);
void fp_mesh_destroy(fp_mesh* mesh);

#define FP_MESH_SET_MAX_ELEMS (1 << 26)
int fp_mesh_set_create(const fp_mesh* const* meshes , int M, fp_mesh_set** out);
void fp_mesh_set_destroy(fp_mesh_set* set);
size_t fp_mesh_set_workspace_bytes(const fp_mesh_set* set, int N, int oh, int ow);

int fp_depth_erode(const float* depth , float* out , int H, int W, int radius,
                   float depth_diff_thres, float ratio_thres, float zfar, void* stream);
int fp_depth_bilateral(const float* depth , float* out , int H, int W, int radius,
                       float zfar, float sigmaD, float sigmaR, void* stream);
int fp_depth_to_xyz(const float* depth , const double* K , float zfar,
                    int f64_internal, float* xyz , int H, int W, void* stream);

int fp_depth_erode_frames(const float* depth , float* out , int H, int W, int V, int radius,
                          float depth_diff_thres, float ratio_thres, float zfar, void* stream);
int fp_depth_bilateral_frames(const float* depth , float* out , int H, int W, int V, int radius,
                              float zfar, float sigmaD, float sigmaR, void* stream);
int fp_depth_to_xyz_frames(const float* depth , const double* Ks , float zfar, int f64_internal,
                           float* xyz , int H, int W, int V, void* stream);

int fp_mask_depth_stats(const float* depth , const uint8_t* masks , const int32_t* view ,
                        int V, int M, int H, int W, float min_depth, int32_t* out , void* stream);

int fp_depth_agreement(const float* depth_crops , const float* xyz_map , const float* tf_to_crops ,
                       const int32_t* view , int V, int H, int W, int N, int oh, int ow, float tol,
                       int32_t* counts , void* stream);
size_t fp_icp_workspace_bytes(int N, int oh, int ow);
int fp_icp_point_plane(const float* xyz_crops , const float* normal_crops ,
                       const float* xyz_map , const float* tf_to_crops ,
                       const int32_t* view , int V, int H, int W, const float* poses_in ,
                       int N, int oh, int ow, float max_dist, double damping, int min_pairs,
                       double* system , float* poses_out ,
                       void* workspace, size_t workspace_bytes, void* stream);
#define FP_ERR_ADD 1
#define FP_ERR_ADDS 2
#define FP_ERR_SYM 4
size_t fp_pose_errors_workspace_bytes(int N, int P, int S);
int fp_pose_errors(const float* model_pts , int P, const double* sym_tfs , int S,
                   const float* poses , const double* gt , const int32_t* gt_index , int G, int N,
                   int flags, double* out , void* workspace , size_t workspace_bytes, void* stream);
#define FP_VSD_MAX_T 16
int fp_vsd_counts(const float* est , const float* gt , const int32_t* gt_index , int G, int N,
                  int h, int w, const float* obs , const float* fac , int H, int W, int x0, int y0, float delta,
                  const float* thr , int T, int32_t* counts , void* stream);
int fp_mspd(const float* model_pts , int P, const double* sym_tfs , int S, const float* poses ,
            const double* gt , const int32_t* gt_index , int G, int N, const float* K ,
            double* out , void* stream);

#define FP_TSDF_MAX_DIM 4096
int fp_tsdf_integrate(const float* depth , const float* rgb , const uint8_t* masks ,
                      const float* ob_in_cams , const double* Ks , int V, int H, int W, int nz, int ny, int nx,
                      const float* origin , float voxel, float trunc, float min_depth, float* tsdf ,
                      float* weight , float* color , float* color_weight , void* stream);
int fp_tsdf_count_triangles(const float* tsdf , const float* weight , int nz, int ny, int nx,
                            float min_weight, int32_t* counts , void* stream);
int fp_tsdf_emit_triangles(const float* tsdf , const float* weight , const float* color ,
                           const float* color_weight , int nz, int ny, int nx, const float* origin , float voxel,
                           float min_weight, const int64_t* offsets , long long total, int64_t* keys ,
                           float* pos , float* col , float* nrm , void* stream);
int fp_tsdf_label_components(const int32_t* counts , int nz, int ny, int nx,
                             int32_t* labels , int32_t* sizes , void* stream);
#define FP_TSDF_RAYCAST_MAX_SAMPLES 65536
int fp_tsdf_raycast(const float* tsdf , const float* weight , const float* color ,
                    const float* color_weight , int nz, int ny, int nx, const float* origin , float voxel,
                    float min_weight, const float* poses , const float* K , const float* Ks ,
                    const int32_t* view , int V, const float* bbox2d , int H, int W, int N, int oh, int ow,
                    float step, float z_near, float z_far, float* depth , float* xyz ,
                    float* normal , float* color_out , void* stream);
#define FP_TEXTURE_BAKE_MAX_TEXELS 16
#define FP_TEXTURE_BAKE_MAX_SIDE 16384
int fp_texture_bake(const float* pos , int Nv, const int32_t* faces , int F,
                    const float* vertex_color , const float* depth ,
                    const float* rgb , const uint8_t* masks ,
                    const float* ob_in_cams , const double* Ks , int V, int H, int W, int T, int Bx, float tol,
                    float min_cos, float min_depth, float* tex , uint8_t* coverage , void* stream);

int fp_crop_windows(const float* poses , const double* K , const double* Ks ,
                    const int32_t* view , int V, double mesh_diameter, const double* diameters ,
                    const int32_t* obj , int M, double crop_ratio, int out_w, int out_h, int N,
                    float* tf_to_crops , float* bbox2d , void* stream);

size_t fp_workspace_bytes(int N, int V, int T, int oh, int ow);
size_t fp_raster_lds_bytes(int ow);

int fp_render_crops(const fp_mesh* mesh , const fp_mesh_set* set , const int32_t* obj ,
                    const double* diameters , float mesh_diameter, const float* poses ,
                    const float* bbox2d , const float* K , const float* Ks ,
                    const int32_t* view , int V, int H, int W, int N, int oh, int ow, float w_ambient,
                    float w_diffuse, float xyz_thr, int flags, void* A , float* color , float* depth ,
                    float* xyz , float* normal , uint32_t* zbuf , int32_t* tri_id ,
                    void* workspace , size_t workspace_bytes, void* stream);

int fp_warp_crops(const float* rgb , const float* xyz_map , const float* depth ,
                  const float* tf_to_crops , const float* K , const float* Ks ,
                  const int32_t* view , int V, const float* poses , float mesh_diameter,
                  const double* diameters , const int32_t* obj , int M, int flags, int mode, int H,
                  int W, int N, int oh, int ow, void* B , void* stream);

int fp_pose_update(const float* trans , const float* rot , const float* poses_in ,
                   int rot_rep, int normalize_xyz, const float* trans_normalizer , float rot_normalizer,
                   float mesh_diameter, const double* diameters , const int32_t* obj , int M, int N,
                   float* poses_out , float* trans_delta_out , float* rot_delta_out ,
                   int trans_rep, const float* K , const float* Ks ,
                   const int32_t* view , int V, const float* tf_to_crops ,
                   float input_w , void* stream);


int fp_conv7x7s2_bn_relu_fwd(const void* x , const void* w , const float* bias ,
                             const float* bn_scale , const float* bn_shift , void* y ,
                             int B, int Hin, int Win, int pad, void* stream);

typedef struct {
  int pixels_per_image, width, padded_h, padded_w, stride, offset, cstride, coff, bsplit, cgroup;
} fp_igemm_geom;

#define FP_IGEMM_RELU 1
#define FP_IGEMM_HAS_W_TILES 4
#define FP_IGEMM_ROUND_ACC 2

#define FP_IGEMM_MFMA_16X16X32 16
#define FP_IGEMM_MFMA_32X32X16 32

#define FP_IGEMM_EPILOGUE_GENERIC 64

#define FP_IGEMM_DIRECT_STORE 256
#define FP_IGEMM_W_TILES_DIRECT 512

typedef struct {
  const float* bias;
  const float* bn_scale;
  const float* bn_shift;
  const void* residual;
  const fp_igemm_geom* r_geom;
  int flags;
  const float* pe;
  int pe_period;
  void* y_pe;
  const void* w_tiles;
} fp_igemm_epilogue;

int fp_igemm_f16_fwd(const void* x , const fp_igemm_geom* x_geom , const void* w , void* y ,
                     const fp_igemm_geom* y_geom , int M, int N, int Cin, int taps,
                     const fp_igemm_epilogue* epilogue , void* stream);

int fp_pack_conv3x3_tiles_f16(const void* w , void* w_tiles , int N, int Cin, void* stream);
int fp_pack_conv3x3_tiles_direct_f16(const void* w , void* w_tiles , int N, int Cin, void* stream);
int fp_conv3x3_sw_lds_bytes(void);

size_t fp_igemm_splitk_workspace_bytes(int M, int N, int splits);
int fp_igemm_f16_splitk_fwd(const void* x , const fp_igemm_geom* x_geom , const void* w , void* y ,
                            const fp_igemm_geom* y_geom , int M, int N, int Cin, int taps,
                            const fp_igemm_epilogue* epilogue , int splits, void* workspace ,
                            size_t workspace_bytes, void* stream);

int fp_add_pe_f16_fwd(const void* tok , const float* pe , void* out , int M, int S, int D, void* stream);

int fp_replicate_rows_f16(const void* src , void* dst , int copies, int rows, int channels, int src_row_stride,
                          int dst_row_stride, long long dst_copy_stride, void* stream);

int fp_replicate_segments_f16(void* buf , const int32_t* seg_offsets , int segments, int images, int pixels,
                              int channels, int pixel_stride, long long image_stride, void* stream);

int fp_layernorm_res_fwd(const float* x32 , const void* tok16 , const float* pe , int S,
                         const void* branch16 , const float* gamma , const float* beta , float eps,
                         float* y32 , void* y16 , int M, int D, void* stream);

int fp_pack_linear512_f16(const void* w16 , void* packed , void* stream);

int fp_linear512_f16_fwd(const void* x16 , const void* w_packed , const float* bias , void* y16 ,
                         int M, int N, int relu, void* stream);

int fp_linear_layernorm_fwd(const void* x16 , const void* w16_packed , const float* bias ,
                            const float* x32 , const void* tok16 , const float* pe , int S,
                            const float* gamma , const float* beta , float eps, float* y32 ,
                            void* y16 , int M, int K, int D, int ldx ,
                            void* stream);

size_t fp_encoder_tail_workspace_bytes(int groups, int rows_per_group);
int fp_encoder_tail_mean_fwd(const void* ctx16 , int ldx, const void* wo_packed , const float* bo ,
                             const void* tok16 , const float* pe , const float* gamma1 , const float* beta1 ,
                             const void* w1_packed , const float* b1 , const void* w2_packed ,
                             const float* b2 , const float* gamma2 , const float* beta2 , float eps,
                             float* out , void* workspace , size_t workspace_bytes, int groups, int rows_per_group,
                             void* stream);

int fp_ffn_layernorm_mean_fwd(const void* y16 , const void* w1_packed , const float* b1 ,
                              const void* w2_packed , const float* b2 , const float* x32 ,
                              const float* gamma , const float* beta , float eps, float* out ,
                              float* workspace , size_t workspace_bytes, int groups, int rows_per_group, void* stream);

int fp_colmean_f16_fwd(const void* x , const float* resid32 , const float* gamma ,
                       const float* beta , float eps, float* out , int groups, int rows_per_group,
                       int D, void* stream);

#define FP_ROWS_ROUND_F16 1
#define FP_ROWS_X_F16 2
#define FP_ROWS_Y_F16 4

int fp_rows_linear_fwd(const void* x , const void* w , const float* bias , void* y ,
                       int M, int K, int N, int flags, void* stream);

#define FP_ATT_FP16_SCORES 1

int fp_attention_f16_fwd(const void* qkv , void* out , int B, int S, int H, int head_dim, int flags,
                         void* stream);

int fp_attention_segments_f16_fwd(const void* qkv , void* out ,
                                  const int32_t* seg_offsets , int B, int max_S, int H, int head_dim, int flags,
                                  void* stream);

int fp_cluster_poses(float angle_diff_deg, float dist_diff, const float* poses , int N,
                     const float* symmetry_tfs , int S, int* keep_idx );

#ifdef __cplusplus
}
#endif
#endif
```

Baseline: 7809.

## Extend direct-store conv epilogue to token layer with positional output

Adds a k_conv_sw_token kernel variant so the conv+BN+residual+positional-embedding layer (which writes a second PE-added output) can use the direct-store epilogue instead of the generic LDS-staged path. The epilogue now loads PE rows via buffer loads and writes the second output inline. It also reuses the output row-offset table for the residual when both share a grid, skipping a table build and barrier. Residual prefetch is deepened to two groups ahead. The cost is more registers for the prefetched residual and PE values, which may lower occupancy, plus a new ABI version and a path-reporting entry point.

```diff
diff --git a/foundationpose_amd/_lib.py b/foundationpose_amd/_lib.py
--- a/foundationpose_amd/_lib.py
+++ b/foundationpose_amd/_lib.py
@@ -5,7 +5,7 @@
 
 _HERE = os.path.dirname(os.path.abspath(__file__))
 LIB_PATH = os.environ.get("FP_AMD_LIB") or os.path.join(_HERE, "csrc", "libfp_amd.so")
-ABI_VERSION = 230
+ABI_VERSION = 231
 _lib = None
 
 vp, ci, cf, cd, sz = C.c_void_p, C.c_int, C.c_float, C.c_double, C.c_size_t
@@ -49,6 +49,7 @@
     "fp_pack_conv3x3_tiles_f16": (ci, [vp, vp, ci, ci, vp]),
     "fp_pack_conv3x3_tiles_direct_f16": (ci, [vp, vp, ci, ci, vp]),
     "fp_conv3x3_sw_lds_bytes": (ci, []),
+    "fp_conv3x3_sw_last_path": (ci, []),
     "fp_igemm_splitk_workspace_bytes": (sz, [ci, ci, ci]),
     "fp_igemm_f16_splitk_fwd": (ci, [vp, vp, vp, vp, vp, ci, ci, ci, ci, vp, ci, vp, sz, vp]),
     "fp_add_pe_f16_fwd": (ci, [vp, vp, vp, ci, ci, ci, vp]),
diff --git a/foundationpose_amd/csrc/conv_sw.hip b/foundationpose_amd/csrc/conv_sw.hip
--- a/foundationpose_amd/csrc/conv_sw.hip
+++ b/foundationpose_amd/csrc/conv_sw.hip
@@ -71,13 +71,19 @@
 
 template <int BM, int BN, int TM, bool S16>
 __global__ __launch_bounds__(512, 1) void k_conv_sw(IgemmParams p) {
-  constexpr bool DIRECT = false;
+  constexpr bool DIRECT = false, TOKEN = false;
 #include "conv_sw_tile.inc"
 }
 
 template <int BM, int BN, int TM, bool S16>
 __global__ __launch_bounds__(512, 1) void k_conv_sw_direct(IgemmParams p) {
-  constexpr bool DIRECT = true;
+  constexpr bool DIRECT = true, TOKEN = false;
+#include "conv_sw_tile.inc"
+}
+
+template <int BM, int BN, int TM, bool S16>
+__global__ __launch_bounds__(512, 1) void k_conv_sw_token(IgemmParams p) {
+  constexpr bool DIRECT = true, TOKEN = true;
 #include "conv_sw_tile.inc"
 }
 
@@ -334,21 +340,43 @@
 
 static bool sw_direct(const IgemmParams& p) {
   if (!p.direct || !p.mfma16 || sw_variant(p) == 1 || sw_use_256(p)) return false;
+  if (p.epi == (IG_EPI_CONV | IG_EPI_BN | IG_EPI_RES | IG_EPI_PE))
+    return (p.direct & 2) && (long long)p.pe_period * p.N < (1ll << 30) && (long long)p.M * p.N < (1ll << 31);
   return p.epi == IG_EPI_CONV || p.epi == (IG_EPI_CONV | IG_EPI_RES) || p.epi == (IG_EPI_CONV | IG_EPI_BN) || p.epi == (IG_EPI_CONV | IG_EPI_BN | IG_EPI_RES);
 }
 
-static int sw_direct_launch(const IgemmParams& p, hipStream_t stream) {
+static bool sw_same_grid(const IgemmGeom& a, const IgemmGeom& b) {
+  return a.HoWo == b.HoWo && a.Wo == b.Wo && a.Hp == b.Hp && a.Wp == b.Wp && a.stride == b.stride && a.off == b.off && a.cstride == b.cstride &&
+         a.coff == b.coff && a.bsplit == b.bsplit && a.cgroup == b.cgroup;
+}
+
+static thread_local int sw_last_path = 0;
+
+static int sw_direct_launch(const IgemmParams& p0, hipStream_t stream) {
   constexpr int LDS = sw_lds_bytes(512, 128);
-  const long long tiles = (long long)fp_cdiv(p.M, 512) * (p.N / 128);
+  const long long tiles = (long long)fp_cdiv(p0.M, 512) * (p0.N / 128);
   FP_REQUIRE(tiles < (1ll << 31), "fp_igemm_f16_fwd: too many tiles");
+  IgemmParams p = p0;
+  if (p.epi & IG_EPI_PE) {
+    FP_SET_MAX_LDS((k_conv_sw_token<512, 128, 4, true>), LDS);
+    hipLaunchKernelGGL((k_conv_sw_token<512, 128, 4, true>), dim3((unsigned)tiles), dim3(512), LDS, stream, p);
+    FP_CHECK_LAUNCH("fp_igemm_f16_fwd(conv_sw_token)");
+    sw_last_path = FP_CONV_SW_PATH_DIRECT | FP_CONV_SW_PATH_RES_OWN_TABLE;
+    return FP_OK;
+  }
+  if (p.R && sw_same_grid(p.out, p.res)) p.epi |= IG_EPI_SAME_GRID;
   FP_SET_MAX_LDS((k_conv_sw_direct<512, 128, 4, true>), LDS);
   hipLaunchKernelGGL((k_conv_sw_direct<512, 128, 4, true>), dim3((unsigned)tiles), dim3(512), LDS, stream, p);
   FP_CHECK_LAUNCH("fp_igemm_f16_fwd(conv_sw_direct)");
+  sw_last_path = FP_CONV_SW_PATH_DIRECT | (p.R ? ((p.epi & IG_EPI_SAME_GRID) ? FP_CONV_SW_PATH_RES_OUTPUT_TABLE : FP_CONV_SW_PATH_RES_OWN_TABLE) : 0);
   return FP_OK;
 }
+
+extern "C" int fp_conv3x3_sw_last_path(void) { return sw_last_path; }
 
 int fp_conv3x3_sw_launch(const IgemmParams& p, hipStream_t stream) {
   const bool direct = sw_direct(p);
+  sw_last_path = 0;
   if (p.Wpk && sw_variant(p) != 1 && !sw_use_256(p))
     FP_REQUIRE((p.wpk_direct != 0) == direct, "fp_igemm_f16_fwd: w_tiles is in the layout of %s but this launch runs %s (FP_IGEMM_W_TILES_DIRECT, FP_IGEMM_DIRECT_STORE)",
                p.wpk_direct ? "fp_pack_conv3x3_tiles_direct_f16" : "fp_pack_conv3x3_tiles_f16", direct ? "k_conv_sw_direct" : "k_conv_sw");
diff --git a/foundationpose_amd/csrc/conv_sw_tile.inc b/foundationpose_amd/csrc/conv_sw_tile.inc
--- a/foundationpose_amd/csrc/conv_sw_tile.inc
+++ b/foundationpose_amd/csrc/conv_sw_tile.inc
@@ -271,17 +271,25 @@
   if constexpr (DIRECT) {
     const IgEpiArgs q = {p.out, p.res, p.R, p.Y, p.pe, p.Ype, p.pe_period, p.pe_mul, p.pe_shr, p.N};
     const int* rowY32 = reinterpret_cast<const int*>(smem + STAGES_BYTES);
+    const bool same_grid = (p.epi & IG_EPI_SAME_GRID) != 0;
 #define SW_DIRECT_CASE(E)                                                                                     \
     case E:                                                                                                   \
-      if (m0 + BM <= M) ig_epilogue_direct<E, true>(q, acc, smem, rowY32, m0, n0, M, wm, wn, tid, lane, bias_lds);  \
-      else ig_epilogue_direct<E, false>(q, acc, smem, rowY32, m0, n0, M, wm, wn, tid, lane, bias_lds);         \
+      if (m0 + BM <= M) ig_epilogue_direct<E, true>(q, acc, smem, rowY32, m0, n0, M, same_grid, wm, wn, tid, lane, bias_lds);  \
+      else ig_epilogue_direct<E, false>(q, acc, smem, rowY32, m0, n0, M, same_grid, wm, wn, tid, lane, bias_lds);         \
       break
-    switch (p.epi) {
-      SW_DIRECT_CASE(IG_EPI_CONV);
-      SW_DIRECT_CASE(IG_EPI_CONV | IG_EPI_RES);
-      SW_DIRECT_CASE(IG_EPI_CONV | IG_EPI_BN);
-      SW_DIRECT_CASE(IG_EPI_CONV | IG_EPI_BN | IG_EPI_RES);
-      default: break;
+    if constexpr (TOKEN) {
+      switch (p.epi) {
+        SW_DIRECT_CASE(IG_EPI_CONV | IG_EPI_BN | IG_EPI_RES | IG_EPI_PE);
+        default: break;
+      }
+    } else {
+      switch (p.epi & ~IG_EPI_SAME_GRID) {
+        SW_DIRECT_CASE(IG_EPI_CONV);
+        SW_DIRECT_CASE(IG_EPI_CONV | IG_EPI_RES);
+        SW_DIRECT_CASE(IG_EPI_CONV | IG_EPI_BN);
+        SW_DIRECT_CASE(IG_EPI_CONV | IG_EPI_BN | IG_EPI_RES);
+        default: break;
+      }
     }
 #undef SW_DIRECT_CASE
   } else {
diff --git a/foundationpose_amd/csrc/igemm.hip b/foundationpose_amd/csrc/igemm.hip
--- a/foundationpose_amd/csrc/igemm.hip
+++ b/foundationpose_amd/csrc/igemm.hip
@@ -340,7 +340,7 @@
   FP_REQUIRE((e.bn_scale == nullptr) == (e.bn_shift == nullptr), "%s: bn_scale and bn_shift go together", who);
   FP_REQUIRE(!e.bn_scale || (e.flags & FP_IGEMM_ROUND_ACC), "%s: BatchNorm needs FP_IGEMM_ROUND_ACC (conv semantics)", who);
   FP_REQUIRE((e.flags & ~(FP_IGEMM_RELU | FP_IGEMM_ROUND_ACC | FP_IGEMM_HAS_W_TILES | FP_IGEMM_MFMA_16X16X32 | FP_IGEMM_MFMA_32X32X16 | FP_IGEMM_EPILOGUE_GENERIC |
-                           FP_IGEMM_DIRECT_STORE | FP_IGEMM_W_TILES_DIRECT)) == 0,
+                           FP_IGEMM_DIRECT_STORE | FP_IGEMM_W_TILES_DIRECT | FP_IGEMM_DIRECT_TOKEN)) == 0,
              "%s: unknown flags 0x%x", who, e.flags);
   FP_REQUIRE((e.flags & (FP_IGEMM_MFMA_16X16X32 | FP_IGEMM_MFMA_32X32X16)) != (FP_IGEMM_MFMA_16X16X32 | FP_IGEMM_MFMA_32X32X16),
              "%s: FP_IGEMM_MFMA_16X16X32 and FP_IGEMM_MFMA_32X32X16 exclude each other", who);
@@ -362,7 +362,7 @@
   p.in = ig_geom(x_geom); p.out = ig_geom(y_geom); p.res = e.residual ? ig_geom(e.r_geom) : ig_geom(y_geom);
   p.slab = nullptr; p.nsplit = 0;
   p.epi = ig_epilogue_mode(p, e.flags);
-  p.direct = (e.flags & FP_IGEMM_DIRECT_STORE) ? 1 : 0; p.wpk_direct = (e.flags & FP_IGEMM_W_TILES_DIRECT) ? 1 : 0;
+  p.direct = (e.flags & FP_IGEMM_DIRECT_STORE) ? 1 | ((e.flags & FP_IGEMM_DIRECT_TOKEN) ? 2 : 0) : 0; p.wpk_direct = (e.flags & FP_IGEMM_W_TILES_DIRECT) ? 1 : 0;
   ig_fastdiv_init(p.pe_period, &p.pe_mul, &p.pe_shr);
   return FP_OK;
 }
diff --git a/foundationpose_amd/csrc/igemm_common.h b/foundationpose_amd/csrc/igemm_common.h
--- a/foundationpose_amd/csrc/igemm_common.h
+++ b/foundationpose_amd/csrc/igemm_common.h
@@ -73,6 +73,7 @@
 #define IG_EPI_RES 16
 #define IG_EPI_RELU 32
 #define IG_EPI_PE 64
+#define IG_EPI_SAME_GRID 128
 #define IG_EPI_CONV (IG_EPI_SPEC | IG_EPI_ROUND_ACC | IG_EPI_BIAS | IG_EPI_RELU)
 
 __device__ __forceinline__ long long ig_row_off(const IgemmGeom& g, int m) {
diff --git a/foundationpose_amd/csrc/igemm_epilogue.h b/foundationpose_amd/csrc/igemm_epilogue.h
--- a/foundationpose_amd/csrc/igemm_epilogue.h
+++ b/foundationpose_amd/csrc/igemm_epilogue.h
@@ -224,25 +224,29 @@
 }
 template <int EPI, bool FULL, typename Acc>
 __device__ __forceinline__ void ig_epilogue_direct(const IgEpiArgs& p, Acc& acc, unsigned char* smem, const int* rowY32, int m0, int n0, int M,
-                                                   int wm, int wn, int tid, int lane, const float* bias_lds) {
+                                                   bool same_grid, int wm, int wn, int tid, int lane, const float* bias_lds) {
   constexpr int TM = 4;
   static_assert(std::is_same<Acc, ig_float4[4][2 * TM]>::value, "accumulators of the 16x16x32 loop");
-  static_assert((EPI & IG_EPI_CONV) == IG_EPI_CONV && !(EPI & IG_EPI_PE), "conv rounding + bias + ReLU, without the positional output");
-  constexpr bool HAS_BN = (EPI & IG_EPI_BN) != 0, RES = (EPI & IG_EPI_RES) != 0;
+  static_assert((EPI & IG_EPI_CONV) == IG_EPI_CONV, "conv rounding + bias + ReLU");
+  constexpr bool HAS_BN = (EPI & IG_EPI_BN) != 0, RES = (EPI & IG_EPI_RES) != 0, PE = (EPI & IG_EPI_PE) != 0;
+  static_assert(!PE || RES, "the token layer: the positional second output on top of a residual");
   typedef float float4_ __attribute__((ext_vector_type(4)));
   typedef int int4_ __attribute__((ext_vector_type(4)));
   typedef unsigned uint2_ __attribute__((ext_vector_type(2)));
   typedef _Float16 half2_ __attribute__((ext_vector_type(2)));
-  constexpr int JG = 2, NG = 2 * TM / JG;
+  constexpr int JG = PE ? 1 : 2, NG = 2 * TM / JG, AHEAD = 2;
   const int nl = wn * 64 + 4 * (lane & 15);
   const int prow = wm * (32 * TM) + 4 * (lane >> 4);
-  int* rowR32 = reinterpret_cast<int*>(smem);
+  const int* rowR32 = same_grid ? rowY32 : reinterpret_cast<const int*>(smem);
   IG_CLK(te0);
   if constexpr (RES) {
-    const int m = FULL || m0 + tid < M ? m0 + tid : M - 1;
-    rowR32[tid] = (int)(ig_row_off(p.res, m) + n0);
-    __syncthreads();
-  }
+    if (!same_grid) {
+      const int m = FULL || m0 + tid < M ? m0 + tid : M - 1;
+      reinterpret_cast<int*>(smem)[tid] = (int)(ig_row_off(p.res, m) + n0);
+      __syncthreads();
+    }
+  }
+  const int r_last = RES && !FULL ? (int)(ig_row_off(p.res, M - 1) + n0) : 0;
   IG_CLK(te1);
   const float4_ bv = *reinterpret_cast<const float4_*>(bias_lds + nl);
   const half2_ b01 = {(_Float16)bv[0], (_Float16)bv[1]}, b23 = {(_Float16)bv[2], (_Float16)bv[3]};
@@ -253,23 +257,38 @@
   }
   const __amdgpu_buffer_rsrc_t rsY = __builtin_amdgcn_make_buffer_rsrc(ig_uniform_ptr(p.Y), 0, -1, 0x00020000);
   const __amdgpu_buffer_rsrc_t rsR = __builtin_amdgcn_make_buffer_rsrc(ig_uniform_ptr(p.R), 0, -1, 0x00020000);
-  half4 rv[RES ? 2 : 1][JG * 4];
+  const __amdgpu_buffer_rsrc_t rsP = __builtin_amdgcn_make_buffer_rsrc(ig_uniform_ptr(p.pe), 0, -1, 0x00020000);
+  const __amdgpu_buffer_rsrc_t rsQ = __builtin_amdgcn_make_buffer_rsrc(ig_uniform_ptr(p.Ype), 0, -1, 0x00020000);
+  const int mrow = m0 + prow;
+  const int ncol = n0 + nl;
+  half4 rv[RES ? NG : 1][JG * 4];
+  float4_ pv[PE ? NG : 1][JG * 4];
   auto res_group = [&](int g) {
     if constexpr (RES) {
 #pragma unroll
       for (int jj = 0; jj < JG; ++jj) {
         const int4_ ro = *reinterpret_cast<const int4_*>(rowR32 + prow + 16 * (g * JG + jj));
 #pragma unroll
-        for (int e = 0; e < 4; ++e)
-          rv[g & 1][jj * 4 + e] = __builtin_bit_cast(half4, __builtin_amdgcn_raw_buffer_load_b64(rsR, (int)((unsigned)(ro[e] + nl) << 1), 0, 0));
+        for (int e = 0; e < 4; ++e) {
+          const int o = FULL || ro[e] != IG_ROW_NONE ? ro[e] : r_last;
+          rv[g][jj * 4 + e] = __builtin_bit_cast(half4, __builtin_amdgcn_raw_buffer_load_b64(rsR, (int)((unsigned)(o + nl) << 1), 0, 0));
+        }
+        if constexpr (PE) {
+#pragma unroll
+          for (int e = 0; e < 4; ++e) {
+            const int m = mrow + 16 * (g * JG + jj) + e;
+            const int mp = m - ig_fastdiv(m, p.pe_mul, p.pe_shr) * p.pe_period;
+            pv[g][jj * 4 + e] = __builtin_bit_cast(float4_, __builtin_amdgcn_raw_buffer_load_b128(rsP, (int)((unsigned)(mp * p.N + ncol) << 2), 0, 0));
+          }
+        }
       }
       __builtin_amdgcn_sched_barrier(0);
     }
   };
-  res_group(0);
+#pragma unroll
+  for (int g = 0; g < AHEAD; ++g) res_group(g);
 #pragma unroll
   for (int g = 0; g < NG; ++g) {
-    if (g + 1 < NG) res_group(g + 1);
 #pragma unroll
     for (int jj = 0; jj < JG; ++jj) {
       const int j = g * JG + jj;
@@ -289,13 +308,23 @@
         } else {
           v[0] = t01[0]; v[1] = t01[1]; v[2] = t23[0]; v[3] = t23[1];
         }
-        if constexpr (RES) v = v + rv[g & 1][jj * 4 + e];
+        if constexpr (RES) v = v + rv[g][jj * 4 + e];
         v = ig_relu4(v);
-        if (FULL || yo[e] != IG_ROW_NONE)
+        if (FULL || yo[e] != IG_ROW_NONE) {
           __builtin_amdgcn_raw_buffer_store_b64(__builtin_bit_cast(uint2_, v), rsY, (int)((unsigned)(yo[e] + nl) << 1), 0, 0);
+          if constexpr (PE) {
+            const float4_ pr = pv[g][jj * 4 + e];
+            half4 w;
+#pragma unroll
+            for (int c = 0; c < 4; ++c) w[c] = (_Float16)((float)v[c] + pr[c]);
+            const int m = mrow + 16 * j + e;
+            __builtin_amdgcn_raw_buffer_store_b64(__builtin_bit_cast(uint2_, w), rsQ, (int)((unsigned)(m * p.N + ncol) << 1), 0, 0);
+          }
+        }
       }
     }
     __builtin_amdgcn_sched_barrier(0);
+    if (g + AHEAD < NG) res_group(g + AHEAD);
   }
 #ifdef FP_PROFILE_BUILD
   IG_CLK(te2);
diff --git a/foundationpose_amd/engine.py b/foundationpose_amd/engine.py
--- a/foundationpose_amd/engine.py
+++ b/foundationpose_amd/engine.py
@@ -22,6 +22,7 @@
 CONV_MFMA_16X16X32 = True
 SPECIALIZED_EPILOGUE = True
 CONV_DIRECT_STORE = True
+CONV_DIRECT_TOKEN = True
 
 
 def _conv_backend():
@@ -133,7 +134,8 @@
     b = sd.get(conv_p + ".bias")
     scale, shift = _bn_affine(sd, bn_p)
     wk = w.permute(0, 2, 3, 1).reshape(w.shape[0], -1).to(torch.float16).contiguous()
-    tiles, direct = None, bool(CONV_DIRECT_STORE and CONV_MFMA_16X16X32 and SPECIALIZED_EPILOGUE and b is not None and not second_output)
+    tiles, direct = None, bool(CONV_DIRECT_STORE and CONV_MFMA_16X16X32 and SPECIALIZED_EPILOGUE and b is not None and
+                               (not second_output or (CONV_DIRECT_TOKEN and scale is not None)))
     if wk.is_cuda and w.shape[2] == 3 and w.shape[3] == 3 and w.shape[0] % 128 == 0 and w.shape[1] % 32 == 0 and PACKED_CONV_TILES:
         tiles = (ops.pack_conv3x3_tiles_direct if direct else ops.pack_conv3x3_tiles)(wk, w.shape[0], w.shape[1])
     return dict(w=wk, w_tiles=tiles, tiles_direct=direct and tiles is not None, bias=None if b is None else _r16(b.float()), scale=scale, shift=shift)
@@ -144,7 +146,7 @@
 SPLITK_TARGET_WGS = 384
 SMALL_CALL_CEILING = 31
 
-_SWITCHES = ("FUSED_OUT_PROJ_LN", "FUSED_FFN", "ROWS_QKV", "PACKED_CONV_TILES", "MERGED_HEAD_QKV", "FUSED_TAIL", "CONV_MFMA_16X16X32", "SPECIALIZED_EPILOGUE", "CONV_DIRECT_STORE", "SPLITK_MAX_HYPS", "HEADS_TWO_STREAMS_MAX_HYPS")
+_SWITCHES = ("FUSED_OUT_PROJ_LN", "FUSED_FFN", "ROWS_QKV", "PACKED_CONV_TILES", "MERGED_HEAD_QKV", "FUSED_TAIL", "CONV_MFMA_16X16X32", "SPECIALIZED_EPILOGUE", "CONV_DIRECT_STORE", "CONV_DIRECT_TOKEN", "SPLITK_MAX_HYPS", "HEADS_TWO_STREAMS_MAX_HYPS")
 
 
 @contextlib.contextmanager
diff --git a/foundationpose_amd/ops.py b/foundationpose_amd/ops.py
--- a/foundationpose_amd/ops.py
+++ b/foundationpose_amd/ops.py
@@ -1220,6 +1220,8 @@
 IGEMM_EPILOGUE_GENERIC = 64
 IGEMM_DIRECT_STORE = 256
 IGEMM_W_TILES_DIRECT = 512
+IGEMM_DIRECT_TOKEN = 1024
+CONV_SW_PATH_DIRECT, CONV_SW_PATH_RES_OUTPUT_TABLE, CONV_SW_PATH_RES_OWN_TABLE = 1, 2, 4
 
 
 class IgemmEpilogue(C.Structure):
@@ -1233,6 +1235,10 @@
     out = torch.empty_like(w)
     _lib.check(_lib.lib().fp_pack_conv3x3_tiles_f16(_ptr(w), _ptr(out), int(N), int(Cin), _stream(w)), "fp_pack_conv3x3_tiles_f16")
     return out
+
+
+def conv3x3_sw_last_path():
+    return int(_lib.lib().fp_conv3x3_sw_last_path())
 
 
 def pack_conv3x3_tiles_direct(w, N, Cin):
@@ -1255,18 +1261,21 @@
 
 
 def igemm_f16(x, x_geom, w, bias, y, y_geom, M, N, Cin, taps, relu=False, residual=None, r_geom=None, bn_scale=None,
-              bn_shift=None, conv_rounding=False, pe=None, y_pe=None, w_tiles=None, mfma16=None, direct_store=None, w_tiles_direct=False):
+              bn_shift=None, conv_rounding=False, pe=None, y_pe=None, w_tiles=None, mfma16=None, direct_store=None, w_tiles_direct=False, direct_token=None):
     x = _dev(x, torch.float16, "x"); w = _dev(w, torch.float16, "w"); y = _dev(y, torch.float16, "y")
     from . import engine
     if mfma16 is None:
         mfma16 = engine.CONV_MFMA_16X16X32
     if direct_store is None:
         direct_store = engine.CONV_DIRECT_STORE and (w_tiles is None or bool(w_tiles_direct))
+    if direct_token is None:
+        direct_token = engine.CONV_DIRECT_TOKEN and (w_tiles is None or bool(w_tiles_direct))
     ep = _igemm_epilogue(bias, residual, r_geom, bn_scale, bn_shift, pe, y_pe,
                          (IGEMM_RELU if relu else 0) | (IGEMM_ROUND_ACC if conv_rounding else 0) | IGEMM_HAS_W_TILES |
                          (IGEMM_MFMA_16X16X32 if mfma16 else IGEMM_MFMA_32X32X16) |
                          (0 if engine.SPECIALIZED_EPILOGUE else IGEMM_EPILOGUE_GENERIC) |
-                         (IGEMM_DIRECT_STORE if direct_store else 0) | (IGEMM_W_TILES_DIRECT if w_tiles_direct else 0), w_tiles)
+                         (IGEMM_DIRECT_STORE if direct_store else 0) | (IGEMM_W_TILES_DIRECT if w_tiles_direct else 0) |
+                         (IGEMM_DIRECT_TOKEN if direct_token else 0), w_tiles)
     st = _lib.lib().fp_igemm_f16_fwd(_ptr(x), C.byref(x_geom), _ptr(w), _ptr(y), C.byref(y_geom), int(M), int(N), int(Cin),
                                      int(taps), C.byref(ep), _stream(x))
     _lib.check(st, "fp_igemm_f16_fwd")
diff --git a/include/fp_amd.h b/include/fp_amd.h
--- a/include/fp_amd.h
+++ b/include/fp_amd.h
@@ -36,7 +36,7 @@
 typedef struct fp_mesh_set fp_mesh_set;
 
 const char* fp_last_error(void);
-#define FP_AMD_ABI_VERSION 230
+#define FP_AMD_ABI_VERSION 231
 int fp_version(void);
 
 int fp_mesh_create(const float* pos , const float* nrm , const int32_t* faces ,
@@ -170,6 +170,7 @@
 
 #define FP_IGEMM_DIRECT_STORE 256
 #define FP_IGEMM_W_TILES_DIRECT 512
+#define FP_IGEMM_DIRECT_TOKEN 1024
 
 typedef struct {
   const float* bias;
@@ -191,6 +192,10 @@
 int fp_pack_conv3x3_tiles_f16(const void* w , void* w_tiles , int N, int Cin, void* stream);
 int fp_pack_conv3x3_tiles_direct_f16(const void* w , void* w_tiles , int N, int Cin, void* stream);
 int fp_conv3x3_sw_lds_bytes(void);
+#define FP_CONV_SW_PATH_DIRECT 1
+#define FP_CONV_SW_PATH_RES_OUTPUT_TABLE 2
+#define FP_CONV_SW_PATH_RES_OWN_TABLE 4
+int fp_conv3x3_sw_last_path(void);
 
 size_t fp_igemm_splitk_workspace_bytes(int M, int N, int splits);
 int fp_igemm_f16_splitk_fwd(const void* x , const fp_igemm_geom* x_geom , const void* w , void* y ,
```

Result: no change. 7808 (-0.0%).
